# vsois/hanabi-agents

Measured on AMD Instinct MI355X. Metric: env_steps_per_sec, higher is better.
Workload: dtype u8 env/encoder + bfloat16 Q-net GEMM (fp32 accumulate, fp32 master weights)

## Files before the change

### hanabi-agents_amd/csrc/learner.hip

```cpp
#include <hip/hip_runtime.h>
#include <cstdlib>
#include <cstdint>
#include <hip/hip_bf16.h>
#include <hip/hip_fp16.h>

#include "../../include/hanabi_hip.h"
#include "common.hpp"

using hb::fail;

namespace {

template <typename T> __device__ __forceinline__ float ld(const T* p, long long i);
template <> __device__ __forceinline__ float ld<float>(const float* p, long long i) { return p[i]; }
template <> __device__ __forceinline__ float ld<__hip_bfloat16>(const __hip_bfloat16* p, long long i) { return __bfloat162float(p[i]); }
template <> __device__ __forceinline__ float ld<__half>(const __half* p, long long i) { return __half2float(p[i]); }
template <typename T> __device__ __forceinline__ void st(T* p, long long i, float v);
template <> __device__ __forceinline__ void st<float>(float* p, long long i, float v) { p[i] = v; }
template <> __device__ __forceinline__ void st<__hip_bfloat16>(__hip_bfloat16* p, long long i, float v) { p[i] = __float2bfloat16(v); }
template <> __device__ __forceinline__ void st<__half>(__half* p, long long i, float v) { p[i] = __float2half(v); }

__device__ __forceinline__ float wave_max(float v) {
  for (int o = 32; o > 0; o >>= 1) v = fmaxf(v, __shfl_xor(v, o));
  return v;
}
__device__ __forceinline__ float wave_sum(float v) {
  for (int o = 32; o > 0; o >>= 1) v += __shfl_xor(v, o);
  return v;
}

struct NStep {
  const long long* size_wp;
  long long cap, n_ins;
  int n_step;
  float gamma;
};

template <typename T>
__global__ __launch_bounds__(256) void gather_kernel(const int8_t* __restrict__ ring_tm1, const int8_t* __restrict__ ring_t,
                                                     const int8_t* __restrict__ ring_act, const float* __restrict__ ring_rew,
                                                     const uint8_t* __restrict__ ring_term, const int64_t* __restrict__ idx,
                                                     int B, int L, T* __restrict__ x, int x_ld, int32_t* __restrict__ act,
                                                     float* __restrict__ rew, float* __restrict__ term,
                                                     float* __restrict__ disc, const NStep ns, int packed_words) {
  __shared__ long long s_slot;
  const int r = blockIdx.x;
  const int b = r < B ? r : r - B;
  long long slot = idx[b];
  if (r >= B) {
    if (threadIdx.x == 0) {
      long long j = slot;
      float R = ring_rew[j], g = ns.gamma;
      int m = 1;
      if (ns.n_step > 1) {
        const long long size = ns.size_wp[0], wp = ns.size_wp[1];
        const long long ahead = size >= ns.cap ? ((wp - 1 - slot) % ns.cap + ns.cap) % ns.cap : size - 1 - slot;
        while (m < ns.n_step && !ring_term[j] && static_cast<long long>(m) * ns.n_ins <= ahead) {
          j = (j + ns.n_ins) % ns.cap;
          R += g * ring_rew[j];
          g *= ns.gamma;
          ++m;
        }
      }
      rew[b] = R;
      term[b] = ring_term[j] ? 1.f : 0.f;
      disc[b] = g;
      s_slot = j;
    }
    __syncthreads();
    slot = s_slot;
  } else if (threadIdx.x == 0) {
    act[b] = ring_act[slot];
  }
  T* dst = x + static_cast<long long>(r) * x_ld;
  if (packed_words > 0) {
    const uint32_t* src = reinterpret_cast<const uint32_t*>(r < B ? ring_tm1 : ring_t) + slot * packed_words;
    for (int j = threadIdx.x; j < L; j += 256) st<T>(dst, j, static_cast<float>((src[j >> 5] >> (j & 31)) & 1u));
    return;
  }
  const int8_t* src = (r < B ? ring_tm1 : ring_t) + slot * L;
  for (int j = threadIdx.x; j < L; j += 256) st<T>(dst, j, static_cast<float>(src[j]));
}

template <typename T>
__global__ __launch_bounds__(256) void c51_kernel(const T* __restrict__ logits_on, const T* __restrict__ logits_t,
                                                  const int32_t* __restrict__ act, const float* __restrict__ rew,
                                                  const float* __restrict__ term, const double* __restrict__ prios,
                                                  const float* __restrict__ beta_dev, const float* __restrict__ disc, int mask_terminal,
                                                  const float* __restrict__ support, int B, int A, int K, int rs,
                                                  float* __restrict__ td_out, float* __restrict__ w_out,
                                                  T* __restrict__ dlogits, float* __restrict__ counter,
                                                  const T* __restrict__ bias_on, const T* __restrict__ bias_t) {
  extern __shared__ float lds[];
  const int lane = threadIdx.x & 63, wave = threadIdx.x >> 6;
  const int b = blockIdx.x * 4 + wave;
  if (counter && blockIdx.x == 0 && threadIdx.x == 0) *counter += 1.f;
  if (b >= B) return;
  const int AK = A * K;
  float* sel = lds + wave * (AK + 64);
  const float beta = *beta_dev;
  float wmax = 0.f;
  for (int j = lane; j < B; j += 64) wmax = fmaxf(wmax, powf(static_cast<float>(1.0 / prios[j]), beta));
  wmax = wave_max(wmax);
  const float w_b = powf(static_cast<float>(1.0 / prios[b]), beta) / wmax;
  const T* row_sel = logits_on + static_cast<long long>(B + b) * rs;
  for (int e = lane; e < AK; e += 64) sel[e] = ld<T>(row_sel, e) + (bias_on ? ld<T>(bias_on, e) : 0.f);
  __builtin_amdgcn_fence(__ATOMIC_RELEASE, "wavefront");
  __builtin_amdgcn_wave_barrier();
  __builtin_amdgcn_fence(__ATOMIC_ACQUIRE, "wavefront");
  float q = -INFINITY;
  if (lane < A) {
    const float* r = sel + lane * K;
    float m = r[0];
    for (int k = 1; k < K; ++k) m = fmaxf(m, r[k]);
    float s = 0.f, t = 0.f;
    for (int k = 0; k < K; ++k) {
      const float e = __expf(r[k] - m);
      s += e;
      t += e * support[k];
    }
    q = t / s / static_cast<float>(K);
  }
  const float qbest = wave_max(q);
  const unsigned long long hit = __ballot(lane < A && q == qbest);
  const int a_star = __ffsll(static_cast<long long>(hit)) - 1;
  const bool atom = lane < K;
  const float lt = atom ? ld<T>(logits_t, static_cast<long long>(b) * rs + a_star * K + lane) +
                              (bias_t ? ld<T>(bias_t, a_star * K + lane) : 0.f)
                        : -INFINITY;
  const float mt = wave_max(lt);
  const float et = atom ? __expf(lt - mt) : 0.f;
  const float p = et / wave_sum(et);
  const float vmin = support[0], vmax = support[K - 1];
  const float delta = (vmax - vmin) / static_cast<float>(K - 1);
  float gamma = disc[b];
  if (mask_terminal) gamma *= 1.f - term[b];
  const float zi = atom ? support[lane] : 0.f;
  const float tz = fminf(fmaxf(rew[b] + gamma * zi, vmin), vmax);
  float target = 0.f;
  const float inv_delta = 1.f / delta;
  for (int j = 0; j < K; ++j) {
    const float pj = __int_as_float(__builtin_amdgcn_readlane(__float_as_int(p), j));
    const float tzj = __int_as_float(__builtin_amdgcn_readlane(__float_as_int(tz), j));
    target += pj * fminf(fmaxf(1.f - fabsf(tzj - zi) * inv_delta, 0.f), 1.f);
  }
  if (!atom) target = 0.f;
  const int a_tm1 = act[b];
  const float l1 = atom ? ld<T>(logits_on, static_cast<long long>(b) * rs + a_tm1 * K + lane) +
                              (bias_on ? ld<T>(bias_on, a_tm1 * K + lane) : 0.f)
                        : -INFINITY;
  const float m1 = wave_max(l1);
  const float e1 = atom ? __expf(l1 - m1) : 0.f;
  const float s1 = wave_sum(e1);
  const float logp = atom ? (l1 - m1 - __logf(s1)) : 0.f;
  const float td = -wave_sum(target * logp);
  const float tsum = wave_sum(target);
  if (lane == 0) {
    td_out[b] = td;
    w_out[b] = w_b;
  }
  T* drow = dlogits + static_cast<long long>(b) * rs;
  for (int e = lane; e < rs; e += 64) st<T>(drow, e, 0.f);
  __builtin_amdgcn_fence(__ATOMIC_RELEASE, "wavefront");
  __builtin_amdgcn_wave_barrier();
  if (atom) st<T>(drow, a_tm1 * K + lane, (w_b / static_cast<float>(B)) * (e1 / s1 * tsum - target));
}

template <typename T>
__global__ __launch_bounds__(1024) void colsum_kernel(const T* __restrict__ x, int rows, int cols, float* __restrict__ out) {
  __shared__ float part[16][64];
  const int l = threadIdx.x & 63, c = blockIdx.x * 64 + l, rg = threadIdx.x >> 6;
  float s = 0.f;
  if (c < cols) {
#pragma unroll 16
    for (int i = rg; i < rows; i += 16) s += ld<T>(x, static_cast<long long>(i) * cols + c);
  }
  part[rg][l] = s;
  __syncthreads();
  if (rg == 0 && c < cols) {
    float t = 0.f;
#pragma unroll
    for (int g = 0; g < 16; ++g) t += part[g][l];
    out[c] = t;
  }
}

template <typename T>
__global__ __launch_bounds__(1024) void relu_bwd_colsum_kernel(T* __restrict__ dy, const T* __restrict__ act, int rows, int cols,
                                                               int act_ld, float* __restrict__ out) {
  __shared__ float part[16][64];
  const int l = threadIdx.x & 63, c = blockIdx.x * 64 + l, rg = threadIdx.x >> 6;
  float s = 0.f;
  if (c < cols) {
#pragma unroll 16
    for (int i = rg; i < rows; i += 16) {
      const long long k = static_cast<long long>(i) * cols + c;
      const float g = ld<T>(act, static_cast<long long>(i) * act_ld + c) > 0.f ? ld<T>(dy, k) : 0.f;
      st<T>(dy, k, g);
      s += g;
    }
  }
  part[rg][l] = s;
  __syncthreads();
  if (rg == 0 && c < cols) {
    float t = 0.f;
#pragma unroll
    for (int g = 0; g < 16; ++g) t += part[g][l];
    out[c] = t;
  }
}

struct AdamArgs {
  float *w, *w_mu, *w_sigma;
  const float* noise;
  const void* grad;
  float *m_w, *v_w, *m_mu, *v_mu, *m_sg, *v_sg;
  const float* step;
  void* eff;
  long long n;
  int cols, eff_ld;
  int grad_dtype, grad_ld;
  float lr, b1, b2, eps;
  float step_offset;
};

__device__ __forceinline__ float load_grad(const void* g, int dtype, long long i) {
  if (dtype == 1) return __bfloat162float(static_cast<const __hip_bfloat16*>(g)[i]);
  if (dtype == 2) return __half2float(static_cast<const __half*>(g)[i]);
  return static_cast<const float*>(g)[i];
}

__device__ __forceinline__ float adam1(float p, float g, float& m, float& v, float b1, float b2, float bc1, float bc2s,
                                       float lr, float eps) {
  m = __fmaf_rn(b1, m, __fmul_rn(1.f - b1, g));
  v = __fmaf_rn(b2, v, __fmul_rn(__fmul_rn(1.f - b2, g), g));
  return __fsub_rn(p, __fdiv_rn(__fmul_rn(lr / bc1, m), __fadd_rn(__fdiv_rn(sqrtf(v), bc2s), eps)));
}
__device__ __forceinline__ float adam_step(float m, float v, float bc1, float bc2s, float lr, float eps) {
  return __fdiv_rn(__fmul_rn(lr / bc1, m), __fadd_rn(__fdiv_rn(sqrtf(v), bc2s), eps));
}
__device__ __forceinline__ float merged(float w, float mu, float sg, float nz) {
  return __fadd_rn(__fadd_rn(w, mu), __fmul_rn(sg, nz));
}

template <typename T>
__global__ __launch_bounds__(256) void noisy_adam_kernel(const AdamArgs a) {
  const float t = *a.step + a.step_offset;
  const float bc1 = 1.f - powf(a.b1, t), bc2s = sqrtf(1.f - powf(a.b2, t));
  T* eff = static_cast<T*>(a.eff);
  for (long long i = static_cast<long long>(blockIdx.x) * blockDim.x + threadIdx.x; i < a.n;
       i += static_cast<long long>(gridDim.x) * blockDim.x) {
    const long long row = i / a.cols, col = i - row * a.cols;
    const float g = load_grad(a.grad, a.grad_dtype, row * a.grad_ld + col), nz = a.noise[i];
    float m, v;
    m = a.m_w[i]; v = a.v_w[i];
    const float w = adam1(a.w[i], g, m, v, a.b1, a.b2, bc1, bc2s, a.lr, a.eps);
    a.m_w[i] = m; a.v_w[i] = v; a.w[i] = w;
    float mu;
    if (a.m_mu == a.m_w) {
      mu = __fsub_rn(a.w_mu[i], adam_step(m, v, bc1, bc2s, a.lr, a.eps));
    } else {
      m = a.m_mu[i]; v = a.v_mu[i];
      mu = adam1(a.w_mu[i], g, m, v, a.b1, a.b2, bc1, bc2s, a.lr, a.eps);
      a.m_mu[i] = m; a.v_mu[i] = v;
    }
    a.w_mu[i] = mu;
    m = a.m_sg[i]; v = a.v_sg[i];
    const float sg = adam1(a.w_sigma[i], __fmul_rn(g, nz), m, v, a.b1, a.b2, bc1, bc2s, a.lr, a.eps);
    a.m_sg[i] = m; a.v_sg[i] = v; a.w_sigma[i] = sg;
    st<T>(eff, row * a.eff_ld + col, merged(w, mu, sg, nz));
  }
}

struct AdamMulti {
  AdamArgs t[8];
  int first[9];
  int count;
};

template <int W> struct VecW;
template <> struct VecW<4> { typedef float4 type; };
template <> struct VecW<2> { typedef float2 type; };
template <int W>
__device__ __forceinline__ void ldw(const float* p, uint32_t off, float out[W]) {
  const typename VecW<W>::type v = *reinterpret_cast<const typename VecW<W>::type*>(reinterpret_cast<const char*>(p) + static_cast<uint64_t>(off << 2));
  const float* f = reinterpret_cast<const float*>(&v);
#pragma unroll
  for (int k = 0; k < W; ++k) out[k] = f[k];
}
template <int W>
__device__ __forceinline__ void stw(float* p, uint32_t off, const float in[W]) {
  typename VecW<W>::type v;
  float* f = reinterpret_cast<float*>(&v);
#pragma unroll
  for (int k = 0; k < W; ++k) f[k] = in[k];
  *reinterpret_cast<typename VecW<W>::type*>(reinterpret_cast<char*>(p) + static_cast<uint64_t>(off << 2)) = v;
}
template <int W>
__device__ __forceinline__ void load_gradw(const void* g, int dtype, uint32_t i, float out[W]) {
  if (dtype == 0) {
    ldw<W>(static_cast<const float*>(g), i, out);
  } else if (dtype == 1) {
    const uint32_t* p = reinterpret_cast<const uint32_t*>(static_cast<const char*>(g) + static_cast<uint64_t>(i << 1));
    if constexpr (W == 4) {
      const uint2 v = *reinterpret_cast<const uint2*>(p);
      out[0] = __uint_as_float(v.x << 16); out[1] = __uint_as_float(v.x & 0xFFFF0000u);
      out[2] = __uint_as_float(v.y << 16); out[3] = __uint_as_float(v.y & 0xFFFF0000u);
    } else {
      const uint32_t v = *p;
      out[0] = __uint_as_float(v << 16); out[1] = __uint_as_float(v & 0xFFFF0000u);
    }
  } else {
    const __half* h = reinterpret_cast<const __half*>(static_cast<const char*>(g) + static_cast<uint64_t>(i << 1));
#pragma unroll
    for (int k = 0; k < W; ++k) out[k] = __half2float(h[k]);
  }
}

template <typename T, int W>
__global__ __launch_bounds__(256) void noisy_adam_multiw_kernel(const AdamMulti m) {
  constexpr int SH = W == 4 ? 2 : 1;
  int ti = 0;
  while (ti + 1 < m.count && static_cast<int>(blockIdx.x) >= m.first[ti + 1]) ++ti;
  const AdamArgs& a = m.t[ti];
  const float t = *a.step + a.step_offset;
  const float bc1 = 1.f - powf(a.b1, t), bc2s = sqrtf(1.f - powf(a.b2, t));
  T* eff = static_cast<T*>(a.eff);
  const int nw = static_cast<int>(a.n >> SH), cw = a.cols >> SH;
  const int q = (static_cast<int>(blockIdx.x) - m.first[ti]) * 256 + static_cast<int>(threadIdx.x);
  if (q < nw) {
    const int row = q / cw, col = (q - row * cw) << SH;
    const uint32_t i = static_cast<uint32_t>(q) << SH;
    float g[W], nz[W];
    load_gradw<W>(a.grad, a.grad_dtype, static_cast<uint32_t>(row) * static_cast<uint32_t>(a.grad_ld) + col, g);
    ldw<W>(a.noise, i, nz);
    float res[3][W], lm[W], lv[W];
    auto one = [&](float* p, float* mp, float* vp, int which) {
      float pa[W], ma[W], va[W];
      ldw<W>(p, i, pa); ldw<W>(mp, i, ma); ldw<W>(vp, i, va);
#pragma unroll
      for (int k = 0; k < W; ++k) {
        pa[k] = adam1(pa[k], which == 2 ? __fmul_rn(g[k], nz[k]) : g[k], ma[k], va[k], a.b1, a.b2, bc1, bc2s, a.lr, a.eps);
        res[which][k] = pa[k];
        lm[k] = ma[k];
        lv[k] = va[k];
      }
      stw<W>(p, i, pa); stw<W>(mp, i, ma); stw<W>(vp, i, va);
    };
    one(a.w, a.m_w, a.v_w, 0);

    if (a.m_mu == a.m_w) {
      float pv[W];
      ldw<W>(a.w_mu, i, pv);
#pragma unroll
      for (int k = 0; k < W; ++k) res[1][k] = pv[k] = __fsub_rn(pv[k], adam_step(lm[k], lv[k], bc1, bc2s, a.lr, a.eps));
      stw<W>(a.w_mu, i, pv);
    } else {
      one(a.w_mu, a.m_mu, a.v_mu, 1);
    }

    one(a.w_sigma, a.m_sg, a.v_sg, 2);
    const uint32_t e = static_cast<uint32_t>(row) * static_cast<uint32_t>(a.eff_ld) + col;
#pragma unroll
    for (int k = 0; k < W; ++k) st<T>(eff, e + k, merged(res[0][k], res[1][k], res[2][k], nz[k]));
  }
}

template <typename T>
__global__ __launch_bounds__(256) void noisy_adam_multi_kernel(const AdamMulti m) {
  int ti = 0;
  while (ti + 1 < m.count && static_cast<int>(blockIdx.x) >= m.first[ti + 1]) ++ti;
  const AdamArgs& a = m.t[ti];
  const int nb = m.first[ti + 1] - m.first[ti];
  const float t = *a.step + a.step_offset;
  const float bc1 = 1.f - powf(a.b1, t), bc2s = sqrtf(1.f - powf(a.b2, t));
  T* eff = static_cast<T*>(a.eff);
  for (long long i = static_cast<long long>(blockIdx.x - m.first[ti]) * 256 + threadIdx.x; i < a.n;
       i += static_cast<long long>(nb) * 256) {
    const long long row = i / a.cols, col = i - row * a.cols;
    const float g = load_grad(a.grad, a.grad_dtype, row * a.grad_ld + col), nz = a.noise[i];
    float mm, vv;
    mm = a.m_w[i]; vv = a.v_w[i];
    const float w = adam1(a.w[i], g, mm, vv, a.b1, a.b2, bc1, bc2s, a.lr, a.eps);
    a.m_w[i] = mm; a.v_w[i] = vv; a.w[i] = w;
    float mu;
    if (a.m_mu == a.m_w) {
      mu = __fsub_rn(a.w_mu[i], adam_step(mm, vv, bc1, bc2s, a.lr, a.eps));
    } else {
      mm = a.m_mu[i]; vv = a.v_mu[i];
      mu = adam1(a.w_mu[i], g, mm, vv, a.b1, a.b2, bc1, bc2s, a.lr, a.eps);
      a.m_mu[i] = mm; a.v_mu[i] = vv;
    }
    a.w_mu[i] = mu;
    mm = a.m_sg[i]; vv = a.v_sg[i];
    const float sg = adam1(a.w_sigma[i], __fmul_rn(g, nz), mm, vv, a.b1, a.b2, bc1, bc2s, a.lr, a.eps);
    a.m_sg[i] = mm; a.v_sg[i] = vv; a.w_sigma[i] = sg;
    st<T>(eff, row * a.eff_ld + col, merged(w, mu, sg, nz));
  }
}

struct AdamPackOut {
  void* wt; int wt_ld;
  uint4* frag; int frag_kind;
  const int* col_map;
  float* bias_f32;
};
struct AdamPackMulti {
  AdamArgs t[4];
  AdamPackOut o[4];
  int first[5];
  int tiles_n[4];
  int count;
};

template <typename T>
__global__ __launch_bounds__(256) void noisy_adam_pack_kernel(const AdamPackMulti m) {
  __shared__ uint16_t tile[8][132];
  int ti = 0;
  while (ti + 1 < m.count && static_cast<int>(blockIdx.x) >= m.first[ti + 1]) ++ti;
  const AdamArgs& a = m.t[ti];
  const AdamPackOut& o = m.o[ti];
  const int tid = static_cast<int>(threadIdx.x), tb = static_cast<int>(blockIdx.x) - m.first[ti];
  const float t = *a.step + a.step_offset;
  const float bc1 = 1.f - powf(a.b1, t), bc2s = sqrtf(1.f - powf(a.b2, t));
  T* eff = static_cast<T*>(a.eff);
  const int tn = m.tiles_n[ti];
  const int rows = static_cast<int>(a.n / a.cols);
  int k, n;
  if (tn > 0) {
    k = (tb / tn) * 8 + (tid >> 5);
    n = (tb % tn) * 128 + 4 * (tid & 31);
  } else {
    k = 0;
    n = (tb * 256 + tid) * 4;
  }
  const bool valid = k < rows && n < a.cols;
  float mv[4] = {0.f, 0.f, 0.f, 0.f};
  if (valid) {
    const uint32_t i = static_cast<uint32_t>(k) * static_cast<uint32_t>(a.cols) + n;
    float g[4], nz[4], res[3][4], lm[4], lv[4];
    load_gradw<4>(a.grad, a.grad_dtype, static_cast<uint32_t>(k) * static_cast<uint32_t>(a.grad_ld) + n, g);
    ldw<4>(a.noise, i, nz);
    auto one = [&](float* p, float* mp, float* vp, int which) {
      float pa[4], ma[4], va[4];
      ldw<4>(p, i, pa); ldw<4>(mp, i, ma); ldw<4>(vp, i, va);
#pragma unroll
      for (int j = 0; j < 4; ++j) {
        pa[j] = adam1(pa[j], which == 2 ? __fmul_rn(g[j], nz[j]) : g[j], ma[j], va[j], a.b1, a.b2, bc1, bc2s, a.lr, a.eps);
        res[which][j] = pa[j];
        lm[j] = ma[j];
        lv[j] = va[j];
      }
      stw<4>(p, i, pa); stw<4>(mp, i, ma); stw<4>(vp, i, va);
    };
    one(a.w, a.m_w, a.v_w, 0);
    if (a.m_mu == a.m_w) {
      float pv[4];
      ldw<4>(a.w_mu, i, pv);
#pragma unroll
      for (int j = 0; j < 4; ++j) res[1][j] = pv[j] = __fsub_rn(pv[j], adam_step(lm[j], lv[j], bc1, bc2s, a.lr, a.eps));
      stw<4>(a.w_mu, i, pv);
    } else {
      one(a.w_mu, a.m_mu, a.v_mu, 1);
    }
    one(a.w_sigma, a.m_sg, a.v_sg, 2);
    const uint32_t e = static_cast<uint32_t>(k) * static_cast<uint32_t>(a.eff_ld) + n;
#pragma unroll
    for (int j = 0; j < 4; ++j) {
      mv[j] = merged(res[0][j], res[1][j], res[2][j], nz[j]);
      st<T>(eff, e + j, mv[j]);
    }
    if (tn == 0 && o.bias_f32) {
#pragma unroll
      for (int j = 0; j < 4; ++j) o.bias_f32[o.col_map ? o.col_map[n + j] : n + j] = ld<T>(eff, e + j);
    }
  }
  if (tn == 0 || (!o.wt && !o.frag_kind)) return;
  {
    T r4[4];
#pragma unroll
    for (int j = 0; j < 4; ++j) st<T>(r4, j, mv[j]);
    *reinterpret_cast<uint2*>(&tile[tid >> 5][4 * (tid & 31)]) = *reinterpret_cast<const uint2*>(r4);
  }
  __syncthreads();
  if (tid < 128) {
    const int col = tid;
    const int nn = (tb % tn) * 128 + col, k0 = (tb / tn) * 8;
    if (nn < a.cols) {
      uint16_t v[8];
#pragma unroll
      for (int i = 0; i < 8; ++i) v[i] = tile[i][col];
      const uint4 vec = *reinterpret_cast<const uint4*>(v);
      if (o.wt) *reinterpret_cast<uint4*>(static_cast<uint16_t*>(o.wt) + static_cast<size_t>(nn) * o.wt_ld + k0) = vec;
      const int s = k0 >> 5, ch = (k0 >> 3) & 3;
      if (o.frag_kind == 1) {
        o.frag[(s * 32 + (nn >> 4)) * 64 + ch * 16 + (nn & 15)] = vec;
      } else if (o.frag_kind == 2) {
        const int ph = o.col_map[nn];
        o.frag[(((ph >> 9) * 16 + s) * 32 + ((ph & 511) >> 4)) * 64 + ch * 16 + (ph & 15)] = vec;
      }
    }
  }
}

template <typename T>
void launch_adam(const AdamArgs& a, hipStream_t s) {
  long long blocks = (a.n + 255) / 256;
  if (blocks > 2048) blocks = 2048;
  hipLaunchKernelGGL((noisy_adam_kernel<T>), dim3(static_cast<unsigned>(blocks)), dim3(256), 0, s, a);
}

}

extern "C" {

static int replay_gather_impl(const int8_t* ring_obs_tm1_dev, const int8_t* ring_obs_t_dev, const int8_t* ring_act_dev,
                     const float* ring_rew_dev, const uint8_t* ring_term_dev, const int64_t* idx_dev, int64_t batch,
                     int32_t obs_len, void* x_dev, int32_t x_dtype, int32_t x_ld, int32_t* act_dev, float* rew_dev,
                     float* term_dev, float* disc_dev, int32_t n_step, float gamma, int64_t capacity, int64_t rows_per_insert,
                     const int64_t* size_wp_dev, void* stream, int packed_words) {
  if (!ring_obs_tm1_dev || !ring_obs_t_dev || !ring_act_dev || !ring_rew_dev || !ring_term_dev || !idx_dev || !x_dev ||
      !act_dev || !rew_dev || !term_dev || !disc_dev)
    return fail(HB_ERR_INVALID, "null argument");
  if (batch <= 0) return HB_OK;
  if (x_ld < obs_len) return fail(HB_ERR_INVALID, "x_ld must be >= obs_len");
  if (n_step < 1) return fail(HB_ERR_INVALID, "n_step must be >= 1");
  if (n_step > 1 && (!size_wp_dev || rows_per_insert < 1 || capacity < 1))
    return fail(HB_ERR_INVALID, "n_step > 1 needs size_wp_dev, rows_per_insert and capacity");
  const NStep ns{reinterpret_cast<const long long*>(size_wp_dev), capacity, rows_per_insert, n_step, gamma};
  hipStream_t s = static_cast<hipStream_t>(stream);
  const dim3 grid(static_cast<unsigned>(2 * batch)), block(256);
  const int B = static_cast<int>(batch);
  if (x_dtype == 0)
    hipLaunchKernelGGL((gather_kernel<float>), grid, block, 0, s, ring_obs_tm1_dev, ring_obs_t_dev, ring_act_dev, ring_rew_dev, ring_term_dev, idx_dev, B, obs_len, static_cast<float*>(x_dev), x_ld, act_dev, rew_dev, term_dev, disc_dev, ns, packed_words);
  else if (x_dtype == 1)
    hipLaunchKernelGGL((gather_kernel<__hip_bfloat16>), grid, block, 0, s, ring_obs_tm1_dev, ring_obs_t_dev, ring_act_dev, ring_rew_dev, ring_term_dev, idx_dev, B, obs_len, static_cast<__hip_bfloat16*>(x_dev), x_ld, act_dev, rew_dev, term_dev, disc_dev, ns, packed_words);
  else if (x_dtype == 2)
    hipLaunchKernelGGL((gather_kernel<__half>), grid, block, 0, s, ring_obs_tm1_dev, ring_obs_t_dev, ring_act_dev, ring_rew_dev, ring_term_dev, idx_dev, B, obs_len, static_cast<__half*>(x_dev), x_ld, act_dev, rew_dev, term_dev, disc_dev, ns, packed_words);
  else
    return fail(HB_ERR_INVALID, "x_dtype must be 0 (f32), 1 (bf16) or 2 (f16)");
  HB_HIP(hipGetLastError());
  return HB_OK;
}

int hb_replay_gather(const int8_t* ring_obs_tm1_dev, const int8_t* ring_obs_t_dev, const int8_t* ring_act_dev,
                     const float* ring_rew_dev, const uint8_t* ring_term_dev, const int64_t* idx_dev, int64_t batch,
                     int32_t obs_len, void* x_dev, int32_t x_dtype, int32_t x_ld, int32_t* act_dev, float* rew_dev,
                     float* term_dev, float* disc_dev, int32_t n_step, float gamma, int64_t capacity, int64_t rows_per_insert,
                     const int64_t* size_wp_dev, void* stream) {
  return replay_gather_impl(ring_obs_tm1_dev, ring_obs_t_dev, ring_act_dev, ring_rew_dev, ring_term_dev, idx_dev, batch, obs_len,
                            x_dev, x_dtype, x_ld, act_dev, rew_dev, term_dev, disc_dev, n_step, gamma, capacity, rows_per_insert,
                            size_wp_dev, stream, 0);
}

int hb_replay_gather_packed(const uint32_t* ring_bits_tm1_dev, const uint32_t* ring_bits_t_dev, const int8_t* ring_act_dev,
                            const float* ring_rew_dev, const uint8_t* ring_term_dev, const int64_t* idx_dev, int64_t batch,
                            int32_t obs_len, void* x_dev, int32_t x_dtype, int32_t x_ld, int32_t* act_dev, float* rew_dev,
                            float* term_dev, float* disc_dev, int32_t n_step, float gamma, int64_t capacity,
                            int64_t rows_per_insert, const int64_t* size_wp_dev, void* stream) {
  if (obs_len < 1) return fail(HB_ERR_INVALID, "obs_len must be positive");
  return replay_gather_impl(reinterpret_cast<const int8_t*>(ring_bits_tm1_dev), reinterpret_cast<const int8_t*>(ring_bits_t_dev),
                            ring_act_dev, ring_rew_dev, ring_term_dev, idx_dev, batch, obs_len, x_dev, x_dtype, x_ld, act_dev,
                            rew_dev, term_dev, disc_dev, n_step, gamma, capacity, rows_per_insert, size_wp_dev, stream,
                            (obs_len + 31) / 32);
}

int hb_c51_loss_grad(const void* logits_online_dev, const void* logits_target_dev, int32_t dtype, const int32_t* act_dev,
                     const float* rew_dev, const float* term_dev, const double* prios_dev, const float* beta_dev,
                     const float* disc_dev, int32_t mask_terminal, const float* support_dev, int64_t batch, int32_t n_actions,
                     int32_t n_atoms, int32_t row_stride, float* td_dev, float* w_dev, void* dlogits_dev, float* update_counter_dev,
                     const void* bias_online_dev, const void* bias_target_dev, void* stream) {
  if (!logits_online_dev || !logits_target_dev || !act_dev || !rew_dev || !term_dev || !prios_dev || !beta_dev || !disc_dev ||
      !support_dev || !td_dev || !w_dev || !dlogits_dev)
    return fail(HB_ERR_INVALID, "null argument");
  if (n_actions < 1 || n_actions > 64 || n_atoms < 2 || n_atoms > 64) return fail(HB_ERR_INVALID, "need n_actions <= 64 and 2 <= n_atoms <= 64");
  if (batch <= 0) return HB_OK;
  if (row_stride < n_actions * n_atoms) return fail(HB_ERR_INVALID, "row_stride must be >= n_actions * n_atoms");
  hipStream_t s = static_cast<hipStream_t>(stream);
  const dim3 grid(static_cast<unsigned>((batch + 3) / 4)), block(256);
  const size_t lds = 4 * (static_cast<size_t>(n_actions) * n_atoms + 64) * sizeof(float);
  const int B = static_cast<int>(batch);
#define HB_C51(T)                                                                                                       \
  hipLaunchKernelGGL((c51_kernel<T>), grid, block, lds, s, static_cast<const T*>(logits_online_dev),                    \
                     static_cast<const T*>(logits_target_dev), act_dev, rew_dev, term_dev, prios_dev, beta_dev, disc_dev, \
                     mask_terminal, support_dev, B, n_actions, n_atoms, row_stride, td_dev, w_dev, static_cast<T*>(dlogits_dev),       \
                     update_counter_dev, static_cast<const T*>(bias_online_dev), static_cast<const T*>(bias_target_dev))
  if (dtype == 0) HB_C51(float);
  else if (dtype == 1) HB_C51(__hip_bfloat16);
  else if (dtype == 2) HB_C51(__half);
  else return fail(HB_ERR_INVALID, "dtype must be 0 (f32), 1 (bf16) or 2 (f16)");
#undef HB_C51
  HB_HIP(hipGetLastError());
  return HB_OK;
}

int hb_colsum(const void* x_dev, int32_t dtype, int64_t rows, int64_t cols, float* out_dev, void* stream) {
  if (!x_dev || !out_dev) return fail(HB_ERR_INVALID, "null argument");
  if (rows <= 0 || cols <= 0) return HB_OK;
  hipStream_t s = static_cast<hipStream_t>(stream);
  const dim3 grid(static_cast<unsigned>((cols + 63) / 64)), block(1024);
  const int r = static_cast<int>(rows), c = static_cast<int>(cols);
  if (dtype == 0) hipLaunchKernelGGL((colsum_kernel<float>), grid, block, 0, s, static_cast<const float*>(x_dev), r, c, out_dev);
  else if (dtype == 1) hipLaunchKernelGGL((colsum_kernel<__hip_bfloat16>), grid, block, 0, s, static_cast<const __hip_bfloat16*>(x_dev), r, c, out_dev);
  else if (dtype == 2) hipLaunchKernelGGL((colsum_kernel<__half>), grid, block, 0, s, static_cast<const __half*>(x_dev), r, c, out_dev);
  else return fail(HB_ERR_INVALID, "dtype must be 0 (f32), 1 (bf16) or 2 (f16)");
  HB_HIP(hipGetLastError());
  return HB_OK;
}

int hb_noisy_adam(float* w_dev, float* w_mu_dev, float* w_sigma_dev, const float* noise_dev, const float* grad_dev,
                  float* m_w_dev, float* v_w_dev, float* m_mu_dev, float* v_mu_dev, float* m_sigma_dev, float* v_sigma_dev,
                  const float* step_dev, void* eff_dev, int32_t eff_dtype, int64_t n, int32_t cols, int32_t eff_ld, float lr,
                  float beta1, float beta2, float eps, void* stream) {
  if (!w_dev || !w_mu_dev || !w_sigma_dev || !noise_dev || !grad_dev || !m_w_dev || !v_w_dev || !m_mu_dev || !v_mu_dev ||
      !m_sigma_dev || !v_sigma_dev || !step_dev || !eff_dev)
    return fail(HB_ERR_INVALID, "null argument");
  if (n <= 0) return HB_OK;
  if (cols < 1 || eff_ld < cols || n % cols) return fail(HB_ERR_INVALID, "need cols >= 1, eff_ld >= cols and n a multiple of cols");
  AdamArgs a{w_dev, w_mu_dev, w_sigma_dev, noise_dev, grad_dev, m_w_dev, v_w_dev, m_mu_dev, v_mu_dev, m_sigma_dev, v_sigma_dev,
             step_dev, eff_dev, n, cols, eff_ld, 0, cols, lr, beta1, beta2, eps, 1.f};
  hipStream_t s = static_cast<hipStream_t>(stream);
  if (eff_dtype == 0) launch_adam<float>(a, s);
  else if (eff_dtype == 1) launch_adam<__hip_bfloat16>(a, s);
  else if (eff_dtype == 2) launch_adam<__half>(a, s);
  else return fail(HB_ERR_INVALID, "eff_dtype must be 0 (f32), 1 (bf16) or 2 (f16)");
  HB_HIP(hipGetLastError());
  return HB_OK;
}

int hb_relu_bwd_colsum(void* dy_dev, const void* act_dev, int64_t act_ld, int32_t dtype, int64_t rows, int64_t cols,
                       float* out_dev, void* stream) {
  if (!dy_dev || !act_dev || !out_dev) return fail(HB_ERR_INVALID, "null argument");
  if (rows <= 0 || cols <= 0) return HB_OK;
  if (act_ld == 0) act_ld = cols;
  if (act_ld < cols) return fail(HB_ERR_INVALID, "act_ld must be 0 or >= cols");
  const int al = static_cast<int>(act_ld);
  hipStream_t s = static_cast<hipStream_t>(stream);
  const dim3 grid(static_cast<unsigned>((cols + 63) / 64)), block(1024);
  const int r = static_cast<int>(rows), c = static_cast<int>(cols);
  if (dtype == 0) hipLaunchKernelGGL((relu_bwd_colsum_kernel<float>), grid, block, 0, s, static_cast<float*>(dy_dev), static_cast<const float*>(act_dev), r, c, al, out_dev);
  else if (dtype == 1) hipLaunchKernelGGL((relu_bwd_colsum_kernel<__hip_bfloat16>), grid, block, 0, s, static_cast<__hip_bfloat16*>(dy_dev), static_cast<const __hip_bfloat16*>(act_dev), r, c, al, out_dev);
  else if (dtype == 2) hipLaunchKernelGGL((relu_bwd_colsum_kernel<__half>), grid, block, 0, s, static_cast<__half*>(dy_dev), static_cast<const __half*>(act_dev), r, c, al, out_dev);
  else return fail(HB_ERR_INVALID, "dtype must be 0 (f32), 1 (bf16) or 2 (f16)");
  HB_HIP(hipGetLastError());
  return HB_OK;
}

int hb_noisy_adam_multi(const hb_adam_tensor* tensors, int32_t count, const float* step_dev, float step_offset, int32_t eff_dtype,
                        float lr, float beta1, float beta2, float eps, void* stream) {
  if (!tensors || !step_dev) return fail(HB_ERR_INVALID, "null argument");
  if (count < 1 || count > 8) return fail(HB_ERR_INVALID, "count must be 1..8");
  AdamMulti m{};
  m.count = count;
  int blocks = 0;
  bool vec4 = true;
  const int width = [] { const char* e = getenv("HB_ADAM_WIDTH"); const int w = e ? atoi(e) : 4; return w == 2 || w == 1 ? w : 4; }();
  if (width == 1) vec4 = false;
  for (int i = 0; i < count; ++i) {
    const hb_adam_tensor& d = tensors[i];
    const int gl = d.grad_ld ? d.grad_ld : d.cols;
    auto al16 = [](const void* p) { return (reinterpret_cast<uintptr_t>(p) & 15u) == 0; };
    vec4 = vec4 && d.cols > 0 && d.cols % 4 == 0 && d.n % 4 == 0 && d.n < (1LL << 30) &&
           (d.n / d.cols) * static_cast<long long>(d.eff_ld > gl ? d.eff_ld : gl) < (1LL << 31) && d.eff_ld % 4 == 0 && gl % 4 == 0 && al16(d.w) &&
           al16(d.w_mu) && al16(d.w_sigma) && al16(d.noise) && al16(d.grad) && al16(d.m_w) && al16(d.v_w) && al16(d.m_mu) &&
           al16(d.v_mu) && al16(d.m_sigma) && al16(d.v_sigma);
  }
  for (int i = 0; i < count; ++i) {
    const hb_adam_tensor& d = tensors[i];
    if (!d.w || !d.w_mu || !d.w_sigma || !d.noise || !d.grad || !d.m_w || !d.v_w || !d.m_mu || !d.v_mu || !d.m_sigma ||
        !d.v_sigma || !d.eff)
      return fail(HB_ERR_INVALID, "null pointer in tensor %d", i);
    if (d.n <= 0 || d.cols < 1 || d.eff_ld < d.cols || d.n % d.cols) return fail(HB_ERR_INVALID, "bad shape in tensor %d", i);
    if (d.grad_dtype < 0 || d.grad_dtype > 2 || (d.grad_ld != 0 && d.grad_ld < d.cols))
      return fail(HB_ERR_INVALID, "bad gradient dtype / row stride in tensor %d", i);
    m.t[i] = AdamArgs{d.w, d.w_mu, d.w_sigma, d.noise, d.grad, d.m_w, d.v_w, d.m_mu, d.v_mu, d.m_sigma, d.v_sigma,
                      step_dev, d.eff, d.n, d.cols, d.eff_ld, d.grad_dtype, d.grad_ld ? d.grad_ld : d.cols, lr, beta1, beta2, eps, step_offset};
    m.first[i] = blocks;
    long long nb = ((vec4 ? d.n / width : d.n) + 255) / 256;
    if (!vec4 && nb > 1024) nb = 1024;
    blocks += static_cast<int>(nb);
  }
  m.first[count] = blocks;
  hipStream_t s = static_cast<hipStream_t>(stream);
  if (vec4 && width == 4 && eff_dtype == 0) hipLaunchKernelGGL((noisy_adam_multiw_kernel<float, 4>), dim3(blocks), dim3(256), 0, s, m);
  else if (vec4 && width == 4 && eff_dtype == 1) hipLaunchKernelGGL((noisy_adam_multiw_kernel<__hip_bfloat16, 4>), dim3(blocks), dim3(256), 0, s, m);
  else if (vec4 && width == 4 && eff_dtype == 2) hipLaunchKernelGGL((noisy_adam_multiw_kernel<__half, 4>), dim3(blocks), dim3(256), 0, s, m);
  else if (vec4 && eff_dtype == 0) hipLaunchKernelGGL((noisy_adam_multiw_kernel<float, 2>), dim3(blocks), dim3(256), 0, s, m);
  else if (vec4 && eff_dtype == 1) hipLaunchKernelGGL((noisy_adam_multiw_kernel<__hip_bfloat16, 2>), dim3(blocks), dim3(256), 0, s, m);
  else if (vec4 && eff_dtype == 2) hipLaunchKernelGGL((noisy_adam_multiw_kernel<__half, 2>), dim3(blocks), dim3(256), 0, s, m);
  else if (eff_dtype == 0) hipLaunchKernelGGL((noisy_adam_multi_kernel<float>), dim3(blocks), dim3(256), 0, s, m);
  else if (eff_dtype == 1) hipLaunchKernelGGL((noisy_adam_multi_kernel<__hip_bfloat16>), dim3(blocks), dim3(256), 0, s, m);
  else if (eff_dtype == 2) hipLaunchKernelGGL((noisy_adam_multi_kernel<__half>), dim3(blocks), dim3(256), 0, s, m);
  else return fail(HB_ERR_INVALID, "eff_dtype must be 0 (f32), 1 (bf16) or 2 (f16)");
  HB_HIP(hipGetLastError());
  return HB_OK;
}


int hb_noisy_adam_multi_pack(const hb_adam_tensor* tensors, const hb_adam_pack* packs, int32_t count, const float* step_dev,
                             float step_offset, int32_t eff_dtype, float lr, float beta1, float beta2, float eps, void* stream) {
  if (!tensors || !packs || !step_dev) return fail(HB_ERR_INVALID, "null argument");
  if (count < 1 || count > 4) return fail(HB_ERR_INVALID, "count must be 1..4");
  if (eff_dtype != 1 && eff_dtype != 2) return fail(HB_ERR_INVALID, "eff_dtype must be 1 (bf16) or 2 (f16): the copies are 16-bit");
  AdamPackMulti m{};
  m.count = count;
  int blocks = 0;
  auto al16 = [](const void* p) { return (reinterpret_cast<uintptr_t>(p) & 15u) == 0; };
  for (int i = 0; i < count; ++i) {
    const hb_adam_tensor& d = tensors[i];
    const hb_adam_pack& k = packs[i];
    if (!d.w || !d.w_mu || !d.w_sigma || !d.noise || !d.grad || !d.m_w || !d.v_w || !d.m_mu || !d.v_mu || !d.m_sigma ||
        !d.v_sigma || !d.eff)
      return fail(HB_ERR_INVALID, "null pointer in tensor %d", i);
    if (d.n <= 0 || d.cols < 1 || d.eff_ld < d.cols || d.n % d.cols) return fail(HB_ERR_INVALID, "bad shape in tensor %d", i);
    const int gl = d.grad_ld ? d.grad_ld : d.cols;
    const long long rows = d.n / d.cols;
    if (d.grad_dtype < 0 || d.grad_dtype > 2 || gl < d.cols) return fail(HB_ERR_INVALID, "bad gradient dtype / row stride in tensor %d", i);
    if (d.cols % 4 || d.n >= (1LL << 30) || rows * static_cast<long long>(d.eff_ld > gl ? d.eff_ld : gl) >= (1LL << 31) || d.eff_ld % 4 ||
        gl % 4 || !al16(d.w) || !al16(d.w_mu) || !al16(d.w_sigma) || !al16(d.noise) || !al16(d.grad) || !al16(d.m_w) || !al16(d.v_w) ||
        !al16(d.m_mu) || !al16(d.v_mu) || !al16(d.m_sigma) || !al16(d.v_sigma) || (reinterpret_cast<uintptr_t>(d.eff) & 7u))
      return fail(HB_ERR_ALIGN, "tensor %d: needs cols, row strides %% 4 == 0 and 16-byte aligned arrays", i);
    const bool tiled = rows > 1;
    if (tiled) {
      if (k.bias_f32) return fail(HB_ERR_INVALID, "tensor %d: bias_f32 is for one-row (bias) tensors", i);
      if (k.frag_kind < 0 || k.frag_kind > 2 || (k.frag_kind != 0) != (k.frag != nullptr)) return fail(HB_ERR_INVALID, "tensor %d: frag / frag_kind", i);
      if (k.frag_kind == 2 && (!k.col_map_dev || rows % 32)) return fail(HB_ERR_INVALID, "tensor %d: the output layer's copy needs col_map and rows %% 32 == 0", i);
      if (k.frag_kind == 1 && d.cols != 512) return fail(HB_ERR_INVALID, "tensor %d: the first layer's fragment copy is for 512 hidden units", i);
      if (k.wt && (k.wt_ld < (rows + 7) / 8 * 8 || k.wt_ld % 8 || !al16(k.wt))) return fail(HB_ERR_INVALID, "tensor %d: wt_ld must cover the rows rounded up to 8 (and be a multiple of 8), wt 16-byte aligned", i);
      if (k.frag && !al16(k.frag)) return fail(HB_ERR_ALIGN, "tensor %d: frag must be 16-byte aligned", i);
    } else if (k.wt || k.frag || k.frag_kind) {
      return fail(HB_ERR_INVALID, "tensor %d: a one-row tensor has no transposed / fragment copy", i);
    }
    m.t[i] = AdamArgs{d.w, d.w_mu, d.w_sigma, d.noise, d.grad, d.m_w, d.v_w, d.m_mu, d.v_mu, d.m_sigma, d.v_sigma,
                      step_dev, d.eff, d.n, d.cols, d.eff_ld, d.grad_dtype, gl, lr, beta1, beta2, eps, step_offset};
    m.o[i] = AdamPackOut{k.wt, k.wt_ld, static_cast<uint4*>(k.frag), k.frag_kind, k.col_map_dev, k.bias_f32};
    m.first[i] = blocks;
    if (tiled) {
      m.tiles_n[i] = (d.cols + 127) / 128;
      blocks += static_cast<int>((rows + 7) / 8) * m.tiles_n[i];
    } else {
      m.tiles_n[i] = 0;
      blocks += static_cast<int>((d.n / 4 + 255) / 256);
    }
  }
  m.first[count] = blocks;
  hipStream_t s = static_cast<hipStream_t>(stream);
  if (eff_dtype == 1) hipLaunchKernelGGL((noisy_adam_pack_kernel<__hip_bfloat16>), dim3(blocks), dim3(256), 0, s, m);
  else hipLaunchKernelGGL((noisy_adam_pack_kernel<__half>), dim3(blocks), dim3(256), 0, s, m);
  HB_HIP(hipGetLastError());
  return HB_OK;
}

}
```

### hanabi-agents_amd/csrc/learner2.hip

```cpp
#include <hip/hip_runtime.h>
#include <hip/hip_bf16.h>
#include <hip/hip_fp16.h>

#include <cstdint>
#include <type_traits>

#include "../../include/hanabi_hip.h"
#include "common.hpp"

using hb::fail;

namespace {

template <typename T> __device__ __forceinline__ float ld(const T* p, long long i);
template <> __device__ __forceinline__ float ld<float>(const float* p, long long i) { return p[i]; }
template <> __device__ __forceinline__ float ld<__hip_bfloat16>(const __hip_bfloat16* p, long long i) { return __bfloat162float(p[i]); }
template <> __device__ __forceinline__ float ld<__half>(const __half* p, long long i) { return __half2float(p[i]); }
template <typename T> __device__ __forceinline__ void st(T* p, long long i, float v);
template <> __device__ __forceinline__ void st<float>(float* p, long long i, float v) { p[i] = v; }
template <> __device__ __forceinline__ void st<__hip_bfloat16>(__hip_bfloat16* p, long long i, float v) { p[i] = __float2bfloat16(v); }
template <> __device__ __forceinline__ void st<__half>(__half* p, long long i, float v) { p[i] = __float2half(v); }

template <typename T> __device__ __forceinline__ float rounded(float v);
template <> __device__ __forceinline__ float rounded<float>(float v) { return v; }
template <> __device__ __forceinline__ float rounded<__hip_bfloat16>(float v) { return __bfloat162float(__float2bfloat16(v)); }
template <> __device__ __forceinline__ float rounded<__half>(float v) { return __half2float(__float2half(v)); }

template <int CTRL, int ROW_MASK>
__device__ __forceinline__ float dpp_mov(float old, float v) {
  return __int_as_float(__builtin_amdgcn_update_dpp(__float_as_int(old), __float_as_int(v), CTRL, ROW_MASK, 0xf, false));
}
#define HB_WAVE_REDUCE(NAME, OP, IDENT)                                                       \
  __device__ __forceinline__ float NAME(float v) {                                            \
    v = OP(v, dpp_mov<0xb1, 0xf>(v, v));                             \
    v = OP(v, dpp_mov<0x4e, 0xf>(v, v));                             \
    v = OP(v, dpp_mov<0x124, 0xf>(v, v));                                      \
    v = OP(v, dpp_mov<0x128, 0xf>(v, v));   \
    v = OP(v, dpp_mov<0x142, 0xa>(IDENT, v));                  \
    v = OP(v, dpp_mov<0x143, 0xc>(IDENT, v));                  \
    return __int_as_float(__builtin_amdgcn_readlane(__float_as_int(v), 63));                  \
  }
__device__ __forceinline__ float op_add(float a, float b) { return a + b; }
HB_WAVE_REDUCE(wave_max, fmaxf, -INFINITY)
HB_WAVE_REDUCE(wave_min, fminf, INFINITY)
HB_WAVE_REDUCE(wave_sum, op_add, 0.f)
#undef HB_WAVE_REDUCE
__device__ __forceinline__ void wave_fence() {
  __builtin_amdgcn_fence(__ATOMIC_RELEASE, "wavefront");
  __builtin_amdgcn_wave_barrier();
  __builtin_amdgcn_fence(__ATOMIC_ACQUIRE, "wavefront");
}

constexpr int DL_LD = 64;

template <typename T> __device__ __forceinline__ float half_lo(uint32_t d);
template <typename T> __device__ __forceinline__ float half_hi(uint32_t d);
template <> __device__ __forceinline__ float half_lo<__hip_bfloat16>(uint32_t d) { return __uint_as_float(d << 16); }
template <> __device__ __forceinline__ float half_hi<__hip_bfloat16>(uint32_t d) { return __uint_as_float(d & 0xFFFF0000u); }
template <> __device__ __forceinline__ float half_lo<__half>(uint32_t d) { return __low2float(*reinterpret_cast<const __half2*>(&d)); }
template <> __device__ __forceinline__ float half_hi<__half>(uint32_t d) { return __high2float(*reinterpret_cast<const __half2*>(&d)); }
template <> __device__ __forceinline__ float half_lo<float>(uint32_t d) { return __uint_as_float(d); }
template <> __device__ __forceinline__ float half_hi<float>(uint32_t d) { return 0.f; }
template <typename T> __device__ __forceinline__ uint32_t pack2(float lo, float hi);
template <> __device__ __forceinline__ uint32_t pack2<__hip_bfloat16>(float lo, float hi) {
  const __hip_bfloat16 a = __float2bfloat16(lo), b = __float2bfloat16(hi);
  return static_cast<uint32_t>(*reinterpret_cast<const uint16_t*>(&a)) | (static_cast<uint32_t>(*reinterpret_cast<const uint16_t*>(&b)) << 16);
}
template <> __device__ __forceinline__ uint32_t pack2<__half>(float lo, float hi) {
  const __half2 h = __floats2half2_rn(lo, hi);
  return *reinterpret_cast<const uint32_t*>(&h);
}
template <> __device__ __forceinline__ uint32_t pack2<float>(float lo, float) { return __float_as_uint(lo); }

template <typename T>
__device__ __forceinline__ void stage_row(const T* __restrict__ row, const T* __restrict__ bias, float* dst, int n, int lane) {
  for (int base = 0; base < n; base += 1024) {
    float v[16];
#pragma unroll
    for (int i = 0; i < 16; ++i) {
      const int e = base + lane + 64 * i;
      v[i] = e < n ? ld<T>(row, e) + (bias ? ld<T>(bias, e) : 0.f) : 0.f;
    }
#pragma unroll
    for (int i = 0; i < 16; ++i) {
      const int e = base + lane + 64 * i;
      if (e < n) dst[e] = v[i];
    }
  }
}

template <typename T>
__global__ __launch_bounds__(64) void c51_sparse_kernel(const T* __restrict__ logits_on, const T* __restrict__ logits_t,
                                                        const int32_t* __restrict__ act, const float* __restrict__ rew,
                                                        const float* __restrict__ term, const double* __restrict__ prios,
                                                        const float* __restrict__ beta_dev, const float* __restrict__ disc,
                                                        int mask_terminal, const float* __restrict__ support, int B, int A, int K, int rs,
                                                        float* __restrict__ td_out, float* __restrict__ w_out, float* __restrict__ dl,
                                                        float* __restrict__ counter, const T* __restrict__ bias_on,
                                                        const T* __restrict__ bias_t) {
  extern __shared__ float sel[];
  const int lane = threadIdx.x, b = blockIdx.x;
  if (counter && b == 0 && lane == 0) *counter += 1.f;
  const int AK = A * K;
  const int a_tm1 = act[b];
  const float r_b = rew[b];
  float gamma = disc[b];
  if (mask_terminal) gamma *= 1.f - term[b];
  const bool atom = lane < K;
  const T* row_sel = logits_on + static_cast<long long>(B + b) * rs;
  stage_row<T>(row_sel, bias_on, sel, AK, lane);
  float* ssup = sel + AK;
  ssup[lane] = lane < K ? support[lane] : 0.f;
  const float l1 = atom ? ld<T>(logits_on, static_cast<long long>(b) * rs + a_tm1 * K + lane) +
                              (bias_on ? ld<T>(bias_on, a_tm1 * K + lane) : 0.f)
                        : -INFINITY;
  const float beta = *beta_dev;
  float ipmin = INFINITY, ipmax = 0.f;
  for (int j = lane; j < B; j += 64) {
    const float ip = static_cast<float>(1.0 / prios[j]);
    ipmin = fminf(ipmin, ip);
    ipmax = fmaxf(ipmax, ip);
  }
  ipmin = wave_min(ipmin);
  ipmax = wave_max(ipmax);
  const float wmax = powf(beta >= 0.f ? ipmax : ipmin, beta);
  const float w_b = powf(static_cast<float>(1.0 / prios[b]), beta) / wmax;
  wave_fence();
  const int S = 64 / A >= 1 ? 64 / A : 1;
  const int a_l = lane / S, part = lane - a_l * S;
  const bool on = a_l < A;
  const int per = (K + S - 1) / S, k0 = part * per, k1 = k0 + per < K ? k0 + per : K;
  const float* r = sel + (on ? a_l : 0) * K;
  float m = -INFINITY;
  if (on)
    for (int k = k0; k < k1; ++k) m = fmaxf(m, r[k]);
  float ma = m;
  for (int i = 0; i < S; ++i) ma = fmaxf(ma, __shfl(m, a_l * S + i));
  float s = 0.f, t = 0.f;
  if (on)
    for (int k = k0; k < k1; ++k) {
      const float e = __expf(r[k] - ma);
      s += e;
      t += e * ssup[k];
    }
  float sa = 0.f, ta = 0.f;
  for (int i = 0; i < S; ++i) {
    sa += __shfl(s, a_l * S + i);
    ta += __shfl(t, a_l * S + i);
  }
  const float q = on ? ta / sa / static_cast<float>(K) : -INFINITY;
  const float qbest = wave_max(q);
  const unsigned long long hit = __ballot(on && part == 0 && q == qbest);
  const int a_star = (__ffsll(static_cast<long long>(hit)) - 1) / S;
  const float lt = atom ? ld<T>(logits_t, static_cast<long long>(b) * rs + a_star * K + lane) +
                              (bias_t ? ld<T>(bias_t, a_star * K + lane) : 0.f)
                        : -INFINITY;
  const float mt = wave_max(lt);
  const float et = atom ? __expf(lt - mt) : 0.f;
  const float p = et / wave_sum(et);
  const float vmin = ssup[0], vmax = ssup[K - 1];
  const float delta = (vmax - vmin) / static_cast<float>(K - 1);
  const float zi = ssup[lane];
  const float tz = fminf(fmaxf(r_b + gamma * zi, vmin), vmax);
  float target = 0.f;
  const float inv_delta = 1.f / delta;
  for (int j = 0; j < K; ++j) {
    const float pj = __int_as_float(__builtin_amdgcn_readlane(__float_as_int(p), j));
    const float tzj = __int_as_float(__builtin_amdgcn_readlane(__float_as_int(tz), j));
    target += pj * fminf(fmaxf(1.f - fabsf(tzj - zi) * inv_delta, 0.f), 1.f);
  }
  if (!atom) target = 0.f;
  const float m1 = wave_max(l1);
  const float e1 = atom ? __expf(l1 - m1) : 0.f;
  const float s1 = wave_sum(e1);
  const float logp = atom ? (l1 - m1 - __logf(s1)) : 0.f;
  const float td = -wave_sum(target * logp);
  const float tsum = wave_sum(target);
  if (lane == 0) {
    td_out[b] = td;
    w_out[b] = w_b;
  }
  dl[static_cast<long long>(b) * DL_LD + lane] = atom ? (w_b / static_cast<float>(B)) * (e1 / s1 * tsum - target) : 0.f;
}

struct BwdArgs {
  const float* dl;
  const int32_t* act;
  const void* h;
  const void* w2;
  void* dh;
  float* db1;
  void* dw2;
  float* db2;
  int B, H, A, K, h_ld, w2_ld, dw2_ld;
  int n_dh_tiles;
};

constexpr int BWD_T = 1024;

template <typename T, int JT>
__global__ __launch_bounds__(BWD_T) void c51_backward_kernel(const BwdArgs a) {
  extern __shared__ __attribute__((aligned(16))) unsigned char smem[];
  __shared__ int wave_cnt[16];
  const int tid = threadIdx.x, lane = tid & 63, wave = tid >> 6;
  const T* h = static_cast<const T*>(a.h);
  const int blk = static_cast<int>(blockIdx.x);
  if (blk < a.n_dh_tiles) {
    constexpr int SLOT = sizeof(T) == 2 ? 72 : 68;
    constexpr int VEC = 16 / sizeof(T);
    constexpr int NCH = DL_LD / VEC;
    constexpr int CPP = NCH / 4;
    const int j0 = blk * JT;
    const int ld_w = a.A * SLOT;
    T* w2s = reinterpret_cast<T*>(smem);
    float* red = reinterpret_cast<float*>(smem + static_cast<size_t>(JT) * ld_w * sizeof(T));
    const T* w2 = static_cast<const T*>(a.w2);
    const int part = tid & 3;
    constexpr bool VEC_IO = JT * sizeof(T) == 16;
    const bool vec = VEC_IO && j0 + JT <= a.H && ((a.h_ld | a.H) & (JT - 1)) == 0;
    float dlv[CPP][VEC];
    float hin[JT];
    int c0 = 0;
    auto load_sample = [&](int base) {
      const int b = base + (tid >> 2);
      const int bb = b < a.B ? b : a.B - 1;
#pragma unroll
      for (int u = 0; u < CPP; ++u) {
        const float4* dlp = reinterpret_cast<const float4*>(a.dl + static_cast<long long>(bb) * DL_LD + (part + 4 * u) * VEC);
#pragma unroll
        for (int i = 0; i < VEC / 4; ++i) {
          const float4 v = dlp[i];
          dlv[u][4 * i] = v.x; dlv[u][4 * i + 1] = v.y; dlv[u][4 * i + 2] = v.z; dlv[u][4 * i + 3] = v.w;
        }
      }
      c0 = a.act[bb] * SLOT;
      if (vec) {
        const uint4 u = *reinterpret_cast<const uint4*>(h + static_cast<long long>(bb) * a.h_ld + j0);
        const uint32_t d[4] = {u.x, u.y, u.z, u.w};
        if constexpr (sizeof(T) == 4) {
#pragma unroll
          for (int i = 0; i < JT; ++i) hin[i] = __uint_as_float(d[i & 3]);
        } else {
#pragma unroll
          for (int i = 0; i < JT / 2; ++i) {
            hin[2 * i] = half_lo<T>(d[i & 3]);
            hin[2 * i + 1] = half_hi<T>(d[i & 3]);
          }
        }
      } else {
#pragma unroll
        for (int jj = 0; jj < JT; ++jj) hin[jj] = j0 + jj < a.H ? ld<T>(h, static_cast<long long>(bb) * a.h_ld + j0 + jj) : 0.f;
      }
    };
    load_sample(0);
    for (int e = tid; e < JT * ld_w * static_cast<int>(sizeof(T)) / 16; e += BWD_T) reinterpret_cast<uint4*>(smem)[e] = make_uint4(0, 0, 0, 0);
    __syncthreads();
    {
      const int AK = a.A * a.K;
      const float inv_k = 1.0f / static_cast<float>(a.K);
#pragma unroll
      for (int jj = 0; jj < JT; ++jj) {
        if (j0 + jj < a.H) {
          const T* src = w2 + static_cast<long long>(j0 + jj) * a.w2_ld;
          for (int c = tid; c < AK; c += BWD_T) {
            const int ac = static_cast<int>((static_cast<float>(c) + 0.5f) * inv_k);
            w2s[jj * ld_w + ac * SLOT + (c - ac * a.K)] = src[c];
          }
        }
      }
    }
    __syncthreads();
    const int kc = (a.K + VEC - 1) / VEC;
    float colsum[JT];
#pragma unroll
    for (int jj = 0; jj < JT; ++jj) colsum[jj] = 0.f;
    T* dh = static_cast<T*>(a.dh);
    for (int base = 0; base < a.B; base += BWD_T / 4) {
      const int b = base + (tid >> 2);
      const bool live = b < a.B;
      if (base > 0) load_sample(base);
      float gout[JT];
#pragma unroll
      for (int jj = 0; jj < JT; ++jj) {
        const uint4* wr = reinterpret_cast<const uint4*>(w2s + jj * ld_w + c0);
        float acc = 0.f;
#pragma unroll
        for (int u = 0; u < CPP; ++u) {
          const int c = part + 4 * u;
          if (c < kc) {
            const uint4 q = wr[c];
            const uint32_t d[4] = {q.x, q.y, q.z, q.w};
#pragma unroll
            for (int i = 0; i < 4; ++i) {
              if constexpr (sizeof(T) == 4) {
                acc = fmaf(dlv[u][i], __uint_as_float(d[i]), acc);
              } else if constexpr (std::is_same<T, __hip_bfloat16>::value) {
                acc = fmaf(dlv[u][2 * i], __uint_as_float(d[i] << 16), acc);
                acc = fmaf(dlv[u][2 * i + 1], __uint_as_float(d[i] & 0xFFFF0000u), acc);
              } else {
                const __half2 hh = *reinterpret_cast<const __half2*>(&d[i]);
                acc = fmaf(dlv[u][2 * i], __low2float(hh), acc);
                acc = fmaf(dlv[u][2 * i + 1], __high2float(hh), acc);
              }
            }
          }
        }
        acc += dpp_mov<0xb1, 0xf>(acc, acc);
        acc += dpp_mov<0x4e, 0xf>(acc, acc);
        const float g = hin[jj] > 0.f ? acc : 0.f;
        gout[jj] = g;
        if (live && part == 0 && j0 + jj < a.H) colsum[jj] += rounded<T>(g);
      }
      if (live && part == 0) {
        if (vec) {
          uint32_t d[4] = {0u, 0u, 0u, 0u};
          if constexpr (sizeof(T) == 4) {
#pragma unroll
            for (int i = 0; i < JT; ++i) d[i & 3] = __float_as_uint(gout[i]);
          } else {
#pragma unroll
            for (int i = 0; i < JT / 2; ++i) d[i & 3] = pack2<T>(gout[2 * i], gout[2 * i + 1]);
          }
          *reinterpret_cast<uint4*>(dh + static_cast<long long>(b) * a.H + j0) = make_uint4(d[0], d[1], d[2], d[3]);
        } else {
#pragma unroll
          for (int jj = 0; jj < JT; ++jj)
            if (j0 + jj < a.H) st<T>(dh, static_cast<long long>(b) * a.H + j0 + jj, gout[jj]);
        }
      }
    }
#pragma unroll
    for (int jj = 0; jj < JT; ++jj) {
      const float v = wave_sum(colsum[jj]);
      if (lane == 0) red[wave * JT + jj] = v;
    }
    __syncthreads();
    if (tid < JT && j0 + tid < a.H) {
      float t = 0.f;
      for (int w = 0; w < BWD_T / 64; ++w) t += red[w * JT + tid];
      a.db1[j0 + tid] = t;
    }
    return;
  }
  const int id = blk - a.n_dh_tiles;
  const int n_jt = (a.H + 63) / 64;
  const int act_id = id / n_jt, j0 = (id - act_id * n_jt) * 64;
  int* list = reinterpret_cast<int*>(smem);
  int n = 0;
  for (int base = 0; base < a.B; base += BWD_T) {
    const int b = base + tid;
    const bool mine = b < a.B && a.act[b] == act_id;
    const unsigned long long mk = __ballot(mine);
    if (lane == 0) wave_cnt[wave] = __popcll(mk);
    __syncthreads();
    int off = n, all = 0;
    for (int w = 0; w < BWD_T / 64; ++w) {
      if (w < wave) off += wave_cnt[w];
      all += wave_cnt[w];
    }
    if (mine) list[off + __popcll(mk & ((1ull << lane) - 1ull))] = b;
    n += all;
    __syncthreads();
  }
  const int kh = wave & 1, sq = wave >> 1;
  const int j = j0 + lane;
  const int per = (n + 7) >> 3;
  const int s_begin = sq * per, s_end = s_begin + per < n ? s_begin + per : n;
  float* dls = reinterpret_cast<float*>(smem) + ((a.B + 3) & ~3);
  float hreg[32];
#pragma unroll
  for (int u = 0; u < 32; ++u) {
    const bool ok = s_begin + u < s_end;
    const int b = list[ok ? s_begin + u : 0];
    hreg[u] = (ok && j < a.H) ? ld<T>(h, static_cast<long long>(b) * a.h_ld + j) : 0.f;
  }
  for (int e = tid; e < n * 16; e += BWD_T)
    reinterpret_cast<float4*>(dls)[e] = reinterpret_cast<const float4*>(a.dl + static_cast<long long>(list[e >> 4]) * DL_LD)[e & 15];
  __syncthreads();
  float acc[32];
#pragma unroll
  for (int i = 0; i < 32; ++i) acc[i] = 0.f;
  float dsum = 0.f;
#pragma unroll
  for (int u = 0; u < 32; ++u) {
    if (s_begin + u < s_end) {
      const float* dlp = dls + (s_begin + u) * DL_LD + kh * 32;
#pragma unroll
      for (int i = 0; i < 8; ++i) {
        const float4 d = reinterpret_cast<const float4*>(dlp)[i];
        acc[4 * i] = fmaf(hreg[u], d.x, acc[4 * i]);
        acc[4 * i + 1] = fmaf(hreg[u], d.y, acc[4 * i + 1]);
        acc[4 * i + 2] = fmaf(hreg[u], d.z, acc[4 * i + 2]);
        acc[4 * i + 3] = fmaf(hreg[u], d.w, acc[4 * i + 3]);
      }
      dsum += lane < 32 ? dlp[lane & 31] : 0.f;
    }
  }
  constexpr int RLD = 20;
  float* red = dls + static_cast<size_t>(a.B) * DL_LD;
  float* red2 = red + 8 * 64 * RLD;
  T* dw2 = static_cast<T*>(a.dw2);
#pragma unroll
  for (int p = 0; p < 4; ++p) {
    if (kh == (p >> 1)) {
      float4* dst = reinterpret_cast<float4*>(red + (sq * 64 + lane) * RLD);
#pragma unroll
      for (int i = 0; i < 4; ++i)
        dst[i] = make_float4(acc[(p & 1) * 16 + 4 * i], acc[(p & 1) * 16 + 4 * i + 1], acc[(p & 1) * 16 + 4 * i + 2],
                             acc[(p & 1) * 16 + 4 * i + 3]);
    }
    __syncthreads();
    {
      const int i = tid & 15, jj = tid >> 4, k = 16 * p + i;
      float t = 0.f;
#pragma unroll
      for (int r = 0; r < 8; ++r) t += red[(r * 64 + jj) * RLD + i];
      if (k < a.K && j0 + jj < a.H) st<T>(dw2, static_cast<long long>(j0 + jj) * a.dw2_ld + act_id * a.K + k, t);
    }
    __syncthreads();
  }
  if (j0 == 0) {
    if (lane < 32) red2[sq * 64 + kh * 32 + lane] = dsum;
    __syncthreads();
    if (tid < a.K) {
      float t = 0.f;
#pragma unroll
      for (int r = 0; r < 8; ++r) t += red2[r * 64 + tid];
      a.db2[act_id * a.K + tid] = t;
    }
  }
}

template <typename T>
int launch_backward(const BwdArgs& a0, hipStream_t s) {
  BwdArgs a = a0;
  const size_t row = static_cast<size_t>(a.A) * (sizeof(T) == 2 ? 72 : 68) * sizeof(T);
  const int n_jt = (a.H + 63) / 64;
  const size_t list_bytes = static_cast<size_t>((a.B + 3) & ~3) * 4;
  int jt = 8;
  while (jt > 1 && jt * row + 16 * jt * 4 > 64 * 1024) jt >>= 1;
  a.n_dh_tiles = (a.H + jt - 1) / jt;
  const unsigned blocks = static_cast<unsigned>(a.n_dh_tiles + a.A * n_jt);
  size_t lds = jt * row + 16 * jt * 4;
  if (lds < list_bytes) lds = list_bytes;
  const size_t dw2_bytes = list_bytes + static_cast<size_t>(a.B) * DL_LD * 4 + (8 * 64 * 20 + 8 * 64) * sizeof(float);
  if (lds < dw2_bytes) lds = dw2_bytes;
  if (lds > 150 * 1024) return fail(HB_ERR_INVALID, "batch / output layer too large for the backward kernel's LDS tile");
#define HB_BWD(JT) hipLaunchKernelGGL((c51_backward_kernel<T, JT>), dim3(blocks), dim3(BWD_T), lds, s, a)
  if (jt == 8) HB_BWD(8);
  else if (jt == 4) HB_BWD(4);
  else if (jt == 2) HB_BWD(2);
  else HB_BWD(1);
#undef HB_BWD
  return HB_OK;
}

template <typename T>
__global__ __launch_bounds__(256) void dqn_loss_kernel(const T* __restrict__ q_on, const T* __restrict__ q_t, const int32_t* __restrict__ act,
                                                       const float* __restrict__ rew, const float* __restrict__ term,
                                                       const double* __restrict__ prios, const float* __restrict__ beta_dev,
                                                       const float* __restrict__ disc, int B, int A, int cs, int rs,
                                                       float* __restrict__ td_out, float* __restrict__ w_out, float* __restrict__ dl,
                                                       const T* __restrict__ bias_on, const T* __restrict__ bias_t) {
  __shared__ float red[8];
  const int b = threadIdx.x, lane = b & 63, wave = b >> 6;
  const bool on = b < B;
  const float beta = *beta_dev;
  float ip = on ? static_cast<float>(1.0 / prios[b]) : (beta >= 0.f ? 0.f : INFINITY);
  float ext = ip;
  ext = beta >= 0.f ? wave_max(ext) : wave_min(ext);
  if (lane == 0) red[wave] = ext;
  __syncthreads();
  float e2 = red[0];
  for (int i = 1; i < (B + 63) / 64; ++i) e2 = beta >= 0.f ? fmaxf(e2, red[i]) : fminf(e2, red[i]);
  if (!on) return;
  const float w = powf(ip, beta) / powf(e2, beta);
  const int a_tm1 = act[b];
  const float q_tm1 = ld<T>(q_on, static_cast<long long>(b) * rs + a_tm1 * cs) + (bias_on ? ld<T>(bias_on, a_tm1 * cs) : 0.f);
  const T* sel = q_on + static_cast<long long>(B + b) * rs;
  int best = 0;
  float bv = -INFINITY;
  for (int a = 0; a < A; ++a) {
    const float v = ld<T>(sel, a * cs) + (bias_on ? ld<T>(bias_on, a * cs) : 0.f);
    if (v > bv) { bv = v; best = a; }
  }
  float qt = ld<T>(q_t, static_cast<long long>(b) * rs + best * cs) + (bias_t ? ld<T>(bias_t, best * cs) : 0.f);
  if (term[b] != 0.f) qt = 0.f;
  const float td = rew[b] + disc[b] * qt - q_tm1;
  td_out[b] = td;
  w_out[b] = w;
  float4* row = reinterpret_cast<float4*>(dl + static_cast<long long>(b) * 64);
  row[0] = make_float4(-w * td / static_cast<float>(B), 0.f, 0.f, 0.f);
#pragma unroll
  for (int i = 1; i < 16; ++i) row[i] = make_float4(0.f, 0.f, 0.f, 0.f);
}

typedef __bf16 tg_bf16x8 __attribute__((ext_vector_type(8)));
typedef _Float16 tg_f16x8 __attribute__((ext_vector_type(8)));
typedef float tg_f32x4 __attribute__((ext_vector_type(4)));
struct ThinArgs {
  const unsigned char* x;
  const unsigned char* wt;
  const __hip_bfloat16* bias;
  void* out;
  unsigned ldx, ldw, ldo;
  unsigned x_bs, w_bs, o_bs;
  int k, relu;
  unsigned n_tiles;
  unsigned nb;
};
template <bool F16>
__device__ __forceinline__ uint32_t tg_pack(float lo, float hi) {
  if constexpr (F16) {
    const _Float16 a = static_cast<_Float16>(lo), b = static_cast<_Float16>(hi);
    uint16_t ua, ub;
    __builtin_memcpy(&ua, &a, 2);
    __builtin_memcpy(&ub, &b, 2);
    return static_cast<uint32_t>(ua) | (static_cast<uint32_t>(ub) << 16);
  } else {
    const __hip_bfloat16 a = __float2bfloat16(lo), b = __float2bfloat16(hi);
    return static_cast<uint32_t>(*reinterpret_cast<const uint16_t*>(&a)) | (static_cast<uint32_t>(*reinterpret_cast<const uint16_t*>(&b)) << 16);
  }
}
template <bool F16>
__device__ __forceinline__ float tg_bias(const __hip_bfloat16* b, unsigned i) {
  if constexpr (F16) return __half2float(reinterpret_cast<const __half*>(b)[i]);
  else return __bfloat162float(b[i]);
}
template <bool F16>
__device__ __forceinline__ tg_f32x4 tg_mfma(const uint4& wv, const uint4& xv, const tg_f32x4& c) {
  if constexpr (F16) {
    union { uint4 u; tg_f16x8 f; } w, x;
    w.u = wv; x.u = xv;
    return __builtin_amdgcn_mfma_f32_16x16x32_f16(w.f, x.f, c, 0, 0, 0);
  } else {
    union { uint4 u; tg_bf16x8 f; } w, x;
    w.u = wv; x.u = xv;
    return __builtin_amdgcn_mfma_f32_16x16x32_bf16(w.f, x.f, c, 0, 0, 0);
  }
}
template <bool F16>
__global__ __launch_bounds__(64) void thin_gemm_kernel(const ThinArgs a, const int batch) {
  const int lane = threadIdx.x;
  const unsigned lr = lane & 15, kq = lane >> 4;
  const unsigned ct = blockIdx.y + a.n_tiles;
  const unsigned c = ct * 16u + 4u * kq;
  const unsigned half = 32u * a.ldx;
#pragma unroll 1
  for (int z = 0; z < batch; ++z) {
    float b0 = 0.f, b1 = 0.f, b2 = 0.f, b3 = 0.f;
    if (a.bias) {
      const __hip_bfloat16* bz = a.bias + static_cast<size_t>(z) * a.nb;
      b0 = tg_bias<F16>(bz, c); b1 = tg_bias<F16>(bz, c + 1); b2 = tg_bias<F16>(bz, c + 2); b3 = tg_bias<F16>(bz, c + 3);
    }
    const unsigned xo = (z * a.x_bs + (blockIdx.x * 32u + lr) * a.ldx + kq * 8u) * 2u;
    const unsigned wo = (z * a.w_bs + (ct * 16u + lr) * a.ldw + kq * 8u) * 2u;
    tg_f32x4 acc0 = tg_f32x4{0.f, 0.f, 0.f, 0.f}, acc1 = acc0;
    const unsigned kend = static_cast<unsigned>(a.k) * 2u;
#pragma unroll 1
    for (unsigned kb = 0; kb < kend; kb += 64u) {
      const uint4 x0 = *reinterpret_cast<const uint4*>(a.x + xo + kb), x1 = *reinterpret_cast<const uint4*>(a.x + xo + kb + half);
      const uint4 w0 = *reinterpret_cast<const uint4*>(a.wt + wo + kb);
      acc0 = tg_mfma<F16>(w0, x0, acc0);
      acc1 = tg_mfma<F16>(w0, x1, acc1);
    }
    float v[8] = {acc0[0] + b0, acc0[1] + b1, acc0[2] + b2, acc0[3] + b3, acc1[0] + b0, acc1[1] + b1, acc1[2] + b2, acc1[3] + b3};
    if (a.relu & 1) {
#pragma unroll
      for (int i = 0; i < 8; ++i) v[i] = fmaxf(v[i], 0.f);
    }
    const size_t oo = z * static_cast<size_t>(a.o_bs) + static_cast<size_t>(blockIdx.x * 32u + lr) * a.ldo + c;
    if (a.relu & 2) {
      float* o = static_cast<float*>(a.out) + oo;
      *reinterpret_cast<float4*>(o) = make_float4(v[0], v[1], v[2], v[3]);
      *reinterpret_cast<float4*>(o + 16u * static_cast<size_t>(a.ldo)) = make_float4(v[4], v[5], v[6], v[7]);
    } else {
      __hip_bfloat16* o = static_cast<__hip_bfloat16*>(a.out) + oo;
      *reinterpret_cast<uint2*>(o) = make_uint2(tg_pack<F16>(v[0], v[1]), tg_pack<F16>(v[2], v[3]));
      *reinterpret_cast<uint2*>(o + 16u * static_cast<size_t>(a.ldo)) = make_uint2(tg_pack<F16>(v[4], v[5]), tg_pack<F16>(v[6], v[7]));
    }
  }
}

struct FwdArgs {
  const unsigned char* x;
  const unsigned char* wt;
  const __hip_bfloat16* bias;
  void* out;
  const int32_t* act;
  unsigned ldx, ldw, ldo, x_bs, w_bs, o_bs, nb;
  int k, relu;
  unsigned n_gather;
  unsigned npair;
  unsigned n_units, stride;
  unsigned nrt;
  unsigned reg0_units;
  unsigned z[2], row0[2];
  int B, A, K;
};

template <bool F16>
__device__ __forceinline__ void tf_store(void* out, int relu, const __hip_bfloat16* bz, unsigned c0, size_t o0, size_t o1, bool st0,
                                         bool st1, const tg_f32x4& am0, const tg_f32x4& am1) {
  float b0 = 0.f, b1 = 0.f, b2 = 0.f, b3 = 0.f;
  if (bz) { b0 = tg_bias<F16>(bz, c0); b1 = tg_bias<F16>(bz, c0 + 1); b2 = tg_bias<F16>(bz, c0 + 2); b3 = tg_bias<F16>(bz, c0 + 3); }
  float v[8] = {am0[0] + b0, am0[1] + b1, am0[2] + b2, am0[3] + b3, am1[0] + b0, am1[1] + b1, am1[2] + b2, am1[3] + b3};
  if (relu & 1) {
#pragma unroll
    for (int i = 0; i < 8; ++i) v[i] = fmaxf(v[i], 0.f);
  }
  if (relu & 2) {
    float* o = static_cast<float*>(out) + c0;
    if (st0) *reinterpret_cast<float4*>(o + o0) = make_float4(v[0], v[1], v[2], v[3]);
    if (st1) *reinterpret_cast<float4*>(o + o1) = make_float4(v[4], v[5], v[6], v[7]);
  } else {
    __hip_bfloat16* o = static_cast<__hip_bfloat16*>(out) + c0;
    if (st0) *reinterpret_cast<uint2*>(o + o0) = make_uint2(tg_pack<F16>(v[0], v[1]), tg_pack<F16>(v[2], v[3]));
    if (st1) *reinterpret_cast<uint2*>(o + o1) = make_uint2(tg_pack<F16>(v[4], v[5]), tg_pack<F16>(v[6], v[7]));
  }
}

template <bool F16>
__global__ __launch_bounds__(64) void thin_forward_kernel(const FwdArgs a) {
  __shared__ int rows[32];
#pragma unroll 1
  for (unsigned u = blockIdx.x; u < a.n_units; u += a.stride) {
    int lane = threadIdx.x;
    asm volatile("" : "+v"(lane));
    const unsigned lr = lane & 15, kq = lane >> 4;
    unsigned z, r0, r1, t0;
    bool v0 = true, v1 = true;
    if (u < a.n_gather) {
      const unsigned g = u / a.npair, p = u - g * a.npair;
      int av[4];
#pragma unroll
      for (int i = 0; i < 4; ++i) av[i] = lane + 64 * i < a.B ? a.act[lane + 64 * i] : -1;
      int act_id = -1, cnt = 0;
      unsigned first = 0;
      for (int c = 0; c < a.A; ++c) {
        int n = 0;
#pragma unroll
        for (int i = 0; i < 4; ++i) n += __popcll(__ballot(av[i] == c));
        const unsigned ng = static_cast<unsigned>(n + 31) >> 5;
        if (g < first + ng) { act_id = c; cnt = n; break; }
        first += ng;
      }
      if (act_id < 0) continue;
      const unsigned tf = static_cast<unsigned>(act_id * a.K) >> 4, tl = static_cast<unsigned>(act_id * a.K + a.K - 1) >> 4;
      t0 = tf + p;
      if (t0 > tl) continue;
      const unsigned j = g - first;
      wave_fence();
      int base = 0;
#pragma unroll
      for (int i = 0; i < 4; ++i) {
        const bool mine = av[i] == act_id;
        const unsigned long long mk = __ballot(mine);
        const int rank = base + __popcll(mk & ((1ull << lane) - 1ull));
        if (mine && static_cast<unsigned>(rank >> 5) == j) rows[rank & 31] = lane + 64 * i;
        base += __popcll(mk);
      }
      wave_fence();
      const unsigned nr = static_cast<unsigned>(cnt) - 32u * j;
      v0 = lr < nr;
      v1 = lr + 16u < nr;
      r0 = static_cast<unsigned>(rows[v0 ? lr : 0u]);
      r1 = static_cast<unsigned>(rows[v1 ? lr + 16u : 0u]);
      z = 0u;
    } else {
      unsigned d = u - a.n_gather;
      const unsigned reg = d < a.reg0_units ? 0u : 1u;
      if (reg) d -= a.reg0_units;
      const unsigned ct = d / a.nrt, rt = d - ct * a.nrt;
      z = a.z[reg];
      r0 = a.row0[reg] + 32u * rt + lr;
      r1 = r0 + 16u;
      t0 = ct;
    }
    const unsigned xo0 = (z * a.x_bs + r0 * a.ldx + kq * 8u) * 2u, xo1 = (z * a.x_bs + r1 * a.ldx + kq * 8u) * 2u;
    const unsigned wo0 = (z * a.w_bs + (t0 * 16u + lr) * a.ldw + kq * 8u) * 2u;
    tg_f32x4 acc0 = {0.f, 0.f, 0.f, 0.f}, acc1 = {0.f, 0.f, 0.f, 0.f};
    const unsigned kend = static_cast<unsigned>(a.k) * 2u;
    unsigned kb = 0;
#pragma unroll 1
    for (; kb + 64u < kend; kb += 128u) {
      const uint4 x0 = *reinterpret_cast<const uint4*>(a.x + (xo0 + kb)), x1 = *reinterpret_cast<const uint4*>(a.x + (xo1 + kb));
      const uint4 w0 = *reinterpret_cast<const uint4*>(a.wt + (wo0 + kb));
      const uint4 y0 = *reinterpret_cast<const uint4*>(a.x + (xo0 + kb + 64u)), y1 = *reinterpret_cast<const uint4*>(a.x + (xo1 + kb + 64u));
      const uint4 u0 = *reinterpret_cast<const uint4*>(a.wt + (wo0 + kb + 64u));
      __builtin_amdgcn_sched_barrier(0);
      acc0 = tg_mfma<F16>(w0, x0, acc0);
      acc1 = tg_mfma<F16>(w0, x1, acc1);
      acc0 = tg_mfma<F16>(u0, y0, acc0);
      acc1 = tg_mfma<F16>(u0, y1, acc1);
    }
    if (kb < kend) {
      const uint4 x0 = *reinterpret_cast<const uint4*>(a.x + (xo0 + kb)), x1 = *reinterpret_cast<const uint4*>(a.x + (xo1 + kb));
      const uint4 w0 = *reinterpret_cast<const uint4*>(a.wt + (wo0 + kb));
      acc0 = tg_mfma<F16>(w0, x0, acc0);
      acc1 = tg_mfma<F16>(w0, x1, acc1);
    }
    const size_t ob = z * static_cast<size_t>(a.o_bs) + 4u * kq;
    const size_t o0 = ob + static_cast<size_t>(r0) * a.ldo, o1 = ob + static_cast<size_t>(r1) * a.ldo;
    const __hip_bfloat16* bz = a.bias ? a.bias + static_cast<size_t>(z) * a.nb + 4u * kq : nullptr;
    tf_store<F16>(a.out, a.relu, bz, t0 * 16u, o0, o1, v0, v1, acc0, acc1);
  }
}

}

extern "C" {

int hb_c51_loss_sparse(const void* logits_online_dev, const void* logits_target_dev, int32_t dtype, const int32_t* act_dev,
                       const float* rew_dev, const float* term_dev, const double* prios_dev, const float* beta_dev,
                       const float* disc_dev, int32_t mask_terminal, const float* support_dev, int64_t batch, int32_t n_actions,
                       int32_t n_atoms, int32_t row_stride, float* td_dev, float* w_dev, float* dl_dev, float* update_counter_dev,
                       const void* bias_online_dev, const void* bias_target_dev, void* stream) {
  if (!logits_online_dev || !logits_target_dev || !act_dev || !rew_dev || !term_dev || !prios_dev || !beta_dev || !disc_dev ||
      !support_dev || !td_dev || !w_dev || !dl_dev)
    return fail(HB_ERR_INVALID, "null argument");
  if (n_actions < 1 || n_actions > 64 || n_atoms < 2 || n_atoms > 64) return fail(HB_ERR_INVALID, "need n_actions <= 64 and 2 <= n_atoms <= 64");
  if (batch <= 0) return HB_OK;
  if (row_stride < n_actions * n_atoms) return fail(HB_ERR_INVALID, "row_stride must be >= n_actions * n_atoms");
  if (reinterpret_cast<uintptr_t>(dl_dev) & 15u) return fail(HB_ERR_ALIGN, "dl_dev must be 16-byte aligned");
  hipStream_t s = static_cast<hipStream_t>(stream);
  const dim3 grid(static_cast<unsigned>(batch)), block(64);
  const size_t lds = (static_cast<size_t>(n_actions) * n_atoms + 64) * sizeof(float);
  const int B = static_cast<int>(batch);
#define HB_C51S(T)                                                                                                        \
  hipLaunchKernelGGL((c51_sparse_kernel<T>), grid, block, lds, s, static_cast<const T*>(logits_online_dev),               \
                     static_cast<const T*>(logits_target_dev), act_dev, rew_dev, term_dev, prios_dev, beta_dev, disc_dev, \
                     mask_terminal, support_dev, B, n_actions, n_atoms, row_stride, td_dev, w_dev, dl_dev, update_counter_dev,       \
                     static_cast<const T*>(bias_online_dev), static_cast<const T*>(bias_target_dev))
  if (dtype == 0) HB_C51S(float);
  else if (dtype == 1) HB_C51S(__hip_bfloat16);
  else if (dtype == 2) HB_C51S(__half);
  else return fail(HB_ERR_INVALID, "dtype must be 0 (f32), 1 (bf16) or 2 (f16)");
#undef HB_C51S
  HB_HIP(hipGetLastError());
  return HB_OK;
}

int hb_thin_gemm(const void* x_dev, const void* wt_dev, const void* bias_dev, void* out_dev, int64_t m, int32_t n, int32_t k,
                 int32_t ldx, int32_t ldw, int32_t ldo, int32_t batch, int64_t x_batch_stride, int64_t w_batch_stride,
                 int64_t out_batch_stride, int32_t relu, void* stream) {
  if (!x_dev || !wt_dev || !out_dev) return fail(HB_ERR_INVALID, "null argument");
  if (m <= 0 || n <= 0 || batch <= 0) return HB_OK;
  if (m % 32 || n % 16 || k % 32 || k < 32) return fail(HB_ERR_INVALID, "need m % 32 == 0, n % 16 == 0, k % 32 == 0");
  if (ldx < k || ldw < k || ldo < n || ldx % 8 || ldw % 8 || ldo % 4) return fail(HB_ERR_INVALID, "bad leading dimensions");
  if (relu < 0 || relu > 7) return fail(HB_ERR_INVALID, "relu: bit 0 = ReLU, bit 1 = fp32 output, bit 2 = fp16 (not bf16) operands");
  if ((reinterpret_cast<uintptr_t>(x_dev) & 15u) || (reinterpret_cast<uintptr_t>(wt_dev) & 15u) ||
      (reinterpret_cast<uintptr_t>(out_dev) & ((relu & 2) ? 15u : 7u)))
    return fail(HB_ERR_ALIGN, "x / wt must be 16-byte aligned, out 8-byte (fp32 output: 16-byte) aligned");
  const int64_t xe = (batch - 1) * x_batch_stride + m * static_cast<int64_t>(ldx), we = (batch - 1) * w_batch_stride + n * static_cast<int64_t>(ldw);
  if (xe >= (1LL << 30) || we >= (1LL << 30)) return fail(HB_ERR_INVALID, "operands beyond the kernel's 32-bit offsets");
  ThinArgs a{static_cast<const unsigned char*>(x_dev), static_cast<const unsigned char*>(wt_dev),
             static_cast<const __hip_bfloat16*>(bias_dev), out_dev, static_cast<unsigned>(ldx),
             static_cast<unsigned>(ldw), static_cast<unsigned>(ldo), static_cast<unsigned>(x_batch_stride),
             static_cast<unsigned>(w_batch_stride), static_cast<unsigned>(out_batch_stride), k, relu, 0u, static_cast<unsigned>(n)};
  const unsigned tiles = static_cast<unsigned>(n / 16), gx = static_cast<unsigned>(m / 32), cap = gx >= 1024u ? 1u : 1024u / gx;
  for (unsigned t0 = 0; t0 < tiles; t0 += cap) {
    a.n_tiles = t0;
    const dim3 grid(gx, tiles - t0 < cap ? tiles - t0 : cap);
    if (relu & 4) hipLaunchKernelGGL((thin_gemm_kernel<true>), grid, dim3(64), 0, static_cast<hipStream_t>(stream), a, batch);
    else hipLaunchKernelGGL((thin_gemm_kernel<false>), grid, dim3(64), 0, static_cast<hipStream_t>(stream), a, batch);
  }
  HB_HIP(hipGetLastError());
  return HB_OK;
}

int hb_thin_forward(int32_t layer, const void* x_dev, const void* wt_dev, const void* bias_dev, void* out_dev, const int32_t* act_dev,
                    int64_t batch, int32_t n, int32_t k, int32_t ldx, int32_t ldw, int32_t ldo, int64_t x_batch_stride,
                    int64_t w_batch_stride, int64_t out_batch_stride, int32_t n_actions, int32_t n_atoms, int32_t relu, void* stream) {
  if (!x_dev || !wt_dev || !out_dev) return fail(HB_ERR_INVALID, "null argument");
  if (layer != 1 && layer != 2) return fail(HB_ERR_INVALID, "layer must be 1 or 2");
  if (batch <= 0 || n <= 0) return HB_OK;
  const int64_t m = 2 * batch;
  const int nz = layer == 2 ? 2 : 1;
  if (batch % 32 || n % (layer == 1 ? 32 : 16) || k % 32 || k < 32)
    return fail(HB_ERR_INVALID, "need batch % 32 == 0, n % 16 == 0 (layer 1: n % 32 == 0), k % 32 == 0");
  if (ldx < k || ldw < k || ldo < n || ldx % 8 || ldw % 8 || ldo % 4) return fail(HB_ERR_INVALID, "bad leading dimensions");
  if (relu < 0 || relu > 7) return fail(HB_ERR_INVALID, "relu: bit 0 = ReLU, bit 1 = fp32 output, bit 2 = fp16 (not bf16) operands");
  if ((reinterpret_cast<uintptr_t>(x_dev) & 15u) || (reinterpret_cast<uintptr_t>(wt_dev) & 15u) ||
      (reinterpret_cast<uintptr_t>(out_dev) & ((relu & 2) ? 15u : 7u)))
    return fail(HB_ERR_ALIGN, "x / wt must be 16-byte aligned, out 8-byte (fp32 output: 16-byte) aligned");
  if (layer == 2) {
    if (!act_dev) return fail(HB_ERR_INVALID, "null argument");
    if (batch > 256) return fail(HB_ERR_INVALID, "batch must be <= 256 (a wavefront keeps the batch's actions in four registers per lane)");
    if (n_actions < 1 || n_actions > 64 || n_atoms < 1 || n_atoms > 64 || n_actions * n_atoms > n)
      return fail(HB_ERR_INVALID, "need n_actions <= 64, n_atoms <= 64, n_actions * n_atoms <= n");
    if (x_batch_stride < 0 || w_batch_stride < 0 || out_batch_stride < 0) return fail(HB_ERR_INVALID, "negative batch stride");
    if (x_batch_stride % 8 || w_batch_stride % 8 || out_batch_stride % 4) return fail(HB_ERR_INVALID, "batch strides must keep the alignment");
  }
  const int64_t xe = (nz - 1) * x_batch_stride + m * static_cast<int64_t>(ldx), we = (nz - 1) * w_batch_stride + n * static_cast<int64_t>(ldw);
  if (xe >= (1LL << 30) || we >= (1LL << 30)) return fail(HB_ERR_INVALID, "operands beyond the kernel's 32-bit offsets");
  FwdArgs a{};
  a.x = static_cast<const unsigned char*>(x_dev);
  a.wt = static_cast<const unsigned char*>(wt_dev);
  a.bias = static_cast<const __hip_bfloat16*>(bias_dev);
  a.out = out_dev;
  a.act = act_dev;
  a.ldx = static_cast<unsigned>(ldx); a.ldw = static_cast<unsigned>(ldw); a.ldo = static_cast<unsigned>(ldo);
  a.nb = static_cast<unsigned>(n);
  a.k = k; a.relu = relu;
  a.B = static_cast<int>(batch);
  a.nrt = static_cast<unsigned>(batch / 32);
  const unsigned ncp = static_cast<unsigned>(n / 16);
  if (layer == 1) {
    a.npair = 1u;
    a.z[0] = a.z[1] = 0u;
    a.row0[0] = 0u; a.row0[1] = static_cast<unsigned>(batch);
    a.reg0_units = a.nrt * (ncp / 2u);
    a.n_units = a.reg0_units + a.nrt * ncp;
  } else {
    a.x_bs = static_cast<unsigned>(x_batch_stride); a.w_bs = static_cast<unsigned>(w_batch_stride); a.o_bs = static_cast<unsigned>(out_batch_stride);
    a.A = n_actions; a.K = n_atoms;
    a.npair = static_cast<unsigned>((n_atoms + 14) / 16 + 1);
    const unsigned groups = a.nrt + static_cast<unsigned>(n_actions < batch ? n_actions : batch);
    a.n_gather = groups * a.npair;
    a.z[0] = 0u; a.z[1] = 1u;
    a.row0[0] = a.row0[1] = static_cast<unsigned>(batch);
    a.reg0_units = a.nrt * ncp;
    a.n_units = a.n_gather + 2u * a.reg0_units;
  }
  const unsigned per = (a.n_units + 1023u) / 1024u;
  a.stride = (a.n_units + per - 1u) / per;
  if (relu & 4) hipLaunchKernelGGL((thin_forward_kernel<true>), dim3(a.stride), dim3(64), 0, static_cast<hipStream_t>(stream), a);
  else hipLaunchKernelGGL((thin_forward_kernel<false>), dim3(a.stride), dim3(64), 0, static_cast<hipStream_t>(stream), a);
  HB_HIP(hipGetLastError());
  return HB_OK;
}

int hb_dqn_loss_sparse(const void* q_online_dev, const void* q_target_dev, int32_t dtype, const int32_t* act_dev, const float* rew_dev,
                       const float* term_dev, const double* prios_dev, const float* beta_dev, const float* disc_dev, int64_t batch,
                       int32_t n_actions, int32_t col_stride, int32_t row_stride, float* td_dev, float* w_dev, float* dl_dev,
                       const void* bias_online_dev, const void* bias_target_dev, void* stream) {
  if (!q_online_dev || !q_target_dev || !act_dev || !rew_dev || !term_dev || !prios_dev || !beta_dev || !disc_dev || !td_dev ||
      !w_dev || !dl_dev)
    return fail(HB_ERR_INVALID, "null argument");
  if (batch <= 0) return HB_OK;
  if (batch > 256) return fail(HB_ERR_INVALID, "batch must be <= 256");
  if (n_actions < 1 || col_stride < 1 || row_stride < (n_actions - 1) * col_stride + 1) return fail(HB_ERR_INVALID, "bad action layout");
  if (reinterpret_cast<uintptr_t>(dl_dev) & 15u) return fail(HB_ERR_ALIGN, "dl_dev must be 16-byte aligned");
  hipStream_t s = static_cast<hipStream_t>(stream);
  const int B = static_cast<int>(batch);
#define HB_DQNL(T)                                                                                                           \
  hipLaunchKernelGGL((dqn_loss_kernel<T>), dim3(1), dim3(256), 0, s, static_cast<const T*>(q_online_dev),                      \
                     static_cast<const T*>(q_target_dev), act_dev, rew_dev, term_dev, prios_dev, beta_dev, disc_dev, B, n_actions, \
                     col_stride, row_stride, td_dev, w_dev, dl_dev, static_cast<const T*>(bias_online_dev),                    \
                     static_cast<const T*>(bias_target_dev))
  if (dtype == 0) HB_DQNL(float);
  else if (dtype == 1) HB_DQNL(__hip_bfloat16);
  else if (dtype == 2) HB_DQNL(__half);
  else return fail(HB_ERR_INVALID, "dtype must be 0 (f32), 1 (bf16) or 2 (f16)");
#undef HB_DQNL
  HB_HIP(hipGetLastError());
  return HB_OK;
}

int hb_c51_backward(const float* dl_dev, const int32_t* act_dev, const void* hidden_dev, int32_t hidden_ld, const void* w2_dev,
                    int32_t w2_ld, int32_t dtype, int64_t batch, int32_t hidden, int32_t n_actions, int32_t n_atoms, void* dh_dev,
                    float* db1_dev, void* dw2_dev, int32_t dw2_ld, float* db2_dev, void* stream) {
  if (!dl_dev || !act_dev || !hidden_dev || !w2_dev || !dh_dev || !db1_dev || !dw2_dev || !db2_dev)
    return fail(HB_ERR_INVALID, "null argument");
  if (n_actions < 1 || n_actions > 64 || n_atoms < 2 || n_atoms > 64) return fail(HB_ERR_INVALID, "need n_actions <= 64 and 2 <= n_atoms <= 64");
  if (batch <= 0) return HB_OK;
  if (batch > 256) return fail(HB_ERR_INVALID, "batch must be <= 256 (a thread keeps its share of one action's samples in 32 registers)");
  const int AK = n_actions * n_atoms;
  if (hidden < 1 || hidden_ld < hidden || w2_ld < AK || dw2_ld < AK) return fail(HB_ERR_INVALID, "bad hidden size / row strides");
  if (reinterpret_cast<uintptr_t>(dl_dev) & 15u) return fail(HB_ERR_ALIGN, "dl_dev must be 16-byte aligned");
  BwdArgs a{dl_dev, act_dev, hidden_dev, w2_dev, dh_dev, db1_dev, dw2_dev, db2_dev, static_cast<int>(batch), hidden, n_actions,
            n_atoms, hidden_ld, w2_ld, dw2_ld, 0};
  hipStream_t s = static_cast<hipStream_t>(stream);
  int rc;
  if (dtype == 0) rc = launch_backward<float>(a, s);
  else if (dtype == 1) rc = launch_backward<__hip_bfloat16>(a, s);
  else if (dtype == 2) rc = launch_backward<__half>(a, s);
  else return fail(HB_ERR_INVALID, "dtype must be 0 (f32), 1 (bf16) or 2 (f16)");
  if (rc) return rc;
  HB_HIP(hipGetLastError());
  return HB_OK;
}

}
```

### hanabi-agents_amd/hanabi_agents/rlax_dqn/fused_learner.py

```python
import os

import torch

from hanabi_hip import _capi as K

_DT = {torch.float32: 0, torch.bfloat16: 1, torch.float16: 2}


class FusedLearner:
    def __init__(self, agent):
        self.agent = agent
        p = agent.params
        dev = agent.device
        self.cd = {"float32": torch.float32, "bfloat16": torch.bfloat16, "float16": torch.float16}[p.compute_dtype]
        self.B = p.train_batch_size
        self.A, self.Kk = agent.atoms.shape
        self.L = agent.obs_len
        layers = agent.online.layers
        assert len(layers) == 2, "the fused learner covers the reference topology: one hidden layer (params.layers=[H])"
        self.layers = layers
        B, AK = self.B, self.A * self.Kk
        H = layers[0].out_features
        f32 = dict(dtype=torch.float32, device=dev)
        pad = (lambda v, m: (v + m - 1) // m * m) if self.cd != torch.float32 else (lambda v, m: v)
        self.Kp = pad(self.L, 64)
        self.Np = pad(AK, 64)
        self.w1cat = torch.zeros(self.Kp, 2 * H, dtype=self.cd, device=dev)
        self.b1cat = torch.zeros(2 * H, dtype=self.cd, device=dev)
        self.w2st = torch.zeros(2, H, self.Np, dtype=self.cd, device=dev)
        self.b2st = torch.zeros(2, self.Np, dtype=self.cd, device=dev)
        self.eff = [(self.w1cat[:, :H], self.b1cat[:H]), (self.w2st[0], self.b2st[0])]
        self.trg = [(self.w1cat[:, H:], self.b1cat[H:]), (self.w2st[1], self.b2st[1])]
        self.H = H
        self.thin = (self.cd in (torch.bfloat16, torch.float16) and self.Kp % 32 == 0 and H % 64 == 0 and self.Np % 16 == 0
                     and (2 * B) % 32 == 0)
        if self.thin:
            self.w1catT = torch.zeros(2 * H, self.Kp, dtype=self.cd, device=dev)
            self.w2stT = torch.zeros(2, self.Np, H, dtype=self.cd, device=dev)
            self._hcat = torch.zeros(2 * B, 2 * H, dtype=self.cd, device=dev)
            self._logits = torch.zeros(2, 2 * B, self.Np, **f32)
            self._bias_sink = torch.zeros(max(2 * H, self.Np), **f32)
            self._t_jobs = [None, None]
        self.trimmed = bool(self.thin and B % 32 == 0 and B <= 256 and self.Np % 32 == 0 and self.A <= 64 and self.Kk <= 64)
        self._dense_forward = False
        sizes = [layers[0].w.numel(), H, layers[1].w.numel(), AK]
        self.flat_grad = torch.zeros(sum(sizes), **f32)
        offs = [0]
        for s in sizes:
            offs.append(offs[-1] + s)
        self.g_w1 = self.flat_grad[offs[0]:offs[1]].view_as(layers[0].w)
        self.g_b1 = self.flat_grad[offs[1]:offs[2]]
        self.g_w2 = self.flat_grad[offs[2]:offs[3]].view_as(layers[1].w)
        self.g_b2 = self.flat_grad[offs[3]:offs[4]]
        self.state = {}
        for li, l in enumerate(layers):
            for name in ("w", "w_mu", "w_sigma", "b", "b_mu", "b_sigma"):
                t = getattr(l, name)
                self.state[(li, name)] = (torch.zeros_like(t), torch.zeros_like(t))
        for li in range(len(layers)):
            self.state[(li, "w_mu")] = self.state[(li, "w")]
            self.state[(li, "b_mu")] = self.state[(li, "b")]
        self.step = torch.zeros((), **f32)
        self.x = torch.zeros(2 * B, self.Kp, dtype=self.cd, device=dev)
        self.act = torch.empty(B, dtype=torch.int32, device=dev)
        self.rew = torch.empty(B, **f32)
        self.term = torch.empty(B, **f32)
        self.disc = torch.empty(B, **f32)
        self.td = torch.empty(B, **f32)
        self.w_is = torch.empty(B, **f32)
        self.dlogits = torch.zeros(B, self.Np, dtype=self.cd, device=dev)
        self.dl = torch.zeros(B, 64, **f32)
        self.dh = torch.zeros(B, H, dtype=self.cd, device=dev)
        self.sparse_backward = self.Kk <= 64 and self.A <= 64 and B <= 256
        self.AK = AK
        self.support = agent.atoms[0].contiguous()
        self._gb2_pad = torch.zeros(self.Np, **f32)
        self._adam_tab = None
        self._idx = self._prob = None
        self._sg_call = None
        self.direct = None
        from hanabi_hip.ops import ActorMFMA

        self.actor = None
        self.actor_stale = True
        self.lag = int(getattr(agent.params, "actor_lag", 0))
        if self.lag not in (0, 1):
            raise ValueError("actor_lag must be 0 or 1")
        self.n_packed = 0
        self._packed_in_part2 = False
        self.packed_ev = [None, None]
        if ActorMFMA.supports(self.L, H, self.Kk, self.Kp, self.cd, self.A) and getattr(agent, "use_mfma_actor", True):
            self.actor = ActorMFMA(self.L, H, self.A, self.Kk, self.Kp, dev, n_sets=2 if self.lag else 1, dtype=self.cd)
        self.pack_thin = bool(self.thin and self.actor is not None and self.actor.fused)
        if self.lag and (self.actor is None or not agent.params.use_priority or agent.params.resample_noise):
            raise ValueError("actor_lag=1 needs the MFMA actor (bf16 GEMM dtype, one hidden layer of a multiple of 256 units), "
                             "prioritized replay and frozen noise")
        self.adam_pack = None
        self._pack_tab = None
        self._gw2_out = torch.zeros(H, self.Np, dtype=self.cd, device=dev)
        self._gw1_out = torch.zeros(self.Kp, H, dtype=self.cd, device=dev)
        self.refresh_effective()
        self.refresh_target()

    @staticmethod
    def _store(dst_w, dst_b, w, b):
        dst_w[:w.shape[0], :w.shape[1]].copy_(w)
        dst_b[:b.shape[0]].copy_(b)

    def _transpose(self, which):
        jobs = self._t_jobs[which]
        if jobs is None:
            H = self.H
            (w1, b1), (w2, b2) = (self.eff, self.trg)[which]
            jobs = (K.HbPackJob * 2)()
            for j, (w, b, wt, k_rows, n_cols, kp) in enumerate(((w1, b1, self.w1catT[which * H:(which + 1) * H], self.Kp, H, self.Kp),
                                                                (w2, b2, self.w2stT[which], H, self.Np, H))):
                jobs[j].w, jobs[j].bias, jobs[j].wt, jobs[j].bias_out = w.data_ptr(), b.data_ptr(), wt.data_ptr(), self._bias_sink.data_ptr()
                jobs[j].k_rows, jobs[j].n_cols, jobs[j].w_ld, jobs[j].group_cols, jobs[j].k_pad = k_rows, n_cols, w.stride(0), 0, kp
            self._t_jobs[which] = jobs
        K.check(K.lib().hb_actor_pack_weights(jobs, 2, K.current_stream()))

    @torch.no_grad()
    def refresh_effective(self):
        for (w_e, b_e), l in zip(self.eff, self.layers):
            self._store(w_e, b_e, *l.effective())
        self.actor_stale = True
        if self.thin:
            self._transpose(0)

    def pack_actor(self):
        if self.actor is not None and self.actor_stale:
            (w1, b1), (w2, b2) = self.eff
            for s in range(self.actor.n_sets):
                self.actor.pack(w1, b1, w2, b2, s, lazy_two_kernel=not self.lag)
            self.actor_stale = False
            self.packed_ev = [None, None]

    def _thin_out(self):
        return (self.w1catT, self.Kp, self.w2stT[0], self.H) if self.pack_thin else None

    def weights_updated(self):
        if not self.lag:
            self.actor_stale = self.actor is not None and not self._packed_in_part2
            if self._packed_in_part2 and self.actor.fused and self.actor.two_kernel:
                self.actor._two_stale[0] = True
            return
        self.pack_actor()
        s = self.n_packed % 2
        (w1, b1), (w2, b2) = self.eff
        self.actor.pack(w1, b1, w2, b2, s, thin=self._thin_out())
        if self.packed_ev[s] is None:
            self.packed_ev[s] = K.Event()
        self.packed_ev[s].record()
        self.n_packed += 1

    def acting_set(self):
        self.pack_actor()
        if not self.lag:
            return 0
        s = self.n_packed % 2
        if self.packed_ev[s] is not None:
            self.packed_ev[s].wait()
        return s

    @torch.no_grad()
    def refresh_target(self):
        for (w_t, b_t), l in zip(self.trg, self.agent.target.layers):
            self._store(w_t, b_t, *l.effective())
        if self.thin:
            self._transpose(1)

    def sample_and_gather(self, seed):
        a = self.agent
        buf, B = a.experience, self.B
        rpi = buf.rows_per_insert
        c = self._sg_call
        if c is not None and c[0] == (rpi, buf._obs_t_buf.data_ptr()) and c[1] == seed:
            K.check(c[2](*c[3], K.current_stream()))
            return self._idx, self._prob
        L = K.lib()
        if a.params.n_step > 1 and (rpi is None or rpi < 1):
            raise ValueError("n_step > 1 needs inserts of a constant row count (lock-step self-play)")
        if self._idx is None:
            self._idx = torch.empty(B, dtype=torch.int64, device=a.device)
            self._prob = torch.empty(B, dtype=torch.float64, device=a.device)
        args = (buf.sum_tree.h, int(seed), K.dptr(self.step), B, K.dptr(self._idx), K.dptr(self._prob),
                K.dptr(buf._obs_tm1_buf), K.dptr(buf._obs_t_buf), K.dptr(buf._act_tm1_buf),
                K.dptr(buf._rew_t_buf), K.dptr(buf._terminal_t_buf), self.L, 1 if buf.packed else 0,
                K.dptr(self.x), _DT[self.cd], self.Kp, K.dptr(self.act), K.dptr(self.rew), K.dptr(self.term),
                K.dptr(self.disc), int(a.params.n_step), float(a.params.discount), buf.capacity,
                int(rpi or 1), K.dptr(buf._size_wp))
        self._sg_call = ((rpi, buf._obs_t_buf.data_ptr()), seed, L.hb_per_sample_gather, args)
        K.check(L.hb_per_sample_gather(*args, K.current_stream()))
        return self._idx, self._prob

    def part1(self, indices, prios, gathered=False):
        a, L = self.agent, K.lib()
        buf, B = a.experience, self.B
        if self.direct is None:
            self.direct = not a._collective()
        if self.adam_pack is None:
            self.adam_pack = bool(self.direct and self.thin and not self.lag and self.actor is not None and self.actor.fused
                                  and self.H == 512 and os.environ.get("HB_ADAM_PACK", "0") == "1")
        if a.params.n_step > 1 and (buf.rows_per_insert is None or buf.rows_per_insert < 1):
            raise ValueError("n_step > 1 needs inserts of a constant row count (lock-step self-play)")
        s = K.current_stream()
        if not gathered:
            gather = L.hb_replay_gather_packed if buf.packed else L.hb_replay_gather
            K.check(gather(K.dptr(buf._obs_tm1_buf), K.dptr(buf._obs_t_buf), K.dptr(buf._act_tm1_buf),
                           K.dptr(buf._rew_t_buf), K.dptr(buf._terminal_t_buf), K.dptr(indices), B, self.L,
                           K.dptr(self.x), _DT[self.cd], self.Kp, K.dptr(self.act), K.dptr(self.rew),
                           K.dptr(self.term), K.dptr(self.disc), int(a.params.n_step), float(a.params.discount),
                           buf.capacity, int(buf.rows_per_insert or 1), K.dptr(buf._size_wp), s))
        H = self.H
        w2 = self.eff[1][0]
        if self.thin:
            hcat, logits = self._hcat, self._logits
            if not (self.adam_pack or self.pack_thin):
                self._transpose(0)
            f16 = 4 if self.cd == torch.float16 else 0
            if self.trimmed and self.sparse_backward and not self._dense_forward:
                K.check(L.hb_thin_forward(1, K.dptr(self.x), K.dptr(self.w1catT), K.dptr(self.b1cat), K.dptr(hcat), None, B, 2 * H,
                                          self.Kp, self.Kp, self.Kp, 2 * H, 0, 0, 0, 0, 0, 1 | f16, s))
                K.check(L.hb_thin_forward(2, K.dptr(hcat), K.dptr(self.w2stT), K.dptr(self.b2st), K.dptr(logits), K.dptr(self.act), B,
                                          self.Np, H, 2 * H, H, self.Np, H, self.Np * H, 2 * B * self.Np, self.A, self.Kk, 2 | f16, s))
            else:
                K.check(L.hb_thin_gemm(K.dptr(self.x), K.dptr(self.w1catT), K.dptr(self.b1cat), K.dptr(hcat), 2 * B, 2 * H, self.Kp,
                                       self.Kp, self.Kp, 2 * H, 1, 0, 0, 0, 1 | f16, s))
                K.check(L.hb_thin_gemm(K.dptr(hcat), K.dptr(self.w2stT), K.dptr(self.b2st), K.dptr(logits), 2 * B, self.Np, H, 2 * H, H,
                                       self.Np, 2, H, self.Np * H, 2 * B * self.Np, 2 | f16, s))
        else:
            hcat = torch._addmm_activation(self.b1cat, self.x, self.w1cat, use_gelu=False)
            logits = torch.bmm(hcat.view(2 * B, 2, H).transpose(0, 1), self.w2st)
        logits_on, logits_t = logits[0], logits[1, B:]
        hb, xb = hcat[:B, :H], self.x[:B]
        ldt = 0 if self.thin else _DT[self.cd]
        bon, btg = (None, None) if self.thin else (self.b2st[0], self.b2st[1])
        if self.sparse_backward:
            K.check(L.hb_c51_loss_sparse(K.dptr(logits_on), K.dptr(logits_t), ldt, K.dptr(self.act), K.dptr(self.rew),
                                         K.dptr(self.term), K.dptr(prios), K.dptr(a._beta), K.dptr(self.disc),
                                         1 if a.params.mask_terminal else 0, K.dptr(self.support), B, self.A, self.Kk, self.Np,
                                         K.dptr(self.td), K.dptr(self.w_is), K.dptr(self.dl), K.dptr(self.step),
                                         K.dptr(bon), K.dptr(btg), s))
            K.check(L.hb_c51_backward(K.dptr(self.dl), K.dptr(self.act), K.dptr(hb), hb.stride(0), K.dptr(w2), w2.stride(0),
                                      _DT[self.cd], B, H, self.A, self.Kk, K.dptr(self.dh), K.dptr(self.g_b1),
                                      K.dptr(self._gw2_out), self.Np, K.dptr(self._gb2_pad), s))
            dh = self.dh
        else:
            if self.thin:
                logits_on, logits_t, ldt = logits_on.to(self.cd), logits_t.to(self.cd), _DT[self.cd]
            K.check(L.hb_c51_loss_grad(K.dptr(logits_on), K.dptr(logits_t), ldt, K.dptr(self.act), K.dptr(self.rew),
                                       K.dptr(self.term), K.dptr(prios), K.dptr(a._beta), K.dptr(self.disc),
                                       1 if a.params.mask_terminal else 0, K.dptr(self.support), B, self.A, self.Kk, self.Np,
                                       K.dptr(self.td), K.dptr(self.w_is), K.dptr(self.dlogits), K.dptr(self.step),
                                       K.dptr(bon), K.dptr(btg), s))
            dl = self.dlogits
            torch.mm(hb.t(), dl, out=self._gw2_out)
            K.check(L.hb_colsum(K.dptr(dl), _DT[self.cd], B, self.Np, K.dptr(self._gb2_pad), s))
            dh = torch.mm(dl, w2.t())
            K.check(L.hb_relu_bwd_colsum(K.dptr(dh), K.dptr(hb), hb.stride(0), _DT[self.cd], B, dh.shape[1], K.dptr(self.g_b1), s))
        torch.mm(xb.t(), dh, out=self._gw1_out)
        if not self.direct:
            self.g_w2.copy_(self._gw2_out[:, :self.AK])
            self.g_b2.copy_(self._gb2_pad[:self.AK])
            self.g_w1.copy_(self._gw1_out[:self.L])
        return self.td, self.w_is

    def _adam_table(self):
        if self._adam_tab is None:
            if self.direct:
                grads = (((self._gw1_out, _DT[self.cd], self._gw1_out.shape[1]), (self.g_b1, 0, 0)),
                         ((self._gw2_out, _DT[self.cd], self.Np), (self._gb2_pad, 0, 0)))
            else:
                grads = (((self.g_w1, 0, 0), (self.g_b1, 0, 0)), ((self.g_w2, 0, 0), (self.g_b2, 0, 0)))
            tab = (K.HbAdamTensor * 4)()
            k = 0
            for li, l in enumerate(self.layers):
                for names, noise, g, eff in ((("w", "w_mu", "w_sigma"), l.eps_w, grads[li][0], self.eff[li][0]),
                                             (("b", "b_mu", "b_sigma"), l.eps_b, grads[li][1], self.eff[li][1])):
                    ps = [getattr(l, n) for n in names]
                    st = [self.state[(li, n)] for n in names]
                    d = tab[k]
                    d.w, d.w_mu, d.w_sigma = (p.data_ptr() for p in ps)
                    d.noise, d.grad, d.grad_dtype, d.grad_ld = noise.data_ptr(), g[0].data_ptr(), g[1], g[2]
                    d.m_w, d.v_w = st[0][0].data_ptr(), st[0][1].data_ptr()
                    d.m_mu, d.v_mu = st[1][0].data_ptr(), st[1][1].data_ptr()
                    d.m_sigma, d.v_sigma = st[2][0].data_ptr(), st[2][1].data_ptr()
                    d.eff, d.n, d.cols = eff.data_ptr(), ps[0].numel(), ps[0].shape[-1]
                    d.eff_ld = eff.stride(0) if eff.dim() == 2 else eff.shape[-1]
                    k += 1
            self._adam_tab = tab
        return self._adam_tab

    def _pack_table(self):
        if self._pack_tab is None:
            import ctypes

            n_log = self.A * self.Kk
            host = (ctypes.c_int32 * n_log)()
            K.check(K.lib().hb_actor_fused_columns(self.A, host))
            self._col_map = torch.tensor(list(host), dtype=torch.int32, device=self.agent.device)
            f = self.actor.fsets[0]
            tab = (K.HbAdamPack * 4)()
            tab[0].wt, tab[0].wt_ld, tab[0].frag, tab[0].frag_kind = self.w1catT.data_ptr(), self.Kp, f[0].data_ptr(), 1
            tab[1].bias_f32 = f[1].data_ptr()
            tab[2].wt, tab[2].wt_ld, tab[2].frag, tab[2].frag_kind = self.w2stT[0].data_ptr(), self.H, f[2].data_ptr(), 2
            tab[2].col_map_dev = self._col_map.data_ptr()
            tab[3].bias_f32, tab[3].col_map_dev = f[3].data_ptr(), self._col_map.data_ptr()
            self._pack_tab = tab
        return self._pack_tab

    def part2(self, opt=True, pack=True):
        p = self.agent.params
        if self.adam_pack:
            assert opt and pack, "hb_noisy_adam_multi_pack: the optimizer step and the copies are one launch"
            K.check(K.lib().hb_noisy_adam_multi_pack(self._adam_table(), self._pack_table(), 4, K.dptr(self.step), 0.0, _DT[self.cd],
                                                     float(p.learning_rate), 0.9, 0.999, 3.125e-5, K.current_stream()))
            self._packed_in_part2 = True
            return
        if opt:
            K.check(K.lib().hb_noisy_adam_multi(self._adam_table(), 4, K.dptr(self.step), 0.0, _DT[self.cd],
                                                float(p.learning_rate), 0.9, 0.999, 3.125e-5, K.current_stream()))
        if not pack:
            return
        self._packed_in_part2 = False
        if self.actor is not None and not self.lag:
            (w1, b1), (w2, b2) = self.eff
            self.actor.pack(w1, b1, w2, b2, 0, lazy_two_kernel=True, thin=self._thin_out())
            self._packed_in_part2 = True

    def loss(self):
        return torch.mean(self.td * self.w_is)
```

### hanabi-agents_amd/hanabi_hip/_capi.py

```python
import ctypes as C
import os

_HERE = os.path.dirname(os.path.abspath(__file__))
_LIB = None

FLAG_AUTO_RESET, FLAG_RESET_START_NEXT, FLAG_LENIENT_REWARD = 1, 2, 4
STEP_FIRST, STEP_MID, STEP_LAST = 0, 1, 2


class HbError(RuntimeError):
    pass


class HbConfig(C.Structure):

    _fields_ = [(n, C.c_int32) for n in ("players", "colors", "ranks", "hand_size", "max_info", "max_life", "flags")]

    def __repr__(self):
        return "HbConfig(" + ", ".join(f"{n}={getattr(self, n)}" for n, _ in self._fields_) + ")"


GAME_TYPES = {
    "Hanabi-Full": dict(colors=5, ranks=5, hand_size=lambda p: 5 if p < 4 else 4, max_info=8, max_life=3),
    "Hanabi-Full-CardKnowledge": dict(colors=5, ranks=5, hand_size=lambda p: 5 if p < 4 else 4, max_info=8, max_life=3),
    "Hanabi-Small": dict(colors=2, ranks=5, hand_size=lambda p: 2, max_info=3, max_life=1),
    "Hanabi-Very-Small": dict(colors=1, ranks=5, hand_size=lambda p: 2, max_info=3, max_life=1),
}


def make_config(game="Hanabi-Full", players=2, flags=0):
    g = GAME_TYPES[game]
    return HbConfig(players, g["colors"], g["ranks"], g["hand_size"](players), g["max_info"], g["max_life"], flags)


class HbAdamTensor(C.Structure):

    _fields_ = [(n, C.c_void_p) for n in ("w", "w_mu", "w_sigma", "noise", "grad", "m_w", "v_w", "m_mu", "v_mu", "m_sigma",
                                          "v_sigma", "eff")] + [("n", C.c_int64), ("cols", C.c_int32), ("eff_ld", C.c_int32),
                                                                                   ("grad_dtype", C.c_int32), ("grad_ld", C.c_int32)]


class HbAdamPack(C.Structure):

    _fields_ = [("wt", C.c_void_p), ("frag", C.c_void_p), ("col_map_dev", C.c_void_p), ("bias_f32", C.c_void_p),
                ("wt_ld", C.c_int32), ("frag_kind", C.c_int32)]


class HbPackJob(C.Structure):

    _fields_ = [("w", C.c_void_p), ("bias", C.c_void_p), ("wt", C.c_void_p), ("bias_out", C.c_void_p)] + [
        (n, C.c_int32) for n in ("k_rows", "n_cols", "w_ld", "group_cols", "k_pad")]


class HbCmd(C.Structure):

    _fields_ = [("op", C.c_int32), ("var", C.c_int32), ("fvar", C.c_int32), ("cond", C.c_int32), ("stream", C.c_void_p),
                ("p", C.c_void_p * 16), ("i", C.c_int64 * 10), ("f", C.c_double * 2)]


(CMD_WAIT_EVENT, CMD_RECORD_EVENT, CMD_REPLAY_INSERT, CMD_ACTOR_FUSED_ACT, CMD_ENV_STEP_PACKED, CMD_TREE_FILL_RANGE,
 CMD_PER_SAMPLE_GATHER, CMD_GRAPH_LAUNCH, CMD_PER_UPDATE, CMD_ACTOR_FUSED_PACK, CMD_ACTOR_PACK_WEIGHTS) = range(1, 12)


class HbFusedTile(C.Structure):

    _fields_ = [(n, C.c_void_p) for n in ("w1f", "b1f", "w2f", "b2f", "support")] + [("first_game_id", C.c_int64),
                                                                                      ("active", C.c_int32), ("pad", C.c_int32)]


class HbRule(C.Structure):

    _fields_ = [("kind", C.c_int32), ("arg", C.c_int32), ("threshold", C.c_float)]


(RULE_LEGAL_RANDOM, RULE_DISCARD_OLDEST_FIRST, RULE_OSAWA_DISCARD, RULE_TELL_UNKNOWN, RULE_TELL_RANDOMLY,
 RULE_PLAY_SAFE_CARD, RULE_PLAY_IF_CERTAIN, RULE_TELL_PLAYABLE_CARD_OUTER, RULE_TELL_DISPENSABLE, RULE_DISCARD_RANDOMLY,
 RULE_PLAY_PROBABLY_SAFE, RULE_DISCARD_PROBABLY_USELESS, RULE_HAIL_MARY, RULE_TELL_ANYONE_USELESS_CARD,
 RULE_TELL_PLAYABLE_CARD, RULE_TELL_MOST_INFORMATION) = range(16)
MAX_RULES = 16
TRAIN_MAX_MEMBERS = 64


def library_path():
    return os.environ.get("HANABI_HIP_LIB") or os.path.join(_HERE, "libhanabi_hip.so")


_P, _I32, _I64, _U64, _F64 = C.c_void_p, C.c_int32, C.c_int64, C.c_uint64, C.c_double
_CFG = C.POINTER(HbConfig)
SIGNATURES = {
    "hb_last_error": (C.c_char_p, []),
    "hb_abi_version": (C.c_int, []),
    "hb_config_validate": (C.c_int, [_CFG]),
    "hb_num_actions": (C.c_int, [_CFG]),
    "hb_obs_len": (C.c_int, [_CFG]),
    "hb_deck_size": (C.c_int, [_CFG]),
    "hb_state_words": (C.c_int, [_CFG]),
    "hb_obs_words": (C.c_int, [_CFG]),
    "hb_env_create": (C.c_int, [_CFG, _I64, _U64, _I64, C.POINTER(_P)]),
    "hb_env_destroy": (C.c_int, [_P]),
    "hb_env_num_games": (_I64, [_P]),
    "hb_env_set_decks": (C.c_int, [_P, _P]),
    "hb_env_reset": (C.c_int, [_P, _P, _I32, _P]),
    "hb_env_observe": (C.c_int, [_P, _P, _P, _P, _P, _P]),
    "hb_env_step": (C.c_int, [_P] + [_P] * 8 + [_P]),
    "hb_env_observe_packed": (C.c_int, [_P, _P, _P, _P, _P, _P, _P]),
    "hb_env_step_packed": (C.c_int, [_P] + [_P] * 9 + [_P]),
    "hb_env_step_select_packed": (C.c_int, [_P, _P, _P, C.c_float, _U64, _U64, _I64, _P] + [_P] * 8 + [_P]),
    "hb_obs_pack": (C.c_int, [_P, _P, _I64, _I32, _P]),
    "hb_obs_unpack": (C.c_int, [_P, _P, _I64, _I32, _P]),
    "hb_env_illegal_count": (C.c_int, [_P, C.POINTER(_I64)]),
    "hb_env_stats": (C.c_int, [_P, C.POINTER(_I64), C.POINTER(_I64)]),
    "hb_env_export_state": (C.c_int, [_P, _P, _P]),
    "hb_env_import_state": (C.c_int, [_P, _P, _P]),
    "hb_env_state": (_P, [_P]),
    "hb_encode_rows": (C.c_int, [_CFG, _P, _I64, _I32, _P, _P, _P, _P]),
    "hb_env_set_color_shuffle": (C.c_int, [_P, _P, C.c_uint8, _P]),
    "hb_env_color_perms": (C.c_int, [_P, _P, _P]),
    "hb_env_color_shuffled": (C.c_int, [_P]),
    "hb_env_set_color_perms": (C.c_int, [_P, _P, _P]),
    "hb_rule_act": (C.c_int, [_CFG, _P, _I64, _I64, C.POINTER(HbRule), _I32, _U64, _U64, _P, _P, _P]),
    "hb_rule_act_grouped": (C.c_int, [_CFG, _P, _I64, _I64, _I64, _P, _P, _P, _I32, _U64, _U64, _P, _P, _P]),
    "hb_rule_act_blocks": (C.c_int, [_CFG, _P, _I64, _I64, _I64, _P, _P, _P, _I32, _U64, _U64, _P, _P, _P]),
    "hb_random_legal_actions": (C.c_int, [_P, _I64, _I32, _U64, _U64, _I64, _P, _P]),
    "hb_env_set_games_per_wave": (C.c_int, [_P, _I32]),
    "hb_env_set_async_refill": (C.c_int, [_P, _I32]),
    "hb_env_set_refill_period": (C.c_int, [_P, _I32]),
    "hb_env_set_profile_events": (C.c_int, [_P, _P, _P]),
    "hb_event_create": (C.c_int, [C.POINTER(_P)]),
    "hb_event_destroy": (C.c_int, [_P]),
    "hb_event_record": (C.c_int, [_P, _P]),
    "hb_stream_wait_event": (C.c_int, [_P, _P]),
    "hb_tree_create": (C.c_int, [_I64, C.POINTER(_P)]),
    "hb_tree_destroy": (C.c_int, [_P]),
    "hb_tree_capacity": (_I64, [_P]),
    "hb_tree_nodes": (_P, [_P]),
    "hb_tree_export_nodes": (C.c_int, [_P, _P, _P]),
    "hb_tree_import_nodes": (C.c_int, [_P, _P, _P]),
    "hb_tree_set_lazy_top": (C.c_int, [_P, _I32]),
    "hb_tree_update": (C.c_int, [_P, _P, _P, _I64, _P]),
    "hb_tree_fill_range": (C.c_int, [_P, _I64, _I64, _P, _P]),
    "hb_tree_sample": (C.c_int, [_P, _P, _P, _P, _I64, _P]),
    "hb_tree_get": (C.c_int, [_P, _P, _P, _I64, _P]),
    "hb_tree_total": (C.c_int, [_P, _P, _P]),
    "hb_tree_error_count": (C.c_int, [_P, C.POINTER(_I64)]),
    "hb_per_sample": (C.c_int, [_P, _P, _I64, _I32, _P, _P, _P]),
    "hb_per_sample_philox": (C.c_int, [_P, _U64, _P, _I64, _P, _P, _P]),
    "hb_per_sample_gather": (C.c_int, [_P, _U64, _P, _I64, _P, _P, _P, _P, _P, _P, _P, _I32, _I32, _P, _I32, _I32, _P, _P, _P, _P, _I32,
                                       C.c_float, _I64, _I64, _P, _P]),
    "hb_per_update": (C.c_int, [_P, _P, _P, _I64, _F64, _P, _P, _P]),
    "hb_obs_cast": (C.c_int, [_P, _P, _I32, _I64, _I32, _I32, _P]),
    "hb_policy_act": (C.c_int, [_P, _I32, _P, _P, _I64, _I32, _I32, _I32, C.c_float, _U64, _U64, _I64, _P, _P, _P]),
    "hb_replay_gather": (C.c_int, [_P] * 6 + [_I64, _I32, _P, _I32, _I32, _P, _P, _P, _P, _I32, C.c_float, _I64, _I64, _P, _P]),
    "hb_replay_gather_packed": (C.c_int, [_P] * 6 + [_I64, _I32, _P, _I32, _I32, _P, _P, _P, _P, _I32, C.c_float, _I64, _I64, _P, _P]),
    "hb_c51_loss_grad": (C.c_int, [_P, _P, _I32, _P, _P, _P, _P, _P, _P, _I32, _P, _I64, _I32, _I32, _I32, _P, _P, _P, _P, _P, _P, _P]),
    "hb_c51_loss_sparse": (C.c_int, [_P, _P, _I32, _P, _P, _P, _P, _P, _P, _I32, _P, _I64, _I32, _I32, _I32, _P, _P, _P, _P, _P, _P, _P]),
    "hb_thin_gemm": (C.c_int, [_P, _P, _P, _P, _I64, _I32, _I32, _I32, _I32, _I32, _I32, _I64, _I64, _I64, _I32, _P]),
    "hb_thin_forward": (C.c_int, [_I32, _P, _P, _P, _P, _P, _I64, _I32, _I32, _I32, _I32, _I32, _I64, _I64, _I64, _I32, _I32, _I32, _P]),
    "hb_dqn_loss_sparse": (C.c_int, [_P, _P, _I32, _P, _P, _P, _P, _P, _P, _I64, _I32, _I32, _I32, _P, _P, _P, _P, _P, _P]),
    "hb_c51_backward": (C.c_int, [_P, _P, _P, _I32, _P, _I32, _I32, _I64, _I32, _I32, _I32, _P, _P, _P, _I32, _P, _P]),
    "hb_colsum": (C.c_int, [_P, _I32, _I64, _I64, _P, _P]),
    "hb_noisy_adam": (C.c_int, [_P] * 11 + [_P, _P, _I32, _I64, _I32, _I32, C.c_float, C.c_float, C.c_float, C.c_float, _P]),
    "hb_noisy_adam_multi": (C.c_int, [C.POINTER(HbAdamTensor), _I32, _P, C.c_float, _I32, C.c_float, C.c_float, C.c_float, C.c_float, _P]),
    "hb_actor_pack_weights": (C.c_int, [C.POINTER(HbPackJob), _I32, _P]),
    "hb_actor_hidden": (C.c_int, [_P, _I64, _I32, _P, _I32, _P, _I32, _P, _P]),
    "hb_actor_hidden_packed": (C.c_int, [_P, _I64, _I32, _P, _I32, _P, _I32, _P, _P]),
    "hb_actor_q": (C.c_int, [_P, _I64, _I32, _P, _P, _P, _I32, _I32, _P, _P]),
    "hb_policy_select": (C.c_int, [_P, _P, _I64, _I32, C.c_float, _U64, _U64, _I64, _P, _P]),
    "hb_actor_q_select": (C.c_int, [_P, _I64, _I32, _P, _P, _P, _I32, _I32, _P, _P, C.c_float, _U64, _U64, _I64, _P, _P, _P]),
    "hb_actor_act": (C.c_int, [_P, _I32, _P, _I64, _I32, _P, _I32, _P, _I32, _P, _P, _P, _P, _I32, _I32, _P, C.c_float, _U64, _U64, _I64,
                               _P, _P, _P]),
    "hb_actor_fused_supported": (C.c_int, [_I32, _I32, _I32, _I32]),
    "hb_actor_fused_sizes": (C.c_int, [_I32, _I32, _I32, _I32, C.POINTER(_I64), C.POINTER(_I64), C.POINTER(_I32)]),
    "hb_actor_fused_pack": (C.c_int, [_P, _I32, _P, _P, _I32, _P, _I32, _I32, _I32, _I32, _P, _P, _P, _P, _P]),
    "hb_actor_fused_q": (C.c_int, [_P, _I64, _I32, _P, _P, _P, _P, _P, _I32, _I32, _I32, _P, _P]),
    "hb_actor_fused_act": (C.c_int, [_P, _P, _I64, _I32, _P, _P, _P, _P, _P, _I32, _I32, _I32, _P, C.c_float, _U64, _U64, _I64, _P, _P]),
    "hb_actor_fused_columns": (C.c_int, [_I32, C.POINTER(_I32)]),
    "hb_noisy_adam_multi_pack": (C.c_int, [_P, _P, _I32, _P, C.c_float, _I32, C.c_float, C.c_float, C.c_float, C.c_float, _P]),
    "hb_actor_fused_pack_dt": (C.c_int, [_P, _I32, _P, _P, _I32, _P, _I32, _I32, _I32, _I32, _P, _P, _P, _P, _I32, _P]),
    "hb_actor_fused_pack_thin": (C.c_int, [_P, _I32, _P, _P, _I32, _P, _I32, _I32, _I32, _I32, _P, _P, _P, _P, _P, _I32, _P, _I32, _I32, _P]),
    "hb_actor_fused_q_dt": (C.c_int, [_P, _I64, _I32, _P, _P, _P, _P, _P, _I32, _I32, _I32, _P, _I32, _P]),
    "hb_actor_fused_act_dt": (C.c_int, [_P, _P, _I64, _I32, _P, _P, _P, _P, _P, _I32, _I32, _I32, _P, C.c_float, _U64, _U64, _I64, _P, _I32, _P]),
    "hb_actor_fused_act_step": (C.c_int, [_P, _P, _P, _I64, _I32, _P, _P, _P, _P, _P, _I32, _I32, _I32, _P, C.c_float, _U64, _U64, _I64, _P,
                                          _I32] + [_P] * 7 + [_P]),
    "hb_actor_fused_step_supported": (C.c_int, [_P]),
    "hb_actor_fused_act_grouped": (C.c_int, [_P, _I64, _P, _P, _I32, _I32, _I32, _I32, _P, C.c_float, _U64, _U64, _P, _I32, _P]),
    "hb_chain_run": (C.c_int, [C.POINTER(HbCmd), _I32, C.POINTER(_I64), C.POINTER(_F64)]),
    "hb_eval_counters": (C.c_int, [_CFG]),
    "hb_eval_tally": (C.c_int, [_CFG, _I64, _I32, _I32] + [_P] * 8 + [_P]),
    "hb_eval_tally_grouped": (C.c_int, [_CFG, _I64, _I64, _I32, _I32] + [_P] * 8 + [_P]),
    "hb_eval_response_bins": (C.c_int, [_CFG]),
    "hb_eval_response_tally": (C.c_int, [_CFG, _I64, _I32] + [_P] * 4 + [_P]),
    "hb_eval_response_tally_grouped": (C.c_int, [_CFG, _I64, _I64, _I32] + [_P] * 4 + [_P]),
    "hb_train_counters": (C.c_int, [_CFG]),
    "hb_train_tally_init": (C.c_int, [_CFG, _P, _I64, _P, _P, _P]),
    "hb_train_tally": (C.c_int, [_CFG, _I64, _I32] + [_P] * 5 + [_I32] + [_P] * 3 + [_P]),
    "hb_belief_determinize": (C.c_int, [_CFG, _P, _I64, _I32, _I32, _U64, _U64, _I64, _P, _P, _P]),
    "hb_search_reduce": (C.c_int, [_P, _P, _P, _I64, _I32, _I32, _P, _P, _P, _P, _P]),
    "hb_search_layout": (C.c_int, [_CFG, _P, _P, _P, _P, _I64, _I32, _I32, _P, _P, _P, _P, _P]),
    "hb_search_compare": (C.c_int, [_P, _P, _P, _P, _I64, _I32, _I32, _P, _P, _P, _P]),
    "hb_belief_splice": (C.c_int, [_CFG, _P, _P, _I64, _I32, _I32, _P, _P]),
    "hb_belief_select": (C.c_int, [_CFG, _P, _P, _P, _P, _P, _P, _I64, _I32, _I32, _P, _P, _P, _P, _P]),
    "hb_belief_splice_alive": (C.c_int, [_CFG, _P, _P, _P, _I64, _I32, _I32, _P, _P]),
    "hb_belief_select_depth": (C.c_int, [_CFG, _P, _P, _P, _P, _P, _P, _I64, _I32, _I32, _I32, _P, _P, _P, _P, _P, _P]),
    "hb_belief_select_soft": (C.c_int, [_CFG, _P, _P, _P, _P, _P, _P, _P, _P, _I64, _I32, _I32, _I32, _U64, _U64, _I64, _P, _P, _P, _P,
                                        _P, _P, _P]),
    "hb_belief_history_step": (C.c_int, [_CFG, _I64, _I32, _I32, _P, _P, _P, _P, _P, _P, _P, _P, _P]),
    "hb_belief_score": (C.c_int, [_CFG, _P, _P, _P, _I64, _I32, _I32, _P, _P, _P, _P, _P, _P, _P, _P]),
    "hb_belief_carry": (C.c_int, [_CFG, _P, _P, _P, _P, _P, _P, _I64, _I32, _I32, _U64, _U64, _I64, _P, _P, _P]),
    "hb_relu_bwd_colsum": (C.c_int, [_P, _P, _I64, _I32, _I64, _I64, _P, _P]),
    "hb_replay_insert": (C.c_int, [_P] * 12 + [_I64, _I32, _I32, _I64, _I64, _P]),
    "hb_obl_insert": (C.c_int, [_P] * 12 + [_I64, _I32, _I32, _I32, _I64, _I64, _P]),
}


def lib():
    global _LIB
    if _LIB is None:
        path = library_path()
        if not os.path.exists(path):
            raise HbError(f"{path} is missing: build it with `python -c 'import __graft_entry__ as g; g.build()'` "
                          f"(there is no CPU fallback)")
        L = C.CDLL(path)
        for name, (res, args) in SIGNATURES.items():
            fn = getattr(L, name)
            fn.restype = res
            fn.argtypes = args
        _LIB = L
    return _LIB


def check(rc):
    if rc != 0:
        raise HbError(f"hanabi_hip error {rc}: {lib().hb_last_error().decode()}")


_RAW_STREAM = None


def current_stream():
    global _RAW_STREAM
    import torch

    if _RAW_STREAM is None:
        raw = getattr(torch._C, "_cuda_getCurrentRawStream", None)
        _RAW_STREAM = (lambda: raw(torch._C._cuda_getDevice())) if raw is not None else (
            lambda: torch.cuda.current_stream().cuda_stream)
    return C.c_void_p(_RAW_STREAM())


def dptr(t):
    return None if t is None else C.c_void_p(t.data_ptr())


class Event:

    __slots__ = ("h", "_lib", "recorded")

    def __init__(self):
        self._lib = lib()
        h = C.c_void_p()
        check(self._lib.hb_event_create(C.byref(h)))
        self.h = h
        self.recorded = False

    def record(self, stream=None):
        check(self._lib.hb_event_record(self.h, current_stream() if stream is None else stream))
        self.recorded = True

    def wait(self, stream=None):
        if self.recorded:
            check(self._lib.hb_stream_wait_event(current_stream() if stream is None else stream, self.h))

    def __del__(self):
        try:
            if self.h:
                self._lib.hb_event_destroy(self.h)
        except Exception:
            pass


def set_stream(stream):
    import torch

    torch._C._cuda_setStream(stream_id=stream.stream_id, device_index=stream.device_index, device_type=stream.device_type)
```

### include/hanabi_hip.h

```cpp
#ifndef HANABI_HIP_H
#define HANABI_HIP_H

#include <stdint.h>

#ifdef __cplusplus
extern "C" {
#endif

#define HB_ABI_VERSION 1

#define HB_OK 0
#define HB_ERR_INVALID (-1)
#define HB_ERR_NO_DEVICE (-2)
#define HB_ERR_HIP (-3)
#define HB_ERR_ALIGN (-4)
#define HB_ERR_NOMEM (-5)

const char* hb_last_error(void);
int hb_abi_version(void);

typedef struct hb_config {
  int32_t players;
  int32_t colors;
  int32_t ranks;
  int32_t hand_size;
  int32_t max_info;
  int32_t max_life;
  int32_t flags;
} hb_config;

#define HB_FLAG_AUTO_RESET 1u
#define HB_FLAG_RESET_START_NEXT 2u
#define HB_FLAG_LENIENT_REWARD 4u

#define HB_STEP_FIRST 0
#define HB_STEP_MID 1
#define HB_STEP_LAST 2

int hb_config_validate(const hb_config* cfg);
int hb_num_actions(const hb_config* cfg);
int hb_obs_len(const hb_config* cfg);
int hb_deck_size(const hb_config* cfg);
int hb_state_words(const hb_config* cfg);
int hb_obs_words(const hb_config* cfg);

typedef struct hb_env hb_env;

int hb_env_create(const hb_config* cfg, int64_t n_games, uint64_t seed, int64_t first_game_id, hb_env** out);
int hb_env_destroy(hb_env* env);
int64_t hb_env_num_games(const hb_env* env);

int hb_env_set_decks(hb_env* env, const uint8_t* decks_dev);

int hb_env_reset(hb_env* env, const uint8_t* mask_dev, int32_t start_player, void* stream);

int hb_env_observe(hb_env* env, int8_t* obs_dev, int8_t* legal_dev, float* agent_reward_dev,
                   int8_t* agent_step_type_dev, void* stream);

int hb_env_step(hb_env* env, const int32_t* actions_dev, int8_t* obs_dev, int8_t* legal_dev,
                float* reward_dev, int8_t* terminal_dev, float* agent_reward_dev,
                int8_t* agent_step_type_dev, int8_t* score_dev, void* stream);

int hb_env_observe_packed(hb_env* env, uint32_t* obs_bits_dev, int8_t* obs_dev, int8_t* legal_dev, float* agent_reward_dev,
                          int8_t* agent_step_type_dev, void* stream);
int hb_env_step_packed(hb_env* env, const int32_t* actions_dev, uint32_t* obs_bits_dev, int8_t* obs_dev, int8_t* legal_dev,
                       float* reward_dev, int8_t* terminal_dev, float* agent_reward_dev, int8_t* agent_step_type_dev,
                       int8_t* score_dev, void* stream);

int hb_env_step_select_packed(hb_env* env, const float* q_dev, const int8_t* sel_legal_dev, float epsilon, uint64_t seed,
                              uint64_t draw, int64_t first_game_id, int32_t* actions_out_dev, uint32_t* obs_bits_dev,
                              int8_t* obs_dev, int8_t* legal_dev, float* reward_dev, int8_t* terminal_dev,
                              float* agent_reward_dev, int8_t* agent_step_type_dev, int8_t* score_dev, void* stream);
int hb_obs_pack(const int8_t* obs_dev, uint32_t* bits_dev, int64_t rows, int32_t obs_len, void* stream);
int hb_obs_unpack(const uint32_t* bits_dev, int8_t* obs_dev, int64_t rows, int32_t obs_len, void* stream);

int hb_env_illegal_count(hb_env* env, int64_t* out);

int hb_env_stats(hb_env* env, int64_t* episodes, int64_t* score_sum);

int hb_env_export_state(hb_env* env, uint32_t* rows_dev, void* stream);
int hb_env_import_state(hb_env* env, const uint32_t* rows_dev, void* stream);

int hb_encode_rows(const hb_config* cfg, const uint32_t* rows_dev, int64_t n_rows, int32_t seat, uint32_t* obs_bits_dev,
                   int8_t* obs_dev, int8_t* legal_dev, void* stream);

int hb_env_set_color_shuffle(hb_env* env, const uint8_t* seat_mask_dev, uint8_t all_seats_mask, void* stream);
int hb_env_color_perms(hb_env* env, uint8_t* out_dev, void* stream);
int hb_env_color_shuffled(const hb_env* env);
int hb_env_set_color_perms(hb_env* env, const uint8_t* perms_dev, void* stream);

int hb_random_legal_actions(const int8_t* legal_dev, int64_t n_games, int32_t n_actions, uint64_t seed,
                            uint64_t draw, int64_t first_game_id, int32_t* actions_dev, void* stream);

enum {
  HB_RULE_LEGAL_RANDOM = 0,
  HB_RULE_DISCARD_OLDEST_FIRST = 1,
  HB_RULE_OSAWA_DISCARD = 2,
  HB_RULE_TELL_UNKNOWN = 3,
  HB_RULE_TELL_RANDOMLY = 4,
  HB_RULE_PLAY_SAFE_CARD = 5,
  HB_RULE_PLAY_IF_CERTAIN = 6,
  HB_RULE_TELL_PLAYABLE_CARD_OUTER = 7,
  HB_RULE_TELL_DISPENSABLE = 8,
  HB_RULE_DISCARD_RANDOMLY = 9,
  HB_RULE_PLAY_PROBABLY_SAFE = 10,
  HB_RULE_DISCARD_PROBABLY_USELESS = 11,
  HB_RULE_HAIL_MARY = 12,
  HB_RULE_TELL_ANYONE_USELESS_CARD = 13,
  HB_RULE_TELL_PLAYABLE_CARD = 14,
  HB_RULE_TELL_MOST_INFORMATION = 15,
  HB_RULE_KINDS = 16
};
#define HB_MAX_RULES 16
typedef struct hb_rule {
  int32_t kind;
  int32_t arg;
  float threshold;
} hb_rule;

const uint32_t* hb_env_state(hb_env* env);

int hb_rule_act(const hb_config* cfg, const uint32_t* state_rows_dev, int64_t n_games, int64_t first_game_id,
                const hb_rule* rules, int32_t n_rules, uint64_t seed, uint64_t draw, int32_t* actions_dev,
                int32_t* fired_dev, void* stream);
int hb_rule_act_grouped(const hb_config* cfg, const uint32_t* state_rows_dev, int64_t n_blocks, int64_t block_rows,
                        int64_t first_game_id, const int32_t* set_of_block_dev, const hb_rule* rules_dev,
                        const int32_t* n_rules_dev, int32_t n_sets, uint64_t seed, uint64_t draw, int32_t* actions_dev,
                        int32_t* fired_dev, void* stream);
int hb_rule_act_blocks(const hb_config* cfg, const uint32_t* state_rows_dev, int64_t n_blocks, int64_t block_rows,
                       int64_t first_game_id, const int32_t* set_of_block_dev, const hb_rule* rules_dev,
                       const int32_t* n_rules_dev, int32_t n_sets, uint64_t seed, uint64_t draw, int32_t* actions_dev,
                       int32_t* fired_dev, void* stream);

int hb_env_set_games_per_wave(hb_env* env, int32_t g);

int hb_env_set_async_refill(hb_env* env, int32_t on);
int hb_env_set_refill_period(hb_env* env, int32_t steps);

int hb_env_set_profile_events(hb_env* env, void* start_event, void* stop_event);

int hb_event_create(void** event_out);
int hb_event_destroy(void* event);
int hb_event_record(void* event, void* stream);
int hb_stream_wait_event(void* stream, void* event);

typedef struct hb_tree hb_tree;

int hb_tree_create(int64_t capacity, hb_tree** out);
int hb_tree_destroy(hb_tree* t);
int64_t hb_tree_capacity(const hb_tree* t);
float* hb_tree_nodes(hb_tree* t);
int hb_tree_export_nodes(hb_tree* t, float* nodes_dev, void* stream);
int hb_tree_import_nodes(hb_tree* t, const float* nodes_dev, void* stream);

int hb_tree_set_lazy_top(hb_tree* t, int32_t on);

int hb_tree_update(hb_tree* t, const int64_t* idx_dev, const float* val_dev, int64_t n, void* stream);

int hb_tree_fill_range(hb_tree* t, int64_t start, int64_t n, const float* value_dev, void* stream);

int hb_tree_sample(hb_tree* t, const float* quantile_dev, int64_t* idx_dev, float* val_dev, int64_t n,
                   void* stream);

int hb_tree_get(hb_tree* t, const int64_t* idx_dev, float* val_dev, int64_t n, void* stream);

int hb_tree_total(hb_tree* t, float* total_dev, void* stream);

int hb_tree_error_count(hb_tree* t, int64_t* out);

int hb_per_sample(hb_tree* t, const double* u_dev, int64_t batch, int32_t unit_uniforms, int64_t* idx_dev,
                  double* prob_dev, void* stream);
int hb_per_sample_philox(hb_tree* t, uint64_t seed, const float* counter_dev, int64_t batch, int64_t* idx_dev,
                         double* prob_dev, void* stream);
int hb_per_sample_gather(hb_tree* t, uint64_t seed, const float* counter_dev, int64_t batch, int64_t* idx_dev, double* prob_dev,
                         const void* ring_obs_tm1_dev, const void* ring_obs_t_dev, const int8_t* ring_act_dev,
                         const float* ring_rew_dev, const uint8_t* ring_term_dev, int32_t obs_len, int32_t packed, void* x_dev,
                         int32_t x_dtype, int32_t x_ld, int32_t* act_dev, float* rew_dev, float* term_dev, float* disc_dev,
                         int32_t n_step, float gamma, int64_t capacity, int64_t rows_per_insert, const int64_t* size_wp_dev,
                         void* stream);
int hb_per_update(hb_tree* t, const int64_t* idx_dev, const float* td_dev, int64_t n, double alpha,
                  float* max_prio_dev, float* min_prio_dev, void* stream);

int hb_policy_act(const void* logits_dev, int32_t logits_dtype, const int8_t* legal_dev, const float* support_dev,
                  int64_t n_games, int32_t n_actions, int32_t n_atoms, int32_t row_stride, float epsilon, uint64_t seed,
                  uint64_t draw, int64_t first_game_id, int32_t* actions_dev, float* q_dev, void* stream);

int hb_obs_cast(const int8_t* obs_dev, void* out_dev, int32_t out_dtype, int64_t rows, int32_t cols, int32_t out_ld,
                void* stream);

int hb_replay_insert(int8_t* last_obs_dev, const int8_t* obs_dev, const int8_t* legal_dev, const int32_t* actions_dev,
                     const float* rewards_dev, const int8_t* step_type_dev, int8_t* ring_obs_tm1_dev,
                     int8_t* ring_obs_t_dev, int8_t* ring_act_dev, int8_t* ring_lms_dev, float* ring_rew_dev,
                     uint8_t* ring_term_dev, int64_t n, int32_t obs_len, int32_t n_actions, int64_t capacity,
                     int64_t start, void* stream);

int hb_obl_insert(const int8_t* obs_tm1_dev, const int32_t* actions_dev, const float* rewards_dev, const int8_t* terminal_dev,
                  const int8_t* obs_t_dev, const int8_t* legal_t_dev, int8_t* ring_obs_tm1_dev, int8_t* ring_obs_t_dev,
                  int8_t* ring_act_dev, int8_t* ring_lms_dev, float* ring_rew_dev, uint8_t* ring_term_dev, int64_t n,
                  int32_t n_steps, int32_t row_bytes, int32_t n_actions, int64_t capacity, int64_t start, void* stream);

int hb_replay_gather(const int8_t* ring_obs_tm1_dev, const int8_t* ring_obs_t_dev, const int8_t* ring_act_dev,
                     const float* ring_rew_dev, const uint8_t* ring_term_dev, const int64_t* idx_dev, int64_t batch,
                     int32_t obs_len, void* x_dev, int32_t x_dtype, int32_t x_ld, int32_t* act_dev, float* rew_dev,
                     float* term_dev, float* disc_dev, int32_t n_step, float gamma, int64_t capacity, int64_t rows_per_insert,
                     const int64_t* size_wp_dev, void* stream);

int hb_replay_gather_packed(const uint32_t* ring_bits_tm1_dev, const uint32_t* ring_bits_t_dev, const int8_t* ring_act_dev,
                            const float* ring_rew_dev, const uint8_t* ring_term_dev, const int64_t* idx_dev, int64_t batch,
                            int32_t obs_len, void* x_dev, int32_t x_dtype, int32_t x_ld, int32_t* act_dev, float* rew_dev,
                            float* term_dev, float* disc_dev, int32_t n_step, float gamma, int64_t capacity,
                            int64_t rows_per_insert, const int64_t* size_wp_dev, void* stream);

int hb_c51_loss_grad(const void* logits_online_dev, const void* logits_target_dev, int32_t dtype, const int32_t* act_dev,
                     const float* rew_dev, const float* term_dev, const double* prios_dev, const float* beta_dev,
                     const float* disc_dev, int32_t mask_terminal, const float* support_dev, int64_t batch, int32_t n_actions,
                     int32_t n_atoms, int32_t row_stride, float* td_dev, float* w_dev, void* dlogits_dev,
                     float* update_counter_dev, const void* bias_online_dev, const void* bias_target_dev, void* stream);

int hb_c51_loss_sparse(const void* logits_online_dev, const void* logits_target_dev, int32_t dtype, const int32_t* act_dev,
                       const float* rew_dev, const float* term_dev, const double* prios_dev, const float* beta_dev,
                       const float* disc_dev, int32_t mask_terminal, const float* support_dev, int64_t batch, int32_t n_actions,
                       int32_t n_atoms, int32_t row_stride, float* td_dev, float* w_dev, float* dl_dev, float* update_counter_dev,
                       const void* bias_online_dev, const void* bias_target_dev, void* stream);

int hb_thin_gemm(const void* x_dev, const void* wt_dev, const void* bias_dev, void* out_dev, int64_t m, int32_t n, int32_t k,
                 int32_t ldx, int32_t ldw, int32_t ldo, int32_t batch, int64_t x_batch_stride, int64_t w_batch_stride,
                 int64_t out_batch_stride, int32_t relu, void* stream);

int hb_thin_forward(int32_t layer, const void* x_dev, const void* wt_dev, const void* bias_dev, void* out_dev, const int32_t* act_dev,
                    int64_t batch, int32_t n, int32_t k, int32_t ldx, int32_t ldw, int32_t ldo, int64_t x_batch_stride,
                    int64_t w_batch_stride, int64_t out_batch_stride, int32_t n_actions, int32_t n_atoms, int32_t relu, void* stream);

int hb_dqn_loss_sparse(const void* q_online_dev, const void* q_target_dev, int32_t dtype, const int32_t* act_dev, const float* rew_dev,
                       const float* term_dev, const double* prios_dev, const float* beta_dev, const float* disc_dev, int64_t batch,
                       int32_t n_actions, int32_t col_stride, int32_t row_stride, float* td_dev, float* w_dev, float* dl_dev,
                       const void* bias_online_dev, const void* bias_target_dev, void* stream);

int hb_c51_backward(const float* dl_dev, const int32_t* act_dev, const void* hidden_dev, int32_t hidden_ld, const void* w2_dev,
                    int32_t w2_ld, int32_t dtype, int64_t batch, int32_t hidden, int32_t n_actions, int32_t n_atoms, void* dh_dev,
                    float* db1_dev, void* dw2_dev, int32_t dw2_ld, float* db2_dev, void* stream);

int hb_colsum(const void* x_dev, int32_t dtype, int64_t rows, int64_t cols, float* out_dev, void* stream);

int hb_noisy_adam(float* w_dev, float* w_mu_dev, float* w_sigma_dev, const float* noise_dev, const float* grad_dev,
                  float* m_w_dev, float* v_w_dev, float* m_mu_dev, float* v_mu_dev, float* m_sigma_dev, float* v_sigma_dev,
                  const float* step_dev, void* eff_dev, int32_t eff_dtype, int64_t n, int32_t cols, int32_t eff_ld, float lr,
                  float beta1, float beta2, float eps, void* stream);

typedef struct hb_adam_tensor {
  float *w, *w_mu, *w_sigma;
  const float* noise;
  const void* grad;
  float *m_w, *v_w, *m_mu, *v_mu, *m_sigma, *v_sigma;
  void* eff;
  int64_t n;
  int32_t cols, eff_ld;
  int32_t grad_dtype, grad_ld;
} hb_adam_tensor;
int hb_noisy_adam_multi(const hb_adam_tensor* tensors , int32_t count,
                        const float* step_dev, float step_offset, int32_t eff_dtype, float lr, float beta1, float beta2,
                        float eps, void* stream);

typedef struct hb_adam_pack {
  void* wt;
  void* frag;
  const int32_t* col_map_dev;
  float* bias_f32;
  int32_t wt_ld, frag_kind;
} hb_adam_pack;
int hb_noisy_adam_multi_pack(const hb_adam_tensor* tensors, const hb_adam_pack* packs, int32_t count, const float* step_dev,
                             float step_offset, int32_t eff_dtype, float lr, float beta1, float beta2, float eps, void* stream);

int hb_relu_bwd_colsum(void* dy_dev, const void* act_dev, int64_t act_ld , int32_t dtype,
                       int64_t rows, int64_t cols, float* out_dev, void* stream);

typedef struct hb_pack_job {
  const void* w;
  const void* bias;
  void* wt;
  float* bias_out;
  int32_t k_rows, n_cols, w_ld, group_cols, k_pad;
} hb_pack_job;
int hb_actor_pack_weights(const hb_pack_job* jobs , int32_t count ,
                          void* stream);
int hb_actor_hidden(const int8_t* obs_dev, int64_t n_rows, int32_t obs_len, const void* w1t_dev, int32_t k_pad,
                    const float* b1_dev, int32_t hidden, void* h_dev, void* stream);
int hb_actor_hidden_packed(const uint32_t* obs_bits_dev, int64_t n_rows, int32_t obs_len, const void* w1t_dev, int32_t k_pad,
                           const float* b1_dev, int32_t hidden, void* h_dev, void* stream);
int hb_actor_q(const void* h_dev, int64_t n_rows, int32_t hidden, const void* w2t_dev, const float* b2_dev,
               const float* support_dev, int32_t n_actions, int32_t n_atoms, float* q_dev, void* stream);
int hb_policy_select(const float* q_dev, const int8_t* legal_dev, int64_t n_games, int32_t n_actions, float epsilon,
                     uint64_t seed, uint64_t draw, int64_t first_game_id, int32_t* actions_dev, void* stream);

int hb_actor_q_select(const void* h_dev, int64_t n_rows, int32_t hidden, const void* w2t_dev, const float* b2_dev,
                      const float* support_dev, int32_t n_actions, int32_t n_atoms, float* q_dev, const int8_t* legal_dev,
                      float epsilon, uint64_t seed, uint64_t draw, int64_t first_game_id, int32_t* actions_dev,
                      uint32_t* tickets_dev, void* stream);

int hb_actor_act(const void* obs_dev, int32_t obs_is_packed, const int8_t* legal_dev, int64_t n_rows, int32_t obs_len,
                 const void* w1t_dev, int32_t k_pad, const float* b1_dev, int32_t hidden, void* h_dev, const void* w2t_dev,
                 const float* b2_dev, const float* support_dev, int32_t n_actions, int32_t n_atoms, float* q_dev, float epsilon,
                 uint64_t seed, uint64_t draw, int64_t first_game_id, int32_t* actions_dev, uint32_t* tickets_dev, void* stream);

int hb_actor_fused_supported(int32_t obs_len, int32_t hidden, int32_t n_actions, int32_t n_atoms);
int hb_actor_fused_sizes(int32_t obs_len, int32_t hidden, int32_t n_actions, int32_t n_atoms, int64_t* w1f_bytes,
                         int64_t* w2f_bytes, int32_t* b2f_floats);
int hb_actor_fused_pack(const void* w1_dev, int32_t w1_ld, const void* b1_dev, const void* w2_dev, int32_t w2_ld,
                        const void* b2_dev, int32_t obs_len, int32_t hidden, int32_t n_actions, int32_t n_atoms, void* w1f_dev,
                        float* b1f_dev, void* w2f_dev, float* b2f_dev, void* stream);
int hb_actor_fused_q(const uint32_t* obs_bits_dev, int64_t n_rows, int32_t obs_len, const void* w1f_dev, const float* b1f_dev,
                     const void* w2f_dev, const float* b2f_dev, const float* support_dev, int32_t hidden, int32_t n_actions,
                     int32_t n_atoms, float* q_dev, void* stream);
int hb_actor_fused_act(const uint32_t* obs_bits_dev, const int8_t* legal_dev, int64_t n_rows, int32_t obs_len, const void* w1f_dev,
                       const float* b1f_dev, const void* w2f_dev, const float* b2f_dev, const float* support_dev, int32_t hidden,
                       int32_t n_actions, int32_t n_atoms, float* q_dev, float epsilon, uint64_t seed, uint64_t draw,
                       int64_t first_game_id, int32_t* actions_dev, void* stream);
int hb_actor_fused_columns(int32_t n_actions, int32_t* phys_of_logit_host);
int hb_actor_fused_pack_dt(const void* w1_dev, int32_t w1_ld, const void* b1_dev, const void* w2_dev, int32_t w2_ld,
                           const void* b2_dev, int32_t obs_len, int32_t hidden, int32_t n_actions, int32_t n_atoms, void* w1f_dev,
                           float* b1f_dev, void* w2f_dev, float* b2f_dev, int32_t dtype, void* stream);
int hb_actor_fused_pack_thin(const void* w1_dev, int32_t w1_ld, const void* b1_dev, const void* w2_dev, int32_t w2_ld,
                             const void* b2_dev, int32_t obs_len, int32_t hidden, int32_t n_actions, int32_t n_atoms,
                             void* w1f_dev, float* b1f_dev, void* w2f_dev, float* b2f_dev, void* w1t_dev, int32_t w1t_ld,
                             void* w2t_dev, int32_t w2t_ld, int32_t dtype, void* stream);
int hb_actor_fused_q_dt(const uint32_t* obs_bits_dev, int64_t n_rows, int32_t obs_len, const void* w1f_dev, const float* b1f_dev,
                        const void* w2f_dev, const float* b2f_dev, const float* support_dev, int32_t hidden, int32_t n_actions,
                        int32_t n_atoms, float* q_dev, int32_t dtype, void* stream);
int hb_actor_fused_act_dt(const uint32_t* obs_bits_dev, const int8_t* legal_dev, int64_t n_rows, int32_t obs_len,
                          const void* w1f_dev, const float* b1f_dev, const void* w2f_dev, const float* b2f_dev,
                          const float* support_dev, int32_t hidden, int32_t n_actions, int32_t n_atoms, float* q_dev, float epsilon,
                          uint64_t seed, uint64_t draw, int64_t first_game_id, int32_t* actions_dev, int32_t dtype, void* stream);
int hb_actor_fused_act_step(hb_env* env, const uint32_t* obs_bits_dev, const int8_t* legal_dev, int64_t n_rows, int32_t obs_len,
                            const void* w1f_dev, const float* b1f_dev, const void* w2f_dev, const float* b2f_dev,
                            const float* support_dev, int32_t hidden, int32_t n_actions, int32_t n_atoms, float* q_dev, float epsilon,
                            uint64_t seed, uint64_t draw, int64_t first_game_id, int32_t* actions_dev, int32_t dtype,
                            uint32_t* obs_bits_out_dev, int8_t* legal_out_dev, float* reward_dev, int8_t* terminal_dev,
                            float* agent_reward_dev, int8_t* agent_step_type_dev, int8_t* score_dev, void* stream);
int hb_actor_fused_step_supported(const hb_env* env);

typedef struct hb_fused_tile {
  const void* w1f;
  const float* b1f;
  const void* w2f;
  const float* b2f;
  const float* support;
  int64_t first_game_id;
  int32_t active;
  int32_t pad;
} hb_fused_tile;
int hb_actor_fused_act_grouped(const hb_fused_tile* tiles_dev, int64_t n_rows, const uint32_t* obs_bits_dev, const int8_t* legal_dev,
                               int32_t obs_len, int32_t hidden, int32_t n_actions, int32_t n_atoms, float* q_dev, float epsilon,
                               uint64_t seed, uint64_t draw, int32_t* actions_dev, int32_t dtype, void* stream);

int hb_eval_counters(const hb_config* cfg);
int hb_eval_tally(const hb_config* cfg, int64_t n_games, int32_t seat, int32_t turn, const int32_t* actions_dev,
                  const float* reward_dev, const int8_t* terminal_dev, const int8_t* score_dev, uint8_t* done_dev,
                  int8_t* final_score_dev, int16_t* length_dev, int64_t* counters_dev, void* stream);
int hb_eval_tally_grouped(const hb_config* cfg, int64_t n_blocks, int64_t block_games, int32_t seat, int32_t turn,
                          const int32_t* actions_dev, const float* reward_dev, const int8_t* terminal_dev, const int8_t* score_dev,
                          uint8_t* done_dev, int8_t* final_score_dev, int16_t* length_dev, int64_t* counters_dev, void* stream);

int hb_eval_response_bins(const hb_config* cfg);
int hb_eval_response_tally(const hb_config* cfg, int64_t n_games, int32_t seat, const int32_t* actions_dev, const uint8_t* done_dev,
                           int32_t* prev_dev, int64_t* resp_dev, void* stream);
int hb_eval_response_tally_grouped(const hb_config* cfg, int64_t n_blocks, int64_t block_games, int32_t seat,
                                   const int32_t* actions_dev, const uint8_t* done_dev, int32_t* prev_dev, int64_t* resp_dev,
                                   void* stream);

#define HB_TRAIN_MAX_MEMBERS 64
int hb_train_counters(const hb_config* cfg);
int hb_train_tally_init(const hb_config* cfg, const uint32_t* state_rows_dev, int64_t n_games, uint8_t* lost_dev, int16_t* length_dev,
                        void* stream);
int hb_train_tally(const hb_config* cfg, int64_t n_games, int32_t seat, const int32_t* actions_dev, const float* reward_dev,
                   const int8_t* terminal_dev, const int8_t* score_dev, const int32_t* tile_member_dev, int32_t n_members,
                   uint8_t* lost_dev, int16_t* length_dev, int64_t* counters_dev, void* stream);

int hb_belief_determinize(const hb_config* cfg, const uint32_t* src_rows_dev, int64_t m, int32_t seat, int32_t replicas, uint64_t seed,
                          uint64_t draw, int64_t first_row_id, uint32_t* out_rows_dev, uint32_t* weight_dev, void* stream);
int hb_search_reduce(const int8_t* score_dev, const uint32_t* weight_dev, const int8_t* legal_dev, int64_t m, int32_t n_actions,
                     int32_t replicas, float* value_dev, int64_t* wsum_dev, int32_t* n_live_dev, int32_t* best_dev, void* stream);
int hb_search_layout(const hb_config* cfg, const uint32_t* det_rows_dev, const uint32_t* weight_dev, const int32_t* cand_dev,
                     const int32_t* filler_dev, int64_t m, int32_t n_cand, int32_t replicas, uint32_t* rows_out_dev,
                     int32_t* forced_out_dev, uint8_t* done_out_dev, int32_t* n_played_out_dev, void* stream);
int hb_search_compare(const int8_t* score_dev, const uint32_t* weight_dev, const int32_t* cand_dev, const int32_t* base_slot_dev,
                      int64_t m, int32_t n_cand, int32_t replicas, double* diff_dev, double* se_dev, int32_t* n_pair_dev, void* stream);
int hb_belief_splice(const hb_config* cfg, const uint32_t* prev_rows_dev, const uint32_t* det_rows_dev, int64_t m, int32_t seat,
                     int32_t n_cand, uint32_t* out_rows_dev, void* stream);
int hb_belief_select(const hb_config* cfg, const uint32_t* src_rows_dev, const uint32_t* det_rows_dev, const uint32_t* weight_dev,
                     const int32_t* hyp_moves_dev, const int32_t* actual_dev, const uint8_t* valid_dev, int64_t m, int32_t n_cand,
                     int32_t replicas, uint32_t* out_rows_dev, uint32_t* out_weight_dev, int32_t* n_surv_dev, uint8_t* fallback_dev,
                     void* stream);
int hb_belief_splice_alive(const hb_config* cfg, const uint32_t* prev_rows_dev, const uint8_t* alive_dev, const uint32_t* det_rows_dev,
                           int64_t m, int32_t seat, int32_t n_cand, uint32_t* out_rows_dev, void* stream);
int hb_belief_select_depth(const hb_config* cfg, const uint32_t* src_rows_dev, const uint32_t* det_rows_dev, const uint32_t* weight_dev,
                           const int32_t* hyp_moves_dev, const int32_t* actual_dev, const uint8_t* valid_dev, int64_t m, int32_t n_cand,
                           int32_t replicas, int32_t depth, uint32_t* out_rows_dev, uint32_t* out_weight_dev, int32_t* n_surv_dev,
                           int32_t* depth_used_dev, uint8_t* fallback_dev, void* stream);
int hb_belief_select_soft(const hb_config* cfg, const uint32_t* src_rows_dev, const uint32_t* det_rows_dev, const uint32_t* weight_dev,
                          const int32_t* hyp_moves_dev, const int32_t* n_legal_dev, const int32_t* actual_dev, const uint8_t* valid_dev,
                          const double* p_table_dev, int64_t m, int32_t n_cand, int32_t replicas, int32_t depth, uint64_t seed,
                          uint64_t draw, int64_t first_row_id, uint32_t* out_rows_dev, uint32_t* out_weight_dev, int32_t* n_surv_dev,
                          int32_t* depth_used_dev, uint8_t* fallback_dev, float* ess_dev, void* stream);
int hb_belief_history_step(const hb_config* cfg, int64_t m, int32_t depth, int32_t seat, const int32_t* own_moves_dev,
                           const uint8_t* reset_dev, const uint32_t* cur_rows_dev, const uint32_t* prev_rows_dev,
                           uint32_t* hist_rows_dev, int32_t* hist_moves_dev, uint8_t* hist_alive_dev, uint8_t* hist_valid_dev,
                           void* stream);
int hb_belief_score(const hb_config* cfg, const uint32_t* true_rows_dev, const uint32_t* det_rows_dev, const uint32_t* weight_dev,
                    int64_t m, int32_t seat, int32_t replicas, int8_t* truth_dev, int64_t* hit_dev, int64_t* joint_dev,
                    int64_t* wsum_dev, int32_t* n_live_dev, int64_t* counts_dev, int8_t* prior_dev, void* stream);
int hb_belief_carry(const hb_config* cfg, const uint32_t* cur_rows_dev, const uint32_t* old_rows_dev, const uint32_t* old_weight_dev,
                    const int32_t* own_slot_dev, const int32_t* revealed_dev, const int32_t* drew_dev, int64_t m, int32_t seat,
                    int32_t n_particles, uint64_t seed, uint64_t draw, int64_t first_row_id, uint32_t* out_rows_dev,
                    uint32_t* out_weight_dev, void* stream);

enum {
  HB_CMD_WAIT_EVENT = 1,
  HB_CMD_RECORD_EVENT = 2,
  HB_CMD_REPLAY_INSERT = 3,
  HB_CMD_ACTOR_FUSED_ACT = 4,
  HB_CMD_ENV_STEP_PACKED = 5,
  HB_CMD_TREE_FILL_RANGE = 6,
  HB_CMD_PER_SAMPLE_GATHER = 7,
  HB_CMD_GRAPH_LAUNCH = 8,
  HB_CMD_PER_UPDATE = 9,
  HB_CMD_ACTOR_FUSED_PACK = 10,
  HB_CMD_ACTOR_PACK_WEIGHTS = 11
};
typedef struct hb_cmd {
  int32_t op, var, fvar, cond;
  void* stream;
  void* p[16];
  int64_t i[10];
  double f[2];
} hb_cmd;
int hb_chain_run(const hb_cmd* cmds, int32_t count, const int64_t* vars_i, const double* vars_f);

#ifdef __cplusplus
}
#endif
#endif
```

Baseline: 317.2 million.

## Restructure noisy Adam kernels to batch loads up front and vectorize eff stores

Moves the noisy Adam per-element work into a shared adam_group helper. It issues every optimizer-state load before any arithmetic (with a sched barrier) and writes the effective weights with one packed vector store. It adds an optional non-temporal load/store path, on by default only for width 2, and exposes width and streaming through a new API entry point. The learner2 kernel prefetches priorities and unrolls row staging to overlap loads. In exchange, the vectorized path now requires eff alignment and a tighter index-range check, and the compiler barriers may raise register pressure.

```diff
diff --git a/hanabi-agents_amd/csrc/learner.hip b/hanabi-agents_amd/csrc/learner.hip
--- a/hanabi-agents_amd/csrc/learner.hip
+++ b/hanabi-agents_amd/csrc/learner.hip
@@ -242,6 +242,11 @@
 __device__ __forceinline__ float merged(float w, float mu, float sg, float nz) {
   return __fadd_rn(__fadd_rn(w, mu), __fmul_rn(sg, nz));
 }
+__device__ __forceinline__ float merged_f32(float w, float mu, float sg, float nz) {
+  float v = merged(w, mu, sg, nz);
+  asm volatile("" : "+v"(v));
+  return v;
+}
 
 template <typename T>
 __global__ __launch_bounds__(256) void noisy_adam_kernel(const AdamArgs a) {
@@ -268,7 +273,7 @@
     m = a.m_sg[i]; v = a.v_sg[i];
     const float sg = adam1(a.w_sigma[i], __fmul_rn(g, nz), m, v, a.b1, a.b2, bc1, bc2s, a.lr, a.eps);
     a.m_sg[i] = m; a.v_sg[i] = v; a.w_sigma[i] = sg;
-    st<T>(eff, row * a.eff_ld + col, merged(w, mu, sg, nz));
+    st<T>(eff, row * a.eff_ld + col, merged_f32(w, mu, sg, nz));
   }
 }
 
@@ -278,91 +283,123 @@
   int count;
 };
 
+typedef float f32x4 __attribute__((ext_vector_type(4)));
+typedef float f32x2 __attribute__((ext_vector_type(2)));
+typedef uint32_t u32x2 __attribute__((ext_vector_type(2)));
 template <int W> struct VecW;
-template <> struct VecW<4> { typedef float4 type; };
-template <> struct VecW<2> { typedef float2 type; };
-template <int W>
-__device__ __forceinline__ void ldw(const float* p, uint32_t off, float out[W]) {
-  const typename VecW<W>::type v = *reinterpret_cast<const typename VecW<W>::type*>(reinterpret_cast<const char*>(p) + static_cast<uint64_t>(off << 2));
-  const float* f = reinterpret_cast<const float*>(&v);
-#pragma unroll
-  for (int k = 0; k < W; ++k) out[k] = f[k];
-}
-template <int W>
-__device__ __forceinline__ void stw(float* p, uint32_t off, const float in[W]) {
-  typename VecW<W>::type v;
-  float* f = reinterpret_cast<float*>(&v);
-#pragma unroll
-  for (int k = 0; k < W; ++k) f[k] = in[k];
-  *reinterpret_cast<typename VecW<W>::type*>(reinterpret_cast<char*>(p) + static_cast<uint64_t>(off << 2)) = v;
-}
-template <int W>
-__device__ __forceinline__ void load_gradw(const void* g, int dtype, uint32_t i, float out[W]) {
-  if (dtype == 0) {
-    ldw<W>(static_cast<const float*>(g), i, out);
-  } else if (dtype == 1) {
-    const uint32_t* p = reinterpret_cast<const uint32_t*>(static_cast<const char*>(g) + static_cast<uint64_t>(i << 1));
-    if constexpr (W == 4) {
-      const uint2 v = *reinterpret_cast<const uint2*>(p);
-      out[0] = __uint_as_float(v.x << 16); out[1] = __uint_as_float(v.x & 0xFFFF0000u);
-      out[2] = __uint_as_float(v.y << 16); out[3] = __uint_as_float(v.y & 0xFFFF0000u);
-    } else {
-      const uint32_t v = *p;
-      out[0] = __uint_as_float(v << 16); out[1] = __uint_as_float(v & 0xFFFF0000u);
-    }
+template <> struct VecW<4> { typedef f32x4 type; };
+template <> struct VecW<2> { typedef f32x2 type; };
+template <int BYTES> struct Bits;
+template <> struct Bits<16> { typedef f32x4 type; };
+template <> struct Bits<8> { typedef u32x2 type; };
+template <> struct Bits<4> { typedef uint32_t type; };
+template <typename V, bool NT>
+__device__ __forceinline__ V ldv(const void* p, uint32_t byte_off) {
+  const V* q = reinterpret_cast<const V*>(static_cast<const char*>(p) + static_cast<uint64_t>(byte_off));
+  if constexpr (NT) return __builtin_nontemporal_load(q);
+  else return *q;
+}
+template <typename V, bool NT>
+__device__ __forceinline__ void stv(void* p, uint32_t byte_off, V v) {
+  V* q = reinterpret_cast<V*>(static_cast<char*>(p) + static_cast<uint64_t>(byte_off));
+  if constexpr (NT) __builtin_nontemporal_store(v, q);
+  else *q = v;
+}
+template <typename T, int W, bool NT>
+__device__ __forceinline__ void st_eff(T* eff, uint32_t e, const float v[W]) {
+  T r[W];
+#pragma unroll
+  for (int k = 0; k < W; ++k) st<T>(r, k, v[k]);
+  typename Bits<W * sizeof(T)>::type bits;
+  __builtin_memcpy(&bits, r, sizeof(bits));
+  stv<typename Bits<W * sizeof(T)>::type, NT>(eff, e * static_cast<uint32_t>(sizeof(T)), bits);
+}
+
+template <int W, bool NT>
+__device__ __forceinline__ void adam_group(const AdamArgs& a, uint32_t i, uint32_t goff, float mv[W]) {
+  typedef typename VecW<W>::type V;
+  typedef typename Bits<2 * W>::type H;
+  const bool shared = a.m_mu == a.m_w;
+  const float t = *a.step + a.step_offset;
+  const uint32_t o = i << 2;
+  V gf;
+  if (a.grad_dtype == 0) {
+    gf = ldv<V, NT>(a.grad, goff << 2);
   } else {
-    const __half* h = reinterpret_cast<const __half*>(static_cast<const char*>(g) + static_cast<uint64_t>(i << 1));
-#pragma unroll
-    for (int k = 0; k < W; ++k) out[k] = __half2float(h[k]);
-  }
-}
-
-template <typename T, int W>
+    const H gh = ldv<H, NT>(a.grad, goff << 1);
+    __builtin_memcpy(&gf, &gh, sizeof(gh));
+  }
+  const V nz = ldv<V, NT>(a.noise, o);
+  V pw = ldv<V, NT>(a.w, o), mw = ldv<V, NT>(a.m_w, o), vw = ldv<V, NT>(a.v_w, o);
+  V pmu = ldv<V, NT>(a.w_mu, o);
+  V psg = ldv<V, NT>(a.w_sigma, o), msg = ldv<V, NT>(a.m_sg, o), vsg = ldv<V, NT>(a.v_sg, o);
+  asm volatile("" ::: "memory");
+  __builtin_amdgcn_sched_barrier(0);
+  float bc1 = 1.f - powf(a.b1, t), bc2s = sqrtf(1.f - powf(a.b2, t));
+  asm volatile("" : "+v"(bc1), "+v"(bc2s), "+v"(gf));
+  uint32_t os = o;
+  asm volatile("" : "+v"(os));
+  float g[W];
+  if (a.grad_dtype == 0) {
+#pragma unroll
+    for (int k = 0; k < W; ++k) g[k] = gf[k];
+  } else {
+    uint32_t d[W / 2];
+    __builtin_memcpy(d, &gf, sizeof(d));
+#pragma unroll
+    for (int k = 0; k < W; k += 2) {
+      if (a.grad_dtype == 1) {
+        g[k] = __uint_as_float(d[k / 2] << 16); g[k + 1] = __uint_as_float(d[k / 2] & 0xFFFF0000u);
+      } else {
+        const __half2 h2 = *reinterpret_cast<const __half2*>(&d[k / 2]);
+        g[k] = __low2float(h2); g[k + 1] = __high2float(h2);
+      }
+    }
+  }
+#pragma unroll
+  for (int k = 0; k < W; ++k) {
+    float m1 = mw[k], v1 = vw[k];
+    pw[k] = adam1(pw[k], g[k], m1, v1, a.b1, a.b2, bc1, bc2s, a.lr, a.eps);
+    mw[k] = m1; vw[k] = v1;
+    float m3 = msg[k], v3 = vsg[k];
+    psg[k] = adam1(psg[k], __fmul_rn(g[k], nz[k]), m3, v3, a.b1, a.b2, bc1, bc2s, a.lr, a.eps);
+    msg[k] = m3; vsg[k] = v3;
+  }
+  if (shared) {
+#pragma unroll
+    for (int k = 0; k < W; ++k) pmu[k] = __fsub_rn(pmu[k], adam_step(mw[k], vw[k], bc1, bc2s, a.lr, a.eps));
+  } else {
+    V mmu = ldv<V, NT>(a.m_mu, os), vmu = ldv<V, NT>(a.v_mu, os);
+#pragma unroll
+    for (int k = 0; k < W; ++k) {
+      float m2 = mmu[k], v2 = vmu[k];
+      pmu[k] = adam1(pmu[k], g[k], m2, v2, a.b1, a.b2, bc1, bc2s, a.lr, a.eps);
+      mmu[k] = m2; vmu[k] = v2;
+    }
+    stv<V, NT>(a.m_mu, os, mmu); stv<V, NT>(a.v_mu, os, vmu);
+  }
+#pragma unroll
+  for (int k = 0; k < W; ++k) mv[k] = merged(pw[k], pmu[k], psg[k], nz[k]);
+  stv<V, NT>(a.w, os, pw); stv<V, NT>(a.m_w, os, mw); stv<V, NT>(a.v_w, os, vw);
+  stv<V, NT>(a.w_mu, os, pmu);
+  stv<V, NT>(a.w_sigma, os, psg); stv<V, NT>(a.m_sg, os, msg); stv<V, NT>(a.v_sg, os, vsg);
+}
+
+template <typename T, int W, bool NT>
 __global__ __launch_bounds__(256) void noisy_adam_multiw_kernel(const AdamMulti m) {
   constexpr int SH = W == 4 ? 2 : 1;
+  const int blk = static_cast<int>(blockIdx.x);
   int ti = 0;
-  while (ti + 1 < m.count && static_cast<int>(blockIdx.x) >= m.first[ti + 1]) ++ti;
+  while (ti + 1 < m.count && blk >= m.first[ti + 1]) ++ti;
+  ti = __builtin_amdgcn_readfirstlane(ti);
   const AdamArgs& a = m.t[ti];
-  const float t = *a.step + a.step_offset;
-  const float bc1 = 1.f - powf(a.b1, t), bc2s = sqrtf(1.f - powf(a.b2, t));
-  T* eff = static_cast<T*>(a.eff);
   const int nw = static_cast<int>(a.n >> SH), cw = a.cols >> SH;
-  const int q = (static_cast<int>(blockIdx.x) - m.first[ti]) * 256 + static_cast<int>(threadIdx.x);
+  const int q = (blk - m.first[ti]) * 256 + static_cast<int>(threadIdx.x);
   if (q < nw) {
     const int row = q / cw, col = (q - row * cw) << SH;
-    const uint32_t i = static_cast<uint32_t>(q) << SH;
-    float g[W], nz[W];
-    load_gradw<W>(a.grad, a.grad_dtype, static_cast<uint32_t>(row) * static_cast<uint32_t>(a.grad_ld) + col, g);
-    ldw<W>(a.noise, i, nz);
-    float res[3][W], lm[W], lv[W];
-    auto one = [&](float* p, float* mp, float* vp, int which) {
-      float pa[W], ma[W], va[W];
-      ldw<W>(p, i, pa); ldw<W>(mp, i, ma); ldw<W>(vp, i, va);
-#pragma unroll
-      for (int k = 0; k < W; ++k) {
-        pa[k] = adam1(pa[k], which == 2 ? __fmul_rn(g[k], nz[k]) : g[k], ma[k], va[k], a.b1, a.b2, bc1, bc2s, a.lr, a.eps);
-        res[which][k] = pa[k];
-        lm[k] = ma[k];
-        lv[k] = va[k];
-      }
-      stw<W>(p, i, pa); stw<W>(mp, i, ma); stw<W>(vp, i, va);
-    };
-    one(a.w, a.m_w, a.v_w, 0);
-
-    if (a.m_mu == a.m_w) {
-      float pv[W];
-      ldw<W>(a.w_mu, i, pv);
-#pragma unroll
-      for (int k = 0; k < W; ++k) res[1][k] = pv[k] = __fsub_rn(pv[k], adam_step(lm[k], lv[k], bc1, bc2s, a.lr, a.eps));
-      stw<W>(a.w_mu, i, pv);
-    } else {
-      one(a.w_mu, a.m_mu, a.v_mu, 1);
-    }
-
-    one(a.w_sigma, a.m_sg, a.v_sg, 2);
-    const uint32_t e = static_cast<uint32_t>(row) * static_cast<uint32_t>(a.eff_ld) + col;
-#pragma unroll
-    for (int k = 0; k < W; ++k) st<T>(eff, e + k, merged(res[0][k], res[1][k], res[2][k], nz[k]));
+    float mv[W];
+    adam_group<W, NT>(a, static_cast<uint32_t>(q) << SH, static_cast<uint32_t>(row) * static_cast<uint32_t>(a.grad_ld) + col, mv);
+    st_eff<T, W, NT>(static_cast<T*>(a.eff), static_cast<uint32_t>(row) * static_cast<uint32_t>(a.eff_ld) + col, mv);
   }
 }
 
@@ -395,7 +432,7 @@
     mm = a.m_sg[i]; vv = a.v_sg[i];
     const float sg = adam1(a.w_sigma[i], __fmul_rn(g, nz), mm, vv, a.b1, a.b2, bc1, bc2s, a.lr, a.eps);
     a.m_sg[i] = mm; a.v_sg[i] = vv; a.w_sigma[i] = sg;
-    st<T>(eff, row * a.eff_ld + col, merged(w, mu, sg, nz));
+    st<T>(eff, row * a.eff_ld + col, merged_f32(w, mu, sg, nz));
   }
 }
 
@@ -421,8 +458,6 @@
   const AdamArgs& a = m.t[ti];
   const AdamPackOut& o = m.o[ti];
   const int tid = static_cast<int>(threadIdx.x), tb = static_cast<int>(blockIdx.x) - m.first[ti];
-  const float t = *a.step + a.step_offset;
-  const float bc1 = 1.f - powf(a.b1, t), bc2s = sqrtf(1.f - powf(a.b2, t));
   T* eff = static_cast<T*>(a.eff);
   const int tn = m.tiles_n[ti];
   const int rows = static_cast<int>(a.n / a.cols);
@@ -438,38 +473,9 @@
   float mv[4] = {0.f, 0.f, 0.f, 0.f};
   if (valid) {
     const uint32_t i = static_cast<uint32_t>(k) * static_cast<uint32_t>(a.cols) + n;
-    float g[4], nz[4], res[3][4], lm[4], lv[4];
-    load_gradw<4>(a.grad, a.grad_dtype, static_cast<uint32_t>(k) * static_cast<uint32_t>(a.grad_ld) + n, g);
-    ldw<4>(a.noise, i, nz);
-    auto one = [&](float* p, float* mp, float* vp, int which) {
-      float pa[4], ma[4], va[4];
-      ldw<4>(p, i, pa); ldw<4>(mp, i, ma); ldw<4>(vp, i, va);
-#pragma unroll
-      for (int j = 0; j < 4; ++j) {
-        pa[j] = adam1(pa[j], which == 2 ? __fmul_rn(g[j], nz[j]) : g[j], ma[j], va[j], a.b1, a.b2, bc1, bc2s, a.lr, a.eps);
-        res[which][j] = pa[j];
-        lm[j] = ma[j];
-        lv[j] = va[j];
-      }
-      stw<4>(p, i, pa); stw<4>(mp, i, ma); stw<4>(vp, i, va);
-    };
-    one(a.w, a.m_w, a.v_w, 0);
-    if (a.m_mu == a.m_w) {
-      float pv[4];
-      ldw<4>(a.w_mu, i, pv);
-#pragma unroll
-      for (int j = 0; j < 4; ++j) res[1][j] = pv[j] = __fsub_rn(pv[j], adam_step(lm[j], lv[j], bc1, bc2s, a.lr, a.eps));
-      stw<4>(a.w_mu, i, pv);
-    } else {
-      one(a.w_mu, a.m_mu, a.v_mu, 1);
-    }
-    one(a.w_sigma, a.m_sg, a.v_sg, 2);
+    adam_group<4, false>(a, i, static_cast<uint32_t>(k) * static_cast<uint32_t>(a.grad_ld) + n, mv);
     const uint32_t e = static_cast<uint32_t>(k) * static_cast<uint32_t>(a.eff_ld) + n;
-#pragma unroll
-    for (int j = 0; j < 4; ++j) {
-      mv[j] = merged(res[0][j], res[1][j], res[2][j], nz[j]);
-      st<T>(eff, e + j, mv[j]);
-    }
+    st_eff<T, 4, false>(eff, e, mv);
     if (tn == 0 && o.bias_f32) {
 #pragma unroll
       for (int j = 0; j < 4; ++j) o.bias_f32[o.col_map ? o.col_map[n + j] : n + j] = ld<T>(eff, e + j);
@@ -509,6 +515,9 @@
   if (blocks > 2048) blocks = 2048;
   hipLaunchKernelGGL((noisy_adam_kernel<T>), dim3(static_cast<unsigned>(blocks)), dim3(256), 0, s, a);
 }
+
+constexpr int HB_ADAM_DEFAULT_WIDTH = 4;
+constexpr bool HB_ADAM_NT_W4 = false, HB_ADAM_NT_W2 = true;
 
 }
 
@@ -646,24 +655,28 @@
   return HB_OK;
 }
 
-int hb_noisy_adam_multi(const hb_adam_tensor* tensors, int32_t count, const float* step_dev, float step_offset, int32_t eff_dtype,
-                        float lr, float beta1, float beta2, float eps, void* stream) {
+int hb_noisy_adam_multi_width(const hb_adam_tensor* tensors, int32_t count, const float* step_dev, float step_offset,
+                              int32_t eff_dtype, float lr, float beta1, float beta2, float eps, int32_t width, int32_t streaming,
+                              void* stream) {
   if (!tensors || !step_dev) return fail(HB_ERR_INVALID, "null argument");
   if (count < 1 || count > 8) return fail(HB_ERR_INVALID, "count must be 1..8");
+  if (width != 4 && width != 2 && width != 1) return fail(HB_ERR_INVALID, "width must be 4, 2 or 1");
+  if (streaming < -1 || streaming > 1) return fail(HB_ERR_INVALID, "streaming must be -1 (the width's default), 0 or 1");
+  if (eff_dtype < 0 || eff_dtype > 2) return fail(HB_ERR_INVALID, "eff_dtype must be 0 (f32), 1 (bf16) or 2 (f16)");
+  const bool nt = streaming < 0 ? (width == 2 ? HB_ADAM_NT_W2 : HB_ADAM_NT_W4) : streaming == 1;
   AdamMulti m{};
   m.count = count;
   int blocks = 0;
-  bool vec4 = true;
-  const int width = [] { const char* e = getenv("HB_ADAM_WIDTH"); const int w = e ? atoi(e) : 4; return w == 2 || w == 1 ? w : 4; }();
-  if (width == 1) vec4 = false;
+  bool vec4 = width != 1;
+  const uintptr_t eff_mask = (eff_dtype == 0 ? 16u : 8u) - 1u;
   for (int i = 0; i < count; ++i) {
     const hb_adam_tensor& d = tensors[i];
     const int gl = d.grad_ld ? d.grad_ld : d.cols;
     auto al16 = [](const void* p) { return (reinterpret_cast<uintptr_t>(p) & 15u) == 0; };
     vec4 = vec4 && d.cols > 0 && d.cols % 4 == 0 && d.n % 4 == 0 && d.n < (1LL << 30) &&
-           (d.n / d.cols) * static_cast<long long>(d.eff_ld > gl ? d.eff_ld : gl) < (1LL << 31) && d.eff_ld % 4 == 0 && gl % 4 == 0 && al16(d.w) &&
+           (d.n / d.cols) * static_cast<long long>(d.eff_ld > gl ? d.eff_ld : gl) < (1LL << 30) && d.eff_ld % 4 == 0 && gl % 4 == 0 && al16(d.w) &&
            al16(d.w_mu) && al16(d.w_sigma) && al16(d.noise) && al16(d.grad) && al16(d.m_w) && al16(d.v_w) && al16(d.m_mu) &&
-           al16(d.v_mu) && al16(d.m_sigma) && al16(d.v_sigma);
+           al16(d.v_mu) && al16(d.m_sigma) && al16(d.v_sigma) && (reinterpret_cast<uintptr_t>(d.eff) & eff_mask) == 0;
   }
   for (int i = 0; i < count; ++i) {
     const hb_adam_tensor& d = tensors[i];
@@ -682,18 +695,26 @@
   }
   m.first[count] = blocks;
   hipStream_t s = static_cast<hipStream_t>(stream);
-  if (vec4 && width == 4 && eff_dtype == 0) hipLaunchKernelGGL((noisy_adam_multiw_kernel<float, 4>), dim3(blocks), dim3(256), 0, s, m);
-  else if (vec4 && width == 4 && eff_dtype == 1) hipLaunchKernelGGL((noisy_adam_multiw_kernel<__hip_bfloat16, 4>), dim3(blocks), dim3(256), 0, s, m);
-  else if (vec4 && width == 4 && eff_dtype == 2) hipLaunchKernelGGL((noisy_adam_multiw_kernel<__half, 4>), dim3(blocks), dim3(256), 0, s, m);
-  else if (vec4 && eff_dtype == 0) hipLaunchKernelGGL((noisy_adam_multiw_kernel<float, 2>), dim3(blocks), dim3(256), 0, s, m);
-  else if (vec4 && eff_dtype == 1) hipLaunchKernelGGL((noisy_adam_multiw_kernel<__hip_bfloat16, 2>), dim3(blocks), dim3(256), 0, s, m);
-  else if (vec4 && eff_dtype == 2) hipLaunchKernelGGL((noisy_adam_multiw_kernel<__half, 2>), dim3(blocks), dim3(256), 0, s, m);
-  else if (eff_dtype == 0) hipLaunchKernelGGL((noisy_adam_multi_kernel<float>), dim3(blocks), dim3(256), 0, s, m);
-  else if (eff_dtype == 1) hipLaunchKernelGGL((noisy_adam_multi_kernel<__hip_bfloat16>), dim3(blocks), dim3(256), 0, s, m);
-  else if (eff_dtype == 2) hipLaunchKernelGGL((noisy_adam_multi_kernel<__half>), dim3(blocks), dim3(256), 0, s, m);
-  else return fail(HB_ERR_INVALID, "eff_dtype must be 0 (f32), 1 (bf16) or 2 (f16)");
+#define HB_ADAM_W(T)                                                                                                       \
+  do {                                                                                                                     \
+    if (!vec4) hipLaunchKernelGGL((noisy_adam_multi_kernel<T>), dim3(blocks), dim3(256), 0, s, m);                         \
+    else if (width == 4 && nt) hipLaunchKernelGGL((noisy_adam_multiw_kernel<T, 4, true>), dim3(blocks), dim3(256), 0, s, m);  \
+    else if (width == 4) hipLaunchKernelGGL((noisy_adam_multiw_kernel<T, 4, false>), dim3(blocks), dim3(256), 0, s, m);    \
+    else if (nt) hipLaunchKernelGGL((noisy_adam_multiw_kernel<T, 2, true>), dim3(blocks), dim3(256), 0, s, m);             \
+    else hipLaunchKernelGGL((noisy_adam_multiw_kernel<T, 2, false>), dim3(blocks), dim3(256), 0, s, m);                    \
+  } while (0)
+  if (eff_dtype == 0) HB_ADAM_W(float);
+  else if (eff_dtype == 1) HB_ADAM_W(__hip_bfloat16);
+  else HB_ADAM_W(__half);
+#undef HB_ADAM_W
   HB_HIP(hipGetLastError());
   return HB_OK;
+}
+
+int hb_noisy_adam_multi(const hb_adam_tensor* tensors, int32_t count, const float* step_dev, float step_offset, int32_t eff_dtype,
+                        float lr, float beta1, float beta2, float eps, void* stream) {
+  const int width = [] { const char* e = getenv("HB_ADAM_WIDTH"); const int w = e ? atoi(e) : HB_ADAM_DEFAULT_WIDTH; return w == 4 || w == 2 || w == 1 ? w : HB_ADAM_DEFAULT_WIDTH; }();
+  return hb_noisy_adam_multi_width(tensors, count, step_dev, step_offset, eff_dtype, lr, beta1, beta2, eps, width, -1, stream);
 }
 
 
@@ -716,7 +737,7 @@
     const int gl = d.grad_ld ? d.grad_ld : d.cols;
     const long long rows = d.n / d.cols;
     if (d.grad_dtype < 0 || d.grad_dtype > 2 || gl < d.cols) return fail(HB_ERR_INVALID, "bad gradient dtype / row stride in tensor %d", i);
-    if (d.cols % 4 || d.n >= (1LL << 30) || rows * static_cast<long long>(d.eff_ld > gl ? d.eff_ld : gl) >= (1LL << 31) || d.eff_ld % 4 ||
+    if (d.cols % 4 || d.n >= (1LL << 30) || rows * static_cast<long long>(d.eff_ld > gl ? d.eff_ld : gl) >= (1LL << 30) || d.eff_ld % 4 ||
         gl % 4 || !al16(d.w) || !al16(d.w_mu) || !al16(d.w_sigma) || !al16(d.noise) || !al16(d.grad) || !al16(d.m_w) || !al16(d.v_w) ||
         !al16(d.m_mu) || !al16(d.v_mu) || !al16(d.m_sigma) || !al16(d.v_sigma) || (reinterpret_cast<uintptr_t>(d.eff) & 7u))
       return fail(HB_ERR_ALIGN, "tensor %d: needs cols, row strides %% 4 == 0 and 16-byte aligned arrays", i);
diff --git a/hanabi-agents_amd/csrc/learner2.hip b/hanabi-agents_amd/csrc/learner2.hip
--- a/hanabi-agents_amd/csrc/learner2.hip
+++ b/hanabi-agents_amd/csrc/learner2.hip
@@ -73,18 +73,30 @@
 template <> __device__ __forceinline__ uint32_t pack2<float>(float lo, float) { return __float_as_uint(lo); }
 
 template <typename T>
+__device__ __forceinline__ float ld_off(const T* base, uint32_t e) {
+  return ld<T>(reinterpret_cast<const T*>(reinterpret_cast<const char*>(base) + static_cast<uint64_t>(e * static_cast<uint32_t>(sizeof(T)))), 0);
+}
+template <typename T>
 __device__ __forceinline__ void stage_row(const T* __restrict__ row, const T* __restrict__ bias, float* dst, int n, int lane) {
-  for (int base = 0; base < n; base += 1024) {
-    float v[16];
-#pragma unroll
-    for (int i = 0; i < 16; ++i) {
+  for (int base = 0; base < n; base += 512) {
+    float v[8], bv[8];
+#pragma unroll
+    for (int i = 0; i < 8; ++i) {
       const int e = base + lane + 64 * i;
-      v[i] = e < n ? ld<T>(row, e) + (bias ? ld<T>(bias, e) : 0.f) : 0.f;
-    }
-#pragma unroll
-    for (int i = 0; i < 16; ++i) {
+      v[i] = ld_off<T>(row, static_cast<uint32_t>(e < n ? e : n - 1));
+    }
+    const T* bsrc = bias ? bias : row;
+#pragma unroll
+    for (int i = 0; i < 8; ++i) {
       const int e = base + lane + 64 * i;
-      if (e < n) dst[e] = v[i];
+      bv[i] = ld_off<T>(bsrc, static_cast<uint32_t>(e < n ? e : n - 1));
+    }
+#pragma unroll
+    for (int i = 0; i < 8; ++i) bv[i] = bias ? bv[i] : 0.f;
+#pragma unroll
+    for (int i = 0; i < 8; ++i) {
+      const int e = base + lane + 64 * i;
+      if (e < n) dst[e] = v[i] + bv[i];
     }
   }
 }
@@ -106,6 +118,13 @@
   const float r_b = rew[b];
   float gamma = disc[b];
   if (mask_terminal) gamma *= 1.f - term[b];
+  const float beta = *beta_dev;
+  const double pr_b = prios[b];
+  double pr[4];
+#pragma unroll
+  for (int u = 0; u < 4; ++u) pr[u] = lane + 64 * u < B ? prios[lane + 64 * u] : 1.0;
+  asm volatile("" ::: "memory");
+  __builtin_amdgcn_sched_barrier(0);
   const bool atom = lane < K;
   const T* row_sel = logits_on + static_cast<long long>(B + b) * rs;
   stage_row<T>(row_sel, bias_on, sel, AK, lane);
@@ -114,9 +133,16 @@
   const float l1 = atom ? ld<T>(logits_on, static_cast<long long>(b) * rs + a_tm1 * K + lane) +
                               (bias_on ? ld<T>(bias_on, a_tm1 * K + lane) : 0.f)
                         : -INFINITY;
-  const float beta = *beta_dev;
   float ipmin = INFINITY, ipmax = 0.f;
-  for (int j = lane; j < B; j += 64) {
+#pragma unroll
+  for (int u = 0; u < 4; ++u) {
+    if (lane + 64 * u < B) {
+      const float ip = static_cast<float>(1.0 / pr[u]);
+      ipmin = fminf(ipmin, ip);
+      ipmax = fmaxf(ipmax, ip);
+    }
+  }
+  for (int j = lane + 256; j < B; j += 64) {
     const float ip = static_cast<float>(1.0 / prios[j]);
     ipmin = fminf(ipmin, ip);
     ipmax = fmaxf(ipmax, ip);
@@ -124,7 +150,7 @@
   ipmin = wave_min(ipmin);
   ipmax = wave_max(ipmax);
   const float wmax = powf(beta >= 0.f ? ipmax : ipmin, beta);
-  const float w_b = powf(static_cast<float>(1.0 / prios[b]), beta) / wmax;
+  const float w_b = powf(static_cast<float>(1.0 / pr_b), beta) / wmax;
   wave_fence();
   const int S = 64 / A >= 1 ? 64 / A : 1;
   const int a_l = lane / S, part = lane - a_l * S;
diff --git a/hanabi-agents_amd/hanabi_agents/rlax_dqn/fused_learner.py b/hanabi-agents_amd/hanabi_agents/rlax_dqn/fused_learner.py
--- a/hanabi-agents_amd/hanabi_agents/rlax_dqn/fused_learner.py
+++ b/hanabi-agents_amd/hanabi_agents/rlax_dqn/fused_learner.py
@@ -96,6 +96,8 @@
             raise ValueError("actor_lag=1 needs the MFMA actor (bf16 GEMM dtype, one hidden layer of a multiple of 256 units), "
                              "prioritized replay and frozen noise")
         self.adam_pack = None
+        self.adam_width = None
+        self.adam_streaming = -1
         self._pack_tab = None
         self._gw2_out = torch.zeros(H, self.Np, dtype=self.cd, device=dev)
         self._gw1_out = torch.zeros(self.Kp, H, dtype=self.cd, device=dev)
@@ -318,9 +320,13 @@
                                                      float(p.learning_rate), 0.9, 0.999, 3.125e-5, K.current_stream()))
             self._packed_in_part2 = True
             return
-        if opt:
+        if opt and self.adam_width is None:
             K.check(K.lib().hb_noisy_adam_multi(self._adam_table(), 4, K.dptr(self.step), 0.0, _DT[self.cd],
                                                 float(p.learning_rate), 0.9, 0.999, 3.125e-5, K.current_stream()))
+        elif opt:
+            K.check(K.lib().hb_noisy_adam_multi_width(self._adam_table(), 4, K.dptr(self.step), 0.0, _DT[self.cd],
+                                                      float(p.learning_rate), 0.9, 0.999, 3.125e-5, int(self.adam_width), int(self.adam_streaming),
+                                                      K.current_stream()))
         if not pack:
             return
         self._packed_in_part2 = False
diff --git a/hanabi-agents_amd/hanabi_hip/_capi.py b/hanabi-agents_amd/hanabi_hip/_capi.py
--- a/hanabi-agents_amd/hanabi_hip/_capi.py
+++ b/hanabi-agents_amd/hanabi_hip/_capi.py
@@ -161,6 +161,7 @@
     "hb_colsum": (C.c_int, [_P, _I32, _I64, _I64, _P, _P]),
     "hb_noisy_adam": (C.c_int, [_P] * 11 + [_P, _P, _I32, _I64, _I32, _I32, C.c_float, C.c_float, C.c_float, C.c_float, _P]),
     "hb_noisy_adam_multi": (C.c_int, [C.POINTER(HbAdamTensor), _I32, _P, C.c_float, _I32, C.c_float, C.c_float, C.c_float, C.c_float, _P]),
+    "hb_noisy_adam_multi_width": (C.c_int, [C.POINTER(HbAdamTensor), _I32, _P, C.c_float, _I32, C.c_float, C.c_float, C.c_float, C.c_float, _I32, _I32, _P]),
     "hb_actor_pack_weights": (C.c_int, [C.POINTER(HbPackJob), _I32, _P]),
     "hb_actor_hidden": (C.c_int, [_P, _I64, _I32, _P, _I32, _P, _I32, _P, _P]),
     "hb_actor_hidden_packed": (C.c_int, [_P, _I64, _I32, _P, _I32, _P, _I32, _P, _P]),
diff --git a/include/hanabi_hip.h b/include/hanabi_hip.h
--- a/include/hanabi_hip.h
+++ b/include/hanabi_hip.h
@@ -260,6 +260,9 @@
 int hb_noisy_adam_multi(const hb_adam_tensor* tensors , int32_t count,
                         const float* step_dev, float step_offset, int32_t eff_dtype, float lr, float beta1, float beta2,
                         float eps, void* stream);
+int hb_noisy_adam_multi_width(const hb_adam_tensor* tensors, int32_t count, const float* step_dev, float step_offset,
+                              int32_t eff_dtype, float lr, float beta1, float beta2, float eps, int32_t width, int32_t streaming,
+                              void* stream);
 
 typedef struct hb_adam_pack {
   void* wt;
```

New measurement: 321.9 million (median of 5 runs). 1.5% higher.
